# lRomul/sensorium

Measured on AMD Instinct MI355X. Metric: training clips/sec/GPU (DwiseNeuro fwd+bwd, B=32 T=32 36x64) at 1/2/4/8 GPUs, higher is better.
Workload: dtype bf16

## Files before the change

### include/dwn.h

```cpp
#ifndef DWN_H_
#define DWN_H_
#include <stddef.h>
#include <stdint.h>

#ifdef __cplusplus
extern "C" {
#endif

#define DWN_ABI_VERSION 7
#define DWN_F32 0
#define DWN_BF16 1
#define DWN_F32_AUTO 0
#define DWN_F32_NATIVE 1
#define DWN_F32_SPLIT3 2
#define DWN_BN_EVAL 0
#define DWN_BN_TRAIN 1
#define DWN_BN_FROZEN 2
#define DWN_NREP 32

#define DWN_LD_PLAIN 0
#define DWN_LD_PE 1
#define DWN_LD_BNACT 2
#define DWN_LD_AFFINE2 3
#define DWN_LD_DY3 4
// ... 85 lines not shown
    void* dh1;
    float* dw;
    int planes, Hin, Win, Hout, Wout, C, stride, ks;
    double* stats;
    int rows_band;
    int impl;
    const void* a0; long long a0_ld; const void* w1; int Cin;
} dwn_dw_spatial_bwd_args;

typedef struct dwn_dw_temporal_fwd_args {
    dwn_load_desc in;
    const float* w;
    void* out;
    int B, T, HW, C, kt;
    double* stats;
    const float* z_scale; const float* z_shift; long long* pooled;
} dwn_dw_temporal_fwd_args;

typedef struct dwn_dw_temporal_bwd_args {
    dwn_load_desc dy; int dy_kind;
    dwn_load_desc y2;
    const float* w;
    void* dh2;
    float* dw;
    int B, T, HW, C, kt;
    double* stats;
} dwn_dw_temporal_bwd_args;

typedef struct dwn_bn {
    const float* gamma; const float* beta;
    float* running_mean; float* running_var; long long* num_batches_tracked;
    float* coef;
    float* dgamma; float* dbeta;
} dwn_bn;

typedef struct dwn_stem_args {
    int dtype, training, B, Cin, C0; long long S;
    float eps, momentum;
    const float* x;
    const float* w;
    dwn_bn bn;
    const float *pe_t, *pe_h, *pe_w;
    int T, H, W;
    void* y0;
    void* out;
    const void* dout;
    float* dw;
    void* ws; size_t ws_bytes;
    double* xmom;
} dwn_stem_args;

typedef struct dwn_stem_input_grad_args {
    int dtype, training, B, Cin, C0; long long S;
    const float* w;
    const float* coef;
    const void* dout;
    float* dx;
} dwn_stem_input_grad_args;

typedef struct dwn_block_args {
    int dtype, training;
    int B, T, Hin, Win, Hout, Wout, Cin, Cmid, Cout, stride, ks, kt, se_r;
    float eps, momentum;
    const void* x; void* out;
    void *y1, *y2, *y3, *y4;
    void* z3;
    int x_has_pe;
    void* a0;
    const float *pe_t, *pe_h, *pe_w;
    const float *out_pe_t, *out_pe_h, *out_pe_w;
    const float *w_pw, *w_dws, *w_dwt, *w_pwl, *se_wr, *se_br, *se_we, *se_be;
    dwn_bn bn1, bn2, bn3, bn4, bnsc;
    const float* drop_scale;
    const int *hsrc, *wsrc, *hinv, *winv;
    float *se_pmean, *se_hidpre, *se_gate;
    const void* dout; void* dx;
    void *buf_a, *buf_b;
    void *dy4, *da0;
    float *dw_pw, *dw_dws, *dw_dwt, *dw_pwl, *dse_wr, *dse_br, *dse_we, *dse_be;
    void* ws; size_t ws_bytes;
    int pwl_bwd;
    int f32_products;
    int y1_mode;
} dwn_block_args;

typedef struct dwn_pool_args {
    int dtype; long long BT; int HW, C;
    const void* x; void* out; const void* dout; void* dx;
} dwn_pool_args;

typedef struct dwn_cortex_args {
    int dtype, training, B, T, Cin, C, groups;
    float eps, momentum;
    const void* x; void* out; void* y;
    const float* w;
    dwn_bn bn, bnsc;
    const float* drop_scale;
    const void* dout; void* dx; float* dw;
    const float* dout_mask; int dout_mask_ld;
    void* ws; size_t ws_bytes;
    int f32_products;
} dwn_cortex_args;

typedef struct dwn_readout_args {
    int dtype, B, T, Cin, groups, n_out;
    float softplus_beta;
    const void* x;
    const float* w; const float* bias;
    const float* drop_mask;
    float* out;
    const float* dout; void* dx; float* dw; float* dbias;
    void* ws; size_t ws_bytes;
    void* wt;
    int f32_products;
    const float* beta_dev; float* dbeta;
} dwn_readout_args;

typedef struct dwn_tensor_entry {
    float* param; const float* grad; float* exp_avg; float* exp_avg_sq; float* ema;
    long long numel; int is_int64; int pad_;
} dwn_tensor_entry;

typedef struct dwn_guarded_entry {
    float* param; const float* grad; float* exp_avg; float* exp_avg_sq; float* ema;
    long long numel; int is_int64; int pad_;
    long long* step;
} dwn_guarded_entry;
typedef struct dwn_step_guard {
    double norm;
    float coef;
    int skip;
    long long nonfinite;
    long long good_steps, skipped_steps;
} dwn_step_guard;
#define DWN_GS_SEG 1024

#define DWN_VID_U8 0
#define DWN_VID_F32 1
typedef struct dwn_clip_src {
    const void* video; const float* behavior; const float* pupil_center; const float* responses;
    long long length;
    int video_dtype;
    int frame_start, frame_step;
    int valid;
} dwn_clip_src;
#define DWN_MIX_BOX 0
#define DWN_MIX_BLEND 1
typedef struct dwn_clip_desc {
    dwn_clip_src src, mix;
    int bbx1, bby1, bbx2, bby2;
    float one_minus_lam, lam;
    int mouse;
    int mix_mode;
} dwn_clip_desc;

enum {
    DWN_FAM_PW_FWD = 0, DWN_FAM_DWS_FWD, DWN_FAM_DWT_FWD, DWN_FAM_SE_POOL, DWN_FAM_PWL_FWD, DWN_FAM_RESID_FWD,
    DWN_FAM_RESID_BWD, DWN_FAM_PWL_DGRAD, DWN_FAM_PWL_WGRAD, DWN_FAM_BN3_REDUCE, DWN_FAM_DWT_BWD, DWN_FAM_DWS_BWD,
    DWN_FAM_PW_DGRAD, DWN_FAM_PW_WGRAD, DWN_FAM_CORTEX_FWD, DWN_FAM_CORTEX_BWD, DWN_FAM_READOUT_FWD, DWN_FAM_READOUT_BWD,
    DWN_FAM_COUNT
};
#define DWN_PROF_ROCTX (1ull << 63)
int dwn_profile_enable(unsigned long long family_mask, int device);
int dwn_profile_collect(int family, double* total_ms, long long* launches);

int dwn_abi_version(void);
const char* dwn_source_hash(void);
int dwn_sizeof(const char* struct_name);
const char* dwn_last_error(void);

int dwn_gemm_nn(const dwn_gemm_nn_args* a, int dtype, int device, void* stream);
int dwn_gemm_tn(const dwn_gemm_tn_args* a, int dtype, int device, void* stream);
int dwn_dw_spatial_fwd(const dwn_dw_spatial_fwd_args* a, int dtype, int device, void* stream);
int dwn_dw_spatial_bwd(const dwn_dw_spatial_bwd_args* a, int dtype, int device, void* stream);
int dwn_dw_spatial_fwd_rc_supported(const dwn_dw_spatial_fwd_args* a, int dtype);
int dwn_dw_spatial_bwd_rc_supported(const dwn_dw_spatial_bwd_args* a, int dtype);
int dwn_dw_temporal_fwd(const dwn_dw_temporal_fwd_args* a, int dtype, int device, void* stream);
int dwn_dw_temporal_bwd(const dwn_dw_temporal_bwd_args* a, int dtype, int device, void* stream);
int dwn_dw_temporal_wide_fwd(const dwn_dw_temporal_fwd_args* a, int dtype, int device, void* stream);
int dwn_dw_temporal_wide_bwd(const dwn_dw_temporal_bwd_args* a, int dtype, int device, void* stream);
int dwn_bn_finalize(const double* stats, int stat_c, double count, const dwn_bn* bn, int C, int training,
                    float momentum, float eps, int device, void* stream);
int dwn_bn_bwd_finalize(const double* stats, double count, const dwn_bn* bn, float* abc, int C, int device,
                        void* stream);
int dwn_pack_weight(const float* src, void* dst, int groups, int R, int C, int transpose, int Rd, int Cd,
                    int dtype, int device, void* stream);
size_t dwn_conv_pw_bn_stats_workspace_bytes(int Cin);
int dwn_conv_pw_bn_stats(const void* a0, long long a0_ld, long long M, const float* w_pw, int E, int Cin, const dwn_bn* bn,
                         float momentum, float eps, double* sc_stats, void* ws, size_t ws_bytes, int dtype, int device,
                         void* stream);

size_t dwn_stem_workspace_bytes(const dwn_stem_args* a);
int dwn_stem_forward(const dwn_stem_args* a, int device, void* stream);
int dwn_stem_backward(const dwn_stem_args* a, int device, void* stream);
int dwn_stem_input_grad(const dwn_stem_input_grad_args* a, int device, void* stream);
int dwn_stem_backward_input(const dwn_stem_args* a, float* dx, int device, void* stream);
size_t dwn_block_workspace_bytes(const dwn_block_args* a, int backward);
int dwn_block_forward(const dwn_block_args* a, int device, void* stream);
int dwn_block_backward(const dwn_block_args* a, int device, void* stream);
int dwn_block_forward_writes(const dwn_block_args* a);
int dwn_pool_forward(const dwn_pool_args* a, int device, void* stream);
int dwn_pool_backward(const dwn_pool_args* a, int device, void* stream);
size_t dwn_cortex_workspace_bytes(const dwn_cortex_args* a, int backward);
int dwn_cortex_forward(const dwn_cortex_args* a, int device, void* stream);
int dwn_cortex_backward(const dwn_cortex_args* a, int device, void* stream);
size_t dwn_readout_workspace_bytes(const dwn_readout_args* a, int backward);
size_t dwn_readout_wt_bytes(const dwn_readout_args* a);
int dwn_readout_forward(const dwn_readout_args* a, int device, void* stream);
int dwn_readout_backward(const dwn_readout_args* a, int device, void* stream);

int dwn_poisson_loss_forward(const float* pred, const float* target, const float* w, long long per_sample,
                             long long total, float eps, double* loss_acc, int device, void* stream);
int dwn_poisson_loss_backward(const float* pred, const float* target, const float* w, const float* gscale,
                              long long per_sample, long long total, float eps, float* dpred, int device,
                              void* stream);
int dwn_f64_to_f32(const double* src, float* dst, int n, int device, void* stream);

int dwn_adamw_ema_multi(const dwn_tensor_entry* list, int ntensors, int max_blocks, double lr, double beta1,
                        double beta2, double eps, double weight_decay, long long step, double ema_decay,
                        double grad_scale, int device, void* stream);
int dwn_ema_lerp_multi(const dwn_tensor_entry* list, int ntensors, int max_blocks, double decay, int device,
                       void* stream);

size_t dwn_grad_guard_workspace_bytes(int ntensors, int max_blocks);
int dwn_grad_sumsq_multi(const dwn_guarded_entry* list, int ntensors, int max_blocks, double grad_scale, void* ws,
                         size_t ws_bytes, double* pair, int device, void* stream);
int dwn_step_guard_finalize(const double* pair_a, const double* pair_b, double max_norm, int skip_nonfinite,
                            const dwn_guarded_entry* list, int ntensors, dwn_step_guard* guard, int device, void* stream);
int dwn_adamw_ema_multi_guarded(const dwn_guarded_entry* list, int ntensors, int max_blocks, double lr, double beta1,
                                double beta2, double eps, double weight_decay, double ema_decay, double grad_scale,
                                const dwn_step_guard* guard, int device, void* stream);


typedef struct dwn_pw_bwd_args {
    const void* dh1; const void* a0; const float* w_pw; const float* abc;
    void* da0; float* dw;
    long long M; int E; int Cin;
    void* ws; size_t ws_bytes;
    const void* res; const float* res_abc; int res_C;
    const int* res_hinv; const int* res_winv; int res_Hin, res_Win, res_Hout, res_Wout;
} dwn_pw_bwd_args;
int dwn_pw_bwd_fused_supported(int dtype, long long M, int E, int Cin);
size_t dwn_pw_backward_workspace_bytes(int E, int Cin, int dtype);
int dwn_pw_backward(const dwn_pw_bwd_args* a, int dtype, int device, void* stream);

typedef struct dwn_dw_spatial_rc_fwd_args {
    const void* a0; long long a0_ld;
    const void* blob;
    void* out;
    int planes, Hin, Win, Hout, Wout, Cin, E, stride;
    double* stats;
    int rows_band;
    int round_y1;
} dwn_dw_spatial_rc_fwd_args;
size_t dwn_dw_spatial_rc_blob_bytes(int E, int Cin);
int dwn_dw_spatial_rc_prep(const float* w_pw, const float* w_dws, const float* bn1_coef, int E, int Cin, void* blob,
                           int device, void* stream);
int dwn_dw_spatial_rc_supported(int dtype, int Cin, int E, int ks, int stride, int Hin, int Win);
int dwn_dw_spatial_fwd_rc(const dwn_dw_spatial_rc_fwd_args* a, int device, void* stream);

int dwn_assemble_inputs(const dwn_clip_desc* descs, int B, int T, int H0, int W0, int H, int W, float pad_fill,
                        float* x, int device, void* stream);
int dwn_assemble_targets(const dwn_clip_desc* descs, int B, int T, float* const* targets, const int* n_neurons,
                         int n_mice, int max_neurons, float* mice_weights, int device, void* stream);

typedef struct dwn_gaze_args {
    int B, Cin, T, H, W;
    int video_channel;
    float fill;
    int pad_;
    const float* x;
    const float* shift;
    float* out;
    const float* dout;
    float* dx;
    float* dshift;
} dwn_gaze_args;
int dwn_gaze_shift_forward(const dwn_gaze_args* a, int device, void* stream);
int dwn_gaze_shift_backward(const dwn_gaze_args* a, int device, void* stream);
int dwn_plane_mean(const float* x, int B, int Cin, int T, int H, int W, int c0, int nc, float* mean, int device, void* stream);

#define DWN_CORR_STAT_ROWS 8
#define DWN_CORR_TILE 16
enum { DWN_CORR_MEAN = 0, DWN_CORR_SUM = 1 };
typedef struct dwn_corr_args {
    int B, N, T;
    int reduction;
    double eps;
    long long w_stride;
    const float* pred;
    const float* target;
    const float* w;
    double* stat;
    double* count;
    const float* share;
    double* loss_acc;
    const float* gscale;
    float* dpred;
    void* ws; size_t ws_bytes;
} dwn_corr_args;
size_t dwn_corr_ws_bytes(const dwn_corr_args* a);
int dwn_corr_moments(const dwn_corr_args* a, int device, void* stream);
int dwn_corr_loss_finalize(const dwn_corr_args* a, int device, void* stream);
int dwn_corr_loss_backward(const dwn_corr_args* a, int device, void* stream);

enum { DWN_GABOR_GAUSSIAN = 0, DWN_GABOR_NONE = 1 };
typedef struct dwn_gabor_args {
    int B, Cin, T, H, W;
    int video_channel;
    int envelope;
    int clamp;
    int y0, x0, wh, ww;
    float background, lo, hi, pad;
    const float* x;
    const float* params;
    float* out;
    const float* dout;
    float* dparams;
    void* ws; size_t ws_bytes;
} dwn_gabor_args;
size_t dwn_gabor_workspace_bytes(const dwn_gabor_args* a);
int dwn_gabor_forward(const dwn_gabor_args* a, int device, void* stream);
int dwn_gabor_backward(const dwn_gabor_args* a, int device, void* stream);
// ... 212 lines not shown
```

### sensorium_amd/_lib.py

```python
from __future__ import annotations

import ctypes as C
import os
from pathlib import Path

import torch

_HERE = Path(__file__).resolve().parent
DETERMINISTIC = os.environ.get("DWN_DETERMINISTIC", "0") == "1"
_LIB_NAME = "libdwiseneuro_hip_det.so" if DETERMINISTIC else "libdwiseneuro_hip.so"
LIB_PATH = Path(os.environ["DWN_LIB_PATH"]) if os.environ.get("DWN_LIB_PATH") else _HERE / "csrc" / _LIB_NAME

c_p = C.c_void_p
c_i = C.c_int
c_ll = C.c_longlong
c_f = C.c_float
c_d = C.c_double
c_sz = C.c_size_t

DWN_F32, DWN_BF16 = 0, 1
DWN_NREP = 32
LD_PLAIN, LD_PE, LD_BNACT, LD_AFFINE2, LD_DY3, LD_GATE, LD_CAT1 = 0, 1, 2, 3, 4, 5, 6
EPI_STORE, EPI_READOUT, EPI_DG, EPI_STORE_CAT, EPI_DH3 = 0, 1, 2, 3, 4
NN_AUTO, NN_XL128, NN_XL256, NN_TILE128, NN_KD = 0, 1, 2, 3, 4
# ... 7 lines not shown
class LoadDesc(C.Structure):
    _fields_ = [("p", c_p), ("q", c_p), ("ld", c_ll), ("v1", c_p), ("v2", c_p), ("v3", c_p), ("v4", c_p),
                ("v5", c_p), ("gate", c_p), ("gate2", c_p), ("gate_ld", c_i), ("rows_per_sample", c_i),
                ("act", c_i), ("pe_t", c_p), ("pe_h", c_p), ("pe_w", c_p), ("pT", c_i), ("pH", c_i),
                ("pW", c_i), ("pe_ld", c_i), ("ld2", c_ll), ("cat_c1", c_i), ("cat_c2", c_i)]


class GemmNNArgs(C.Structure):
    _fields_ = [("a", LoadDesc), ("a_kind", c_i), ("b", c_p), ("ldb", c_ll), ("c", c_p), ("ldc", c_ll),
                ("M", c_i), ("N", c_i), ("K", c_i), ("groups", c_i), ("stats", c_p),
                ("f32_split", c_i), ("stat_nchan", c_i), ("epi", c_i), ("bias", c_p),
                ("sp_beta", c_f), ("out_nct", c_p), ("Tn", c_i), ("n_valid", c_i), ("y3", c_p), ("ldy3", c_ll),
                ("s3", c_p), ("t3", c_p), ("dg", c_p), ("dg_ld", c_i), ("rows_per_sample", c_i),
                ("a2", c_p), ("a2_ld", c_ll), ("K1", c_i), ("b_sample_stride", c_ll), ("b_rows_per_sample", c_i),
                ("gate3", c_p), ("dps3", c_p), ("coef3", c_p), ("coef3_ld", c_i), ("variant", c_i), ("sp_beta_dev", c_p)]


class GemmTNArgs(C.Structure):
    _fields_ = [("p", LoadDesc), ("p_kind", c_i), ("q", LoadDesc), ("q_kind", c_i), ("M", c_i), ("R", c_i),
                ("Cc", c_i), ("dw", c_p), ("lddw", c_ll), ("groups", c_i), ("rows_per_split", c_i),
                ("nsplit", c_i), ("R_load", c_i), ("rows_per_sample", c_i), ("splits_per_sample", c_i),
                ("dw_sample_stride", c_ll), ("overwrite", c_i), ("dw_f64", c_i)]


class DwSpatialFwdArgs(C.Structure):
    _fields_ = [("inp", LoadDesc), ("w", c_p), ("out", c_p), ("planes", c_i), ("Hin", c_i), ("Win", c_i),
                ("Hout", c_i), ("Wout", c_i), ("C", c_i), ("stride", c_i), ("ks", c_i), ("stats", c_p),
                ("rows_band", c_i), ("impl", c_i),
                ("a0", c_p), ("a0_ld", c_ll), ("w1", c_p), ("Cin", c_i)]


class DwSpatialBwdArgs(C.Structure):
    _fields_ = [("dy", LoadDesc), ("y1", LoadDesc), ("w", c_p), ("dh1", c_p), ("dw", c_p), ("planes", c_i),
                ("Hin", c_i), ("Win", c_i), ("Hout", c_i), ("Wout", c_i), ("C", c_i), ("stride", c_i),
                ("ks", c_i), ("stats", c_p), ("rows_band", c_i), ("impl", c_i),
                ("a0", c_p), ("a0_ld", c_ll), ("w1", c_p), ("Cin", c_i)]


class DwTemporalFwdArgs(C.Structure):
    _fields_ = [("inp", LoadDesc), ("w", c_p), ("out", c_p), ("B", c_i), ("T", c_i), ("HW", c_i), ("C", c_i),
                ("kt", c_i), ("stats", c_p), ("z_scale", c_p), ("z_shift", c_p), ("pooled", c_p)]


class DwTemporalBwdArgs(C.Structure):
    _fields_ = [("dy", LoadDesc), ("dy_kind", c_i), ("y2", LoadDesc), ("w", c_p), ("dh2", c_p), ("dw", c_p),
                ("B", c_i), ("T", c_i), ("HW", c_i), ("C", c_i), ("kt", c_i), ("stats", c_p)]


class BN(C.Structure):
    _fields_ = [("gamma", c_p), ("beta", c_p), ("running_mean", c_p), ("running_var", c_p),
                ("num_batches_tracked", c_p), ("coef", c_p), ("dgamma", c_p), ("dbeta", c_p)]


class StemArgs(C.Structure):
    _fields_ = [("dtype", c_i), ("training", c_i), ("B", c_i), ("Cin", c_i), ("C0", c_i), ("S", c_ll),
                ("eps", c_f), ("momentum", c_f), ("x", c_p), ("w", c_p), ("bn", BN),
                ("pe_t", c_p), ("pe_h", c_p), ("pe_w", c_p), ("T", c_i), ("H", c_i), ("W", c_i),
                ("y0", c_p), ("out", c_p),
                ("dout", c_p), ("dw", c_p), ("ws", c_p), ("ws_bytes", c_sz), ("xmom", c_p)]


class StemInputGradArgs(C.Structure):
    _fields_ = [("dtype", c_i), ("training", c_i), ("B", c_i), ("Cin", c_i), ("C0", c_i), ("S", c_ll),
                ("w", c_p), ("coef", c_p), ("dout", c_p), ("dx", c_p)]


class BlockArgs(C.Structure):
    _fields_ = [("dtype", c_i), ("training", c_i),
                ("B", c_i), ("T", c_i), ("Hin", c_i), ("Win", c_i), ("Hout", c_i), ("Wout", c_i), ("Cin", c_i),
                ("Cmid", c_i), ("Cout", c_i), ("stride", c_i), ("ks", c_i), ("kt", c_i), ("se_r", c_i),
                ("eps", c_f), ("momentum", c_f),
                ("x", c_p), ("out", c_p), ("y1", c_p), ("y2", c_p), ("y3", c_p), ("y4", c_p),
                ("z3", c_p), ("x_has_pe", c_i), ("a0", c_p),
                ("pe_t", c_p), ("pe_h", c_p), ("pe_w", c_p),
                ("out_pe_t", c_p), ("out_pe_h", c_p), ("out_pe_w", c_p),
                ("w_pw", c_p), ("w_dws", c_p), ("w_dwt", c_p), ("w_pwl", c_p), ("se_wr", c_p), ("se_br", c_p),
                ("se_we", c_p), ("se_be", c_p),
                ("bn1", BN), ("bn2", BN), ("bn3", BN), ("bn4", BN), ("bnsc", BN),
                ("drop_scale", c_p), ("hsrc", c_p), ("wsrc", c_p), ("hinv", c_p), ("winv", c_p),
                ("se_pmean", c_p), ("se_hidpre", c_p), ("se_gate", c_p),
                ("dout", c_p), ("dx", c_p), ("buf_a", c_p), ("buf_b", c_p), ("dy4", c_p), ("da0", c_p),
                ("dw_pw", c_p), ("dw_dws", c_p), ("dw_dwt", c_p), ("dw_pwl", c_p), ("dse_wr", c_p),
                ("dse_br", c_p), ("dse_we", c_p), ("dse_be", c_p),
                ("ws", c_p), ("ws_bytes", c_sz), ("pwl_bwd", c_i), ("f32_products", c_i), ("y1_mode", c_i)]


class PoolArgs(C.Structure):
    _fields_ = [("dtype", c_i), ("BT", c_ll), ("HW", c_i), ("C", c_i), ("x", c_p), ("out", c_p), ("dout", c_p),
                ("dx", c_p)]


class CortexArgs(C.Structure):
    _fields_ = [("dtype", c_i), ("training", c_i), ("B", c_i), ("T", c_i), ("Cin", c_i), ("C", c_i),
                ("groups", c_i), ("eps", c_f), ("momentum", c_f), ("x", c_p), ("out", c_p), ("y", c_p),
                ("w", c_p), ("bn", BN), ("bnsc", BN), ("drop_scale", c_p), ("dout", c_p), ("dx", c_p),
                ("dw", c_p), ("dout_mask", c_p), ("dout_mask_ld", c_i), ("ws", c_p), ("ws_bytes", c_sz), ("f32_products", c_i)]


class ReadoutArgs(C.Structure):
    _fields_ = [("dtype", c_i), ("B", c_i), ("T", c_i), ("Cin", c_i), ("groups", c_i), ("n_out", c_i),
                ("softplus_beta", c_f), ("x", c_p), ("w", c_p), ("bias", c_p), ("drop_mask", c_p), ("out", c_p),
                ("dout", c_p), ("dx", c_p), ("dw", c_p), ("dbias", c_p), ("ws", c_p), ("ws_bytes", c_sz), ("wt", c_p),
                ("f32_products", c_i), ("beta_dev", c_p), ("dbeta", c_p)]


class TensorEntry(C.Structure):
    _fields_ = [("param", c_p), ("grad", c_p), ("exp_avg", c_p), ("exp_avg_sq", c_p), ("ema", c_p),
                ("numel", c_ll), ("is_int64", c_i), ("pad_", c_i)]


class GuardedEntry(C.Structure):
    _fields_ = [("param", c_p), ("grad", c_p), ("exp_avg", c_p), ("exp_avg_sq", c_p), ("ema", c_p),
                ("numel", c_ll), ("is_int64", c_i), ("pad_", c_i), ("step", c_p)]


class StepGuard(C.Structure):
    _fields_ = [("norm", c_d), ("coef", c_f), ("skip", c_i), ("nonfinite", c_ll), ("good_steps", c_ll),
                ("skipped_steps", c_ll)]


class ClipSrc(C.Structure):
    _fields_ = [("video", c_p), ("behavior", c_p), ("pupil_center", c_p), ("responses", c_p), ("length", c_ll),
                ("video_dtype", c_i), ("frame_start", c_i), ("frame_step", c_i), ("valid", c_i)]


class ClipDesc(C.Structure):
    _fields_ = [("src", ClipSrc), ("mix", ClipSrc), ("bbx1", c_i), ("bby1", c_i), ("bbx2", c_i), ("bby2", c_i),
                ("one_minus_lam", c_f), ("lam", c_f), ("mouse", c_i), ("mix_mode", c_i)]


class PwBwdArgs(C.Structure):
    _fields_ = [("dh1", c_p), ("a0", c_p), ("w_pw", c_p), ("abc", c_p), ("da0", c_p), ("dw", c_p),
                ("M", c_ll), ("E", c_i), ("Cin", c_i), ("ws", c_p), ("ws_bytes", c_sz), ("res", c_p), ("res_abc", c_p),
                ("res_C", c_i), ("res_hinv", c_p), ("res_winv", c_p), ("res_Hin", c_i), ("res_Win", c_i), ("res_Hout", c_i),
                ("res_Wout", c_i)]


class DwSpatialRcFwdArgs(C.Structure):
    _fields_ = [("a0", c_p), ("a0_ld", c_ll), ("blob", c_p), ("out", c_p), ("planes", c_i), ("Hin", c_i),
                ("Win", c_i), ("Hout", c_i), ("Wout", c_i), ("Cin", c_i), ("E", c_i), ("stride", c_i),
                ("stats", c_p), ("rows_band", c_i), ("round_y1", c_i)]


class GazeArgs(C.Structure):
    _fields_ = [("B", c_i), ("Cin", c_i), ("T", c_i), ("H", c_i), ("W", c_i), ("video_channel", c_i), ("fill", c_f),
                ("pad_", c_i), ("x", c_p), ("shift", c_p), ("out", c_p), ("dout", c_p), ("dx", c_p), ("dshift", c_p)]


class CorrArgs(C.Structure):
    _fields_ = [("B", c_i), ("N", c_i), ("T", c_i), ("reduction", c_i), ("eps", c_d), ("w_stride", c_ll), ("pred", c_p),
                ("target", c_p), ("w", c_p), ("stat", c_p), ("count", c_p), ("share", c_p), ("loss_acc", c_p), ("gscale", c_p),
                ("dpred", c_p), ("ws", c_p), ("ws_bytes", c_sz)]


class GaborArgs(C.Structure):
    _fields_ = [("B", c_i), ("Cin", c_i), ("T", c_i), ("H", c_i), ("W", c_i), ("video_channel", c_i), ("envelope", c_i),
                ("clamp", c_i), ("y0", c_i), ("x0", c_i), ("wh", c_i), ("ww", c_i), ("background", c_f), ("lo", c_f), ("hi", c_f),
                ("pad", c_f), ("x", c_p), ("params", c_p), ("out", c_p), ("dout", c_p), ("dparams", c_p), ("ws", c_p),
                ("ws_bytes", c_sz)]


class ModulatorArgs(C.Structure):
    _fields_ = [("B", c_i), ("N", c_i), ("T", c_i), ("K", c_i), ("max_log_gain", c_f), ("pad_", c_i), ("y", c_p), ("h", c_p),
                ("u", c_p), ("c", c_p), ("out", c_p), ("dout", c_p), ("dy", c_p), ("dh", c_p), ("du", c_p), ("dc", c_p),
                ("ws", c_p), ("ws_bytes", c_sz)]


class Blur3dArgs(C.Structure):
    _fields_ = [("B", c_i), ("T", c_i), ("H", c_i), ("W", c_i), ("Cin_src", c_i), ("c_src", c_i), ("Cin_dst", c_i), ("c_dst", c_i),
                ("Rt", c_i), ("Rh", c_i), ("Rw", c_i), ("y0", c_i), ("x0", c_i), ("wh", c_i), ("ww", c_i), ("pad_", c_i),
                ("src", c_p), ("dst", c_p), ("taps", c_p), ("ws", c_p), ("ws_bytes", c_sz)]


class ClipMomentsArgs(C.Structure):
    _fields_ = [("B", c_i), ("Cin", c_i), ("T", c_i), ("H", c_i), ("W", c_i), ("c", c_i), ("y0", c_i), ("x0", c_i), ("wh", c_i),
                ("ww", c_i), ("x", c_p), ("stat", c_p), ("ws", c_p), ("ws_bytes", c_sz)]


class MeiUpdateArgs(C.Structure):
    _fields_ = [("mode", c_i), ("B", c_i), ("Cin", c_i), ("T", c_i), ("H", c_i), ("W", c_i), ("c", c_i), ("y0", c_i), ("x0", c_i),
                ("wh", c_i), ("ww", c_i), ("Cin_g", c_i), ("c_g", c_i), ("has_mean", c_i), ("has_contrast", c_i),
                ("contrast_mode", c_i), ("lo", c_f), ("hi", c_f), ("mean_target", C.c_double), ("contrast", C.c_double),
                ("x", c_p), ("g", c_p), ("stat", c_p), ("lr", c_p)]


class TrialDesc(C.Structure):
    _fields_ = [("pred", c_p), ("target", c_p), ("ld_pred", c_ll), ("ld_target", c_ll), ("first", c_i), ("frames", c_i)]


class TrialGroup(C.Structure):
    _fields_ = [("first_trial", c_i), ("repeats", c_i), ("frames", c_i)]


class TrialScoreArgs(C.Structure):
    _fields_ = [("N", c_i), ("n_trials", c_i), ("n_groups", c_i), ("max_repeats", c_i), ("max_frames", c_i), ("pad_", c_i),
                ("n_all", c_ll), ("n_repeat", c_ll), ("n_group_frames", c_ll), ("eps", c_d), ("fev_threshold", c_d),
                ("trials", c_p), ("groups", c_p), ("state", c_p), ("scores", c_p), ("summary", c_p), ("ws", c_p), ("ws_bytes", c_sz)]


class PairSeg(C.Structure):
    _fields_ = [("x", c_p), ("ld", c_ll), ("first", c_i), ("frames", c_i)]


class PairArgs(C.Structure):
    _fields_ = [("N", c_i), ("kind", c_i), ("n_segs", c_i), ("n_groups", c_i), ("max_repeats", c_i), ("max_frames", c_i),
                ("cols", c_i), ("out_f32", c_i), ("n", c_ll), ("eps", c_d), ("segs", c_p), ("groups", c_p), ("state", c_p),
                ("out", c_p), ("ws", c_p), ("ws_bytes", c_sz)]


class PairCompareArgs(C.Structure):
    _fields_ = [("N", c_i), ("M", c_i), ("lda", c_ll), ("ldb", c_ll), ("eps", c_d), ("A", c_p), ("B", c_p), ("sel", c_p),
                ("per_neuron", c_p), ("summary", c_p), ("ws", c_p), ("ws_bytes", c_sz)]


class SpatialGainArgs(C.Structure):
    _fields_ = [("B", c_i), ("N", c_i), ("T", c_i), ("Hf", c_i), ("Wf", c_i), ("K", c_i), ("g_dtype", c_i), ("max_log_gain", c_f),
                ("y", c_p), ("g", c_p), ("pos", c_p), ("weight", c_p), ("bias", c_p), ("out", c_p), ("dout", c_p), ("dy", c_p),
                ("dg", c_p), ("dpos", c_p), ("dweight", c_p), ("dbias", c_p), ("ws", c_p), ("ws_bytes", c_sz)]
# ... 12 lines not shown
                ("rel_threshold", c_d), ("x", c_p), ("r", c_p), ("r0", c_p), ("state", c_p), ("cov", c_p), ("z", c_p),
                ("summary", c_p), ("ws", c_p), ("ws_bytes", c_sz)]


class Gauss2dArgs(C.Structure):
    _fields_ = [("R", c_i), ("gh", c_i), ("gw", c_i), ("M", c_i), ("fit_baseline", c_i), ("max_iter", c_i), ("rel_threshold", c_d),
                ("xtol", c_d), ("ftol", c_d), ("maps", c_p), ("sel", c_p), ("params", c_p), ("table", c_p), ("ws", c_p),
                ("ws_bytes", c_sz)]


class Gauss2dProfileArgs(C.Structure):
    _fields_ = [("N", c_i), ("L", c_i), ("gh", c_i), ("gw", c_i), ("fit_baseline", c_i), ("pad_", c_i), ("params", c_p), ("maps", c_p),
                ("profile", c_p), ("separability", c_p)]


CORR_STAT_ROWS, CORR_TILE = 8, 16
CORR_MEAN, CORR_SUM = 0, 1
GABOR_GAUSSIAN, GABOR_NONE = 0, 1
BLUR_MAX_RADIUS, BLUR_TAPS_STRIDE, MOMENTS_CHUNK = 16, 33, 4096
MEI_STEP, MEI_PROJECT = 0, 1
MEI_CONTRAST_MAX, MEI_CONTRAST_FIXED = 0, 1
TRIAL_STATE_ROWS, TRIAL_SCORE_ROWS, TRIAL_SUMMARY, TRIAL_TILE = 17, 5, 8, 4
NOISE_BINARY, NOISE_SPARSE = 0, 1
STA_SUMMARY = 8
GAUSS_PARAMS, GAUSS_TABLE = 7, 16
PAIR_TOTAL, PAIR_SIGNAL, PAIR_NOISE = 0, 1, 2
PAIR_TILE, PAIR_KSTEP, PAIR_SUMMARY, PAIR_ROW_STATS = 64, 4, 8, 8
MIX_BOX, MIX_BLEND = 0, 1
VID_U8, VID_F32 = 0, 1

_OLD_STRUCTS = {
    "dwn_load_desc": LoadDesc, "dwn_gemm_nn_args": GemmNNArgs, "dwn_gemm_tn_args": GemmTNArgs,
    "dwn_dw_spatial_fwd_args": DwSpatialFwdArgs, "dwn_dw_spatial_bwd_args": DwSpatialBwdArgs,
    "dwn_dw_temporal_fwd_args": DwTemporalFwdArgs, "dwn_dw_temporal_bwd_args": DwTemporalBwdArgs,
    "dwn_bn": BN, "dwn_stem_args": StemArgs, "dwn_block_args": BlockArgs, "dwn_pool_args": PoolArgs,
    "dwn_cortex_args": CortexArgs, "dwn_readout_args": ReadoutArgs, "dwn_tensor_entry": TensorEntry,
    "dwn_clip_src": ClipSrc, "dwn_clip_desc": ClipDesc, "dwn_pw_bwd_args": PwBwdArgs,
    "dwn_dw_spatial_rc_fwd_args": DwSpatialRcFwdArgs,
}
_NEW_STRUCTS = {
    "dwn_stem_input_grad_args": StemInputGradArgs,
    "dwn_guarded_entry": GuardedEntry, "dwn_step_guard": StepGuard, "dwn_gaze_args": GazeArgs,
    "dwn_corr_args": CorrArgs, "dwn_gabor_args": GaborArgs, "dwn_modulator_args": ModulatorArgs,
    "dwn_blur3d_args": Blur3dArgs, "dwn_clip_moments_args": ClipMomentsArgs, "dwn_mei_update_args": MeiUpdateArgs,
    "dwn_trial_desc": TrialDesc, "dwn_trial_group": TrialGroup, "dwn_trial_score_args": TrialScoreArgs,
    "dwn_spatial_gain_args": SpatialGainArgs, "dwn_noise_args": NoiseArgs, "dwn_sta_args": StaArgs,
    "dwn_gauss2d_args": Gauss2dArgs, "dwn_gauss2d_profile_args": Gauss2dProfileArgs,
    "dwn_pair_seg": PairSeg, "dwn_pair_args": PairArgs, "dwn_pair_compare_args": PairCompareArgs,
}
_STRUCTS = {**_OLD_STRUCTS, **_NEW_STRUCTS}


class _new(tuple):
    def __new__(cls, restype, argtypes):
        return super().__new__(cls, (restype, argtypes))


_P = C.POINTER
SYMBOLS = {
    "dwn_abi_version": (c_i, []),
    "dwn_source_hash": (C.c_char_p, []),
    "dwn_sizeof": (c_i, [C.c_char_p]),
    "dwn_last_error": (C.c_char_p, []),
    "dwn_profile_enable": (c_i, [C.c_ulonglong, c_i]),
    "dwn_profile_collect": (c_i, [c_i, _P(c_d), _P(c_ll)]),
    "dwn_gemm_nn": (c_i, [_P(GemmNNArgs), c_i, c_i, c_p]),
    "dwn_gemm_tn": (c_i, [_P(GemmTNArgs), c_i, c_i, c_p]),
    "dwn_dw_spatial_fwd": (c_i, [_P(DwSpatialFwdArgs), c_i, c_i, c_p]),
    "dwn_dw_spatial_bwd": (c_i, [_P(DwSpatialBwdArgs), c_i, c_i, c_p]),
    "dwn_dw_spatial_bwd_rc_supported": (c_i, [_P(DwSpatialBwdArgs), c_i]),
    "dwn_dw_spatial_fwd_rc_supported": (c_i, [_P(DwSpatialFwdArgs), c_i]),
    "dwn_dw_temporal_fwd": (c_i, [_P(DwTemporalFwdArgs), c_i, c_i, c_p]),
    "dwn_dw_temporal_bwd": (c_i, [_P(DwTemporalBwdArgs), c_i, c_i, c_p]),
    "dwn_dw_temporal_wide_fwd": _new(c_i, [_P(DwTemporalFwdArgs), c_i, c_i, c_p]),
    "dwn_dw_temporal_wide_bwd": _new(c_i, [_P(DwTemporalBwdArgs), c_i, c_i, c_p]),
    "dwn_bn_finalize": (c_i, [c_p, c_i, c_d, _P(BN), c_i, c_i, c_f, c_f, c_i, c_p]),
    "dwn_bn_bwd_finalize": (c_i, [c_p, c_d, _P(BN), c_p, c_i, c_i, c_p]),
    "dwn_pack_weight": (c_i, [c_p, c_p, c_i, c_i, c_i, c_i, c_i, c_i, c_i, c_i, c_p]),
    "dwn_stem_workspace_bytes": (c_sz, [_P(StemArgs)]),
    "dwn_stem_forward": (c_i, [_P(StemArgs), c_i, c_p]),
    "dwn_stem_backward": (c_i, [_P(StemArgs), c_i, c_p]),
    "dwn_stem_input_grad": _new(c_i, [_P(StemInputGradArgs), c_i, c_p]),
    "dwn_stem_backward_input": _new(c_i, [_P(StemArgs), c_p, c_i, c_p]),
    "dwn_block_workspace_bytes": (c_sz, [_P(BlockArgs), c_i]),
    "dwn_block_forward": (c_i, [_P(BlockArgs), c_i, c_p]),
    "dwn_block_backward": (c_i, [_P(BlockArgs), c_i, c_p]),
    "dwn_block_forward_writes": (c_i, [_P(BlockArgs)]),
    "dwn_pool_forward": (c_i, [_P(PoolArgs), c_i, c_p]),
    "dwn_pool_backward": (c_i, [_P(PoolArgs), c_i, c_p]),
    "dwn_cortex_workspace_bytes": (c_sz, [_P(CortexArgs), c_i]),
    "dwn_cortex_forward": (c_i, [_P(CortexArgs), c_i, c_p]),
    "dwn_cortex_backward": (c_i, [_P(CortexArgs), c_i, c_p]),
    "dwn_readout_workspace_bytes": (c_sz, [_P(ReadoutArgs), c_i]),
    "dwn_readout_wt_bytes": (c_sz, [_P(ReadoutArgs)]),
    "dwn_readout_forward": (c_i, [_P(ReadoutArgs), c_i, c_p]),
    "dwn_readout_backward": (c_i, [_P(ReadoutArgs), c_i, c_p]),
    "dwn_poisson_loss_forward": (c_i, [c_p, c_p, c_p, c_ll, c_ll, c_f, c_p, c_i, c_p]),
    "dwn_poisson_loss_backward": (c_i, [c_p, c_p, c_p, c_p, c_ll, c_ll, c_f, c_p, c_i, c_p]),
    "dwn_f64_to_f32": (c_i, [c_p, c_p, c_i, c_i, c_p]),
    "dwn_adamw_ema_multi": (c_i, [c_p, c_i, c_i, c_d, c_d, c_d, c_d, c_d, c_ll, c_d, c_d, c_i, c_p]),
    "dwn_ema_lerp_multi": (c_i, [c_p, c_i, c_i, c_d, c_i, c_p]),
    "dwn_grad_guard_workspace_bytes": _new(c_sz, [c_i, c_i]),
    "dwn_grad_sumsq_multi": _new(c_i, [c_p, c_i, c_i, c_d, c_p, c_sz, c_p, c_i, c_p]),
    "dwn_step_guard_finalize": _new(c_i, [c_p, c_p, c_d, c_i, c_p, c_i, c_p, c_i, c_p]),
    "dwn_adamw_ema_multi_guarded": _new(c_i, [c_p, c_i, c_i, c_d, c_d, c_d, c_d, c_d, c_d, c_d, c_p, c_i, c_p]),
    "dwn_conv_pw_bn_stats_workspace_bytes": (c_sz, [c_i]),
    "dwn_conv_pw_bn_stats": (c_i, [c_p, c_ll, c_ll, c_p, c_i, c_i, _P(BN), c_f, c_f, c_p, c_p, c_sz, c_i, c_i, c_p]),
    "dwn_pw_bwd_fused_supported": (c_i, [c_i, c_ll, c_i, c_i]),
    "dwn_pw_backward_workspace_bytes": (c_sz, [c_i, c_i, c_i]),
    "dwn_pw_backward": (c_i, [_P(PwBwdArgs), c_i, c_i, c_p]),
    "dwn_dw_spatial_rc_blob_bytes": (c_sz, [c_i, c_i]),
    "dwn_dw_spatial_rc_prep": (c_i, [c_p, c_p, c_p, c_i, c_i, c_p, c_i, c_p]),
    "dwn_dw_spatial_rc_supported": (c_i, [c_i, c_i, c_i, c_i, c_i, c_i, c_i]),
    "dwn_dw_spatial_fwd_rc": (c_i, [_P(DwSpatialRcFwdArgs), c_i, c_p]),
    "dwn_assemble_inputs": (c_i, [c_p, c_i, c_i, c_i, c_i, c_i, c_i, c_f, c_p, c_i, c_p]),
    "dwn_assemble_targets": (c_i, [c_p, c_i, c_i, c_p, c_p, c_i, c_i, c_p, c_i, c_p]),
    "dwn_gaze_shift_forward": _new(c_i, [_P(GazeArgs), c_i, c_p]),
    "dwn_gaze_shift_backward": _new(c_i, [_P(GazeArgs), c_i, c_p]),
    "dwn_plane_mean": _new(c_i, [c_p, c_i, c_i, c_i, c_i, c_i, c_i, c_i, c_p, c_i, c_p]),
    "dwn_corr_ws_bytes": _new(c_sz, [_P(CorrArgs)]),
    "dwn_corr_moments": _new(c_i, [_P(CorrArgs), c_i, c_p]),
    "dwn_corr_loss_finalize": _new(c_i, [_P(CorrArgs), c_i, c_p]),
    "dwn_corr_loss_backward": _new(c_i, [_P(CorrArgs), c_i, c_p]),
    "dwn_gabor_workspace_bytes": _new(c_sz, [_P(GaborArgs)]),
    "dwn_gabor_forward": _new(c_i, [_P(GaborArgs), c_i, c_p]),
    "dwn_gabor_backward": _new(c_i, [_P(GaborArgs), c_i, c_p]),
    "dwn_modulator_ws_bytes": _new(c_sz, [_P(ModulatorArgs)]),
    "dwn_modulator_forward": _new(c_i, [_P(ModulatorArgs), c_i, c_p]),
    "dwn_modulator_backward": _new(c_i, [_P(ModulatorArgs), c_i, c_p]),
    "dwn_blur3d_ws_bytes": _new(c_sz, [_P(Blur3dArgs)]),
    "dwn_clip_moments_ws_bytes": _new(c_sz, [_P(ClipMomentsArgs)]),
    "dwn_blur3d": _new(c_i, [_P(Blur3dArgs), c_i, c_p]),
    "dwn_clip_moments": _new(c_i, [_P(ClipMomentsArgs), c_i, c_p]),
    "dwn_mei_update": _new(c_i, [_P(MeiUpdateArgs), c_i, c_p]),
    "dwn_trial_score_ws_bytes": _new(c_sz, [_P(TrialScoreArgs)]),
    "dwn_trial_moments": _new(c_i, [_P(TrialScoreArgs), c_i, c_p]),
    "dwn_trial_score_finalize": _new(c_i, [_P(TrialScoreArgs), c_i, c_p]),
    "dwn_spatial_gain_ws_bytes": _new(c_sz, [_P(SpatialGainArgs)]),
    "dwn_spatial_gain_forward": _new(c_i, [_P(SpatialGainArgs), c_i, c_p]),
    "dwn_spatial_gain_backward": _new(c_i, [_P(SpatialGainArgs), c_i, c_p]),
    "dwn_pair_ldz": _new(c_ll, [c_i]),
    "dwn_pair_state_bytes": _new(c_sz, [_P(PairArgs)]),
    "dwn_pair_ws_bytes": _new(c_sz, [_P(PairArgs)]),
    "dwn_pair_compare_ws_bytes": _new(c_sz, [_P(PairCompareArgs)]),
    "dwn_pair_stage": _new(c_i, [_P(PairArgs), c_i, c_p]),
    "dwn_pair_syrk": _new(c_i, [_P(PairArgs), c_i, c_p]),
    "dwn_pair_corr_finalize": _new(c_i, [_P(PairArgs), c_i, c_p]),
    "dwn_pair_compare": _new(c_i, [_P(PairCompareArgs), c_i, c_p]),
    "dwn_gauss2d_ws_bytes": _new(c_sz, [_P(Gauss2dArgs)]),
    "dwn_gauss2d_fit": _new(c_i, [_P(Gauss2dArgs), c_i, c_p]),
    "dwn_gauss2d_profile": _new(c_i, [_P(Gauss2dProfileArgs), c_i, c_p]),
    "dwn_noise_forward": _new(c_i, [_P(NoiseArgs), c_i, c_p]),
    "dwn_sta_state_bytes": _new(c_sz, [_P(StaArgs)]),
    "dwn_sta_ws_bytes": _new(c_sz, [_P(StaArgs)]),
    "dwn_sta_accumulate": _new(c_i, [_P(StaArgs), c_i, c_p]),
    "dwn_sta_finalize": _new(c_i, [_P(StaArgs), c_i, c_p]),
}


class DwnError(RuntimeError):
    pass


HASH_SRCS = ("dwn_api.hip", "dwn_gemm.hip", "dwn_gemm_nn_1.hip", "dwn_gemm_nn_2.hip", "dwn_gemm_nn_3.hip", "dwn_gemm_nn_4.hip", "dwn_gemm_nn_5.hip",
             "dwn_gemm_nn_6.hip", "dwn_gemm_tn.hip", "dwn_gram.hip", "dwn_pw_bwd.hip", "dwn_gemm_xl.hip", "dwn_gemm_kd.hip", "dwn_dwconv.hip", "dwn_dwrc.hip",
             "dwn_dwbwd.hip", "dwn_dwfwd.hip", "dwn_elementwise.hip", "dwn_data.hip", "dwn_gaze.hip", "dwn_modulator.hip", "dwn_spatial.hip", "dwn_mei.hip", "dwn_rf_fit.hip", "dwn_pairwise.hip", "dwn_trial_score.hip", "dwn_rf.hip", "dwn_corr.hip", "dwn_stim.hip", "dwn_common.h", "dwn_internal.h",
             "dwn_kernels.h", "dwn_launch.h", "dwn_gemm_nn.h", "dwn_gain.h", "dwn_reduce.h",
             "../../include/dwn.h")


def source_hash() -> str:
    import hashlib
    h = hashlib.sha256()
    for name in HASH_SRCS:
        h.update((_HERE / "csrc" / name).read_bytes())
    return h.hexdigest()[:16]


def _load():
    if not LIB_PATH.exists():
        raise ImportError(
            f"{LIB_PATH} is missing: build it with `python -c 'import __graft_entry__ as g; g.build()'` "
            f"(or `make -C {LIB_PATH.parent}`).  sensorium_amd has no fallback path.")
    lib = C.CDLL(str(LIB_PATH), mode=getattr(os, "RTLD_NOW", 2))
    ab = bool(os.environ.get("DWN_LIB_PATH"))
    for name, proto in SYMBOLS.items():
        if ab and isinstance(proto, _new) and not hasattr(lib, name):
            continue
        restype, argtypes = proto
        fn = getattr(lib, name)
        fn.restype = restype
        fn.argtypes = argtypes
    if lib.dwn_abi_version() != 7 and not (ab and lib.dwn_abi_version() == 6):
        raise ImportError("libdwiseneuro_hip.so ABI version mismatch")
    built, have = lib.dwn_source_hash().decode(), source_hash()
    if built != have and not os.environ.get("DWN_LIB_PATH"):
        raise ImportError(f"{LIB_PATH.name} was built from other sources (binary {built}, tree {have}): rebuild it with "
                          f"`make -C {LIB_PATH.parent}` — binaries are not in git, so what runs must be what is committed")
    for cname, struct in _STRUCTS.items():
        n = lib.dwn_sizeof(cname.encode())
        if n != C.sizeof(struct) and not (ab and (0 < n < C.sizeof(struct) or cname in _NEW_STRUCTS)):
            raise ImportError(f"struct layout mismatch for {cname}: C {n} bytes vs ctypes {C.sizeof(struct)}")
    return lib


lib = _load()


def check(rc: int, what: str = ""):
    if rc != 0:
        msg = lib.dwn_last_error()
        raise DwnError(f"{what} failed (rc={rc}): {msg.decode() if msg else ''}")
```

### sensorium_amd/csrc/dwn_api.hip

```cpp
#include "dwn_internal.h"
#include "dwn_kernels.h"
#include <string.h>
#include <math.h>

static thread_local char g_err[512] = "";
#ifndef DWN_EVAL_CHAIN
#define DWN_EVAL_CHAIN 1
#endif

extern "C" size_t dwn_dw_spatial_rc_blob_bytes(int E, int Cin);
extern "C" int dwn_dw_spatial_rc_supported(int dtype, int Cin, int E, int ks, int stride, int Hin, int Win);
extern "C" int dwn_dw_spatial_rc_prep(const float* w_pw, const float* w_dws, const float* bn1_coef, int E, int Cin, void* blob,
                                      int device, void* stream);
extern "C" int dwn_dw_spatial_fwd_rc(const dwn_dw_spatial_rc_fwd_args* a, int device, void* stream);
bool dw_spatial_bwd_rc_supported(const DwSpatialBwd& a, int dtype);
bool dw_spatial_fwd_rc_walk_supported(const DwSpatialFwd& a, int dtype);

int dwn_set_error(int code, const char* msg) {
    snprintf(g_err, sizeof(g_err), "dwn error %d: %s", code, msg ? msg : "");
    return code;
}

#define TRY(x) do { int rc__ = (x); if (rc__ != 0) return rc__; } while (0)

// ... 334 lines not shown
    ENTER(device);
    return bn_finalize(stats, stat_c, count, *bn, C, training, momentum, eps, (hipStream_t)stream);
}
int dwn_bn_bwd_finalize(const double* stats, double count, const dwn_bn* bn, float* abc, int C, int device,
                        void* stream) {
    ENTER(device);
    return k_bn_bwd_finalize(bwd_job(stats, count, *bn, abc, C, false), BnBwdJob{}, (hipStream_t)stream);
}
size_t dwn_conv_pw_bn_stats_workspace_bytes(int Cin) {
    const int nrep = gram_nrep(DWN_BF16, Cin) > gram_nrep(DWN_F32, Cin) ? gram_nrep(DWN_BF16, Cin) : gram_nrep(DWN_F32, Cin);
    return (size_t)nrep * (Cin + 8) * Cin * sizeof(double) + 256;
}
int dwn_conv_pw_bn_stats(const void* a0, long long a0_ld, long long M, const float* w_pw, int E, int Cin, const dwn_bn* bn,
                         float momentum, float eps, double* sc_stats, void* ws, size_t ws_bytes, int dtype, int device, void* stream) {
    ENTER(device);
    hipStream_t s = (hipStream_t)stream;
    if (!a0 || !w_pw || !bn || !bn->coef || !ws) return dwn_set_error(-1, "conv_pw_bn_stats: null pointer");
    if (Cin % 8 || E <= 0 || M <= 0 || M >= (1ll << 31)) return dwn_set_error(-2, "conv_pw_bn_stats: Cin % 8 == 0, 0 < M < 2^31");
    if (ws_bytes < dwn_conv_pw_bn_stats_workspace_bytes(Cin)) return dwn_set_error(-6, "conv_pw_bn_stats: workspace too small");
    double* gram = reinterpret_cast<double*>(((size_t)ws + 255) & ~(size_t)255);
    const int nrep = gram_nrep(dtype, Cin);
    TRY(k_zero(gram, (size_t)nrep * (Cin + 8) * Cin * sizeof(double), s));
    bool streamed = false;
    TRY(k_gram(a0, a0_ld, M, Cin, gram, dtype, &streamed, s));
    if (!streamed) {
        LoadDesc cat = ld_plain(a0, a0_ld);
        cat.cat_c1 = Cin; cat.cat_c2 = 0;
        GemmTN g = tn_base(cat, LD_CAT1, ld_plain(a0, a0_ld), LD_PLAIN, (int)M, Cin + 8, Cin, reinterpret_cast<float*>(gram), Cin, 1);
        g.dw_f64 = 1;
        TRY(launch_gemm_tn(g, dtype, s));
    }
    return k_bn1_gram_finalize(gram, streamed ? nrep : 1, w_pw, E, Cin, (double)M, bn->gamma, bn->beta, bn->running_mean, bn->running_var,
                               bn->num_batches_tracked, momentum, eps, bn->coef, sc_stats, dtype, s);
}
int dwn_pack_weight(const float* src, void* dst, int groups, int R, int C, int transpose, int Rd, int Cd, int dtype,
                    int device, void* stream) {
    ENTER(device);
    return k_pack_weight(src, dst, groups, R, C, transpose, Rd, Cd, dtype, (hipStream_t)stream);
}

size_t dwn_stem_workspace_bytes(const dwn_stem_args* a) {
    return ((size_t)DWN_NREP * stem_moment_count() * sizeof(double) + 256 +
            (size_t)DWN_NREP * a->C0 * stem_acc_stride() * sizeof(double) + 1024);
}
int dwn_stem_forward(const dwn_stem_args* a, int device, void* stream) {
    ENTER(device);
    hipStream_t s = (hipStream_t)stream;
    if (a->C0 % 8) return dwn_set_error(-2, "stem: C0 must be a multiple of 8");
    if (a->pe_t && (i64)a->T * a->H * a->W != a->S) return dwn_set_error(-2, "stem: T*H*W != S");
    Carver c(a->ws, a->ws_bytes);
    double* mom = c.take<double>((size_t)DWN_NREP * stem_moment_count());
    if (!c.ok()) return dwn_set_error(-6, "stem: workspace too small");
    const i64 M = (i64)a->B * a->S;
    if (a->training == DWN_BN_TRAIN) {
        if (!a->xmom) return dwn_set_error(-1, "stem_forward: xmom buffer required in training mode");
        TRY(k_zero(mom, (size_t)DWN_NREP * stem_moment_count() * sizeof(double), s));
        TRY(k_stem_xmom(a->x, a->B, a->Cin, a->S, mom, s));
        TRY(k_stem_bn_finalize(mom, (double)M, a->w, a->bn.gamma, a->bn.beta, a->bn.running_mean, a->bn.running_var,
                               a->bn.num_batches_tracked, a->momentum, a->eps, a->bn.coef, a->xmom, a->C0, a->Cin, s));
    } else {
        TRY(bn_finalize(nullptr, a->C0, (double)M, a->bn, a->C0, 0, a->momentum, a->eps, s));
    }
    return k_stem_out(a->x, a->w, a->bn.coef, a->pe_t, a->pe_h, a->pe_w, a->T, a->H, a->W, a->B, a->Cin, a->S, a->C0, a->out,
                      a->dtype, s);
}
int dwn_stem_backward(const dwn_stem_args* a, int device, void* stream) {
    ENTER(device);
    hipStream_t s = (hipStream_t)stream;
    const bool frozen = a->training == DWN_BN_FROZEN;
    if (!frozen && !a->xmom) return dwn_set_error(-1, "stem_backward: xmom (saved by the forward) required");
    Carver c(a->ws, a->ws_bytes);
    double* mom = c.take<double>((size_t)DWN_NREP * stem_moment_count());
    double* acc = c.take<double>((size_t)DWN_NREP * a->C0 * stem_acc_stride());
    if (!c.ok()) return dwn_set_error(-6, "stem: workspace too small");
    const i64 M = (i64)a->B * a->S;
    if (frozen) {
        TRY(k_zero(mom, (size_t)((char*)(acc + (size_t)DWN_NREP * a->C0 * stem_acc_stride()) - (char*)mom), s));
        TRY(k_stem_bwd_acc(a->dout, a->x, mom, (double)M, a->B, a->Cin, a->S, a->C0, acc, a->dtype, s));
        return k_stem_bwd_finalize_frozen(acc, a->w, a->bn.coef, a->bn.dgamma, a->bn.dbeta, a->dw, a->C0, a->Cin, s);
    }
    TRY(k_zero(acc, (size_t)DWN_NREP * a->C0 * stem_acc_stride() * sizeof(double), s));
    TRY(k_stem_bwd_acc(a->dout, a->x, a->xmom, (double)M, a->B, a->Cin, a->S, a->C0, acc, a->dtype, s));
    return k_stem_bwd_finalize(acc, a->xmom, a->w, a->bn.coef, (double)M, a->bn.dgamma, a->bn.dbeta, a->dw, a->C0, a->Cin, s);
}

int dwn_stem_backward_input(const dwn_stem_args* a, float* dx, int device, void* stream) {
    g_err[0] = 0;
    if (!a || !dx) return dwn_set_error(-1, "stem_backward_input: null pointer (args, dx)");
    if (a->training != DWN_BN_TRAIN)
        return dwn_set_error(-7, "stem_backward_input: built for batch statistics (DWN_BN_TRAIN) only; the frozen-statistics input "
                                 "gradient is dwn_stem_backward + dwn_stem_input_grad");
    if (!a->x || !a->w || !a->bn.coef || !a->dout || !a->dw || !a->xmom || !a->ws)
        return dwn_set_error(-1, "stem_backward_input: null pointer (x, w, bn.coef, dout, dw, xmom, ws)");
    if (a->C0 <= 0 || a->C0 % 8 || a->Cin <= 0 || a->B <= 0 || a->S <= 0)
        return dwn_set_error(-2, "stem_backward_input: C0 must be a positive multiple of 8; B, Cin, S positive");
    if (a->dtype != DWN_F32 && a->dtype != DWN_BF16) return dwn_set_error(-2, "stem_backward_input: dtype");
    if (a->C0 > (a->dtype == DWN_BF16 ? 128 : 64) || a->Cin > 8)
        return dwn_set_error(-4, "stem_backward_input: more than 128 (bf16) / 64 (fp32) stem channels or 8 input channels not built");
    ENTER(device);
    hipStream_t s = (hipStream_t)stream;
    Carver c(a->ws, a->ws_bytes);
    double* mom = c.take<double>((size_t)DWN_NREP * stem_moment_count());
    double* acc = c.take<double>((size_t)DWN_NREP * a->C0 * stem_acc_stride());
    if (!c.ok()) return dwn_set_error(-6, "stem: workspace too small");
    float* qx = reinterpret_cast<float*>(mom);
    const i64 M = (i64)a->B * a->S;
    TRY(k_zero(acc, (size_t)DWN_NREP * a->C0 * stem_acc_stride() * sizeof(double), s));
    TRY(k_stem_bwd_acc(a->dout, a->x, a->xmom, (double)M, a->B, a->Cin, a->S, a->C0, acc, a->dtype, s));
    TRY(k_stem_bwd_finalize(acc, a->xmom, a->w, a->bn.coef, (double)M, a->bn.dgamma, a->bn.dbeta, a->dw, a->C0, a->Cin, s));
    TRY(k_stem_bwd_finalize_dx(acc, a->xmom, a->w, a->bn.coef, (double)M, qx, a->C0, a->Cin, s));
    return k_stem_input_grad_train(a->dout, a->w, a->bn.coef, a->x, qx, a->B, a->Cin, a->S, a->C0, dx, a->dtype, s);
}

int dwn_stem_input_grad(const dwn_stem_input_grad_args* a, int device, void* stream) {
    g_err[0] = 0;
    if (!a || !a->w || !a->coef || !a->dout || !a->dx) return dwn_set_error(-1, "stem_input_grad: null pointer");
    if (a->C0 <= 0 || a->C0 % 8 || a->Cin <= 0 || a->B <= 0 || a->S <= 0)
        return dwn_set_error(-2, "stem_input_grad: C0 must be a positive multiple of 8; B, Cin, S positive");
    if (a->dtype != DWN_F32 && a->dtype != DWN_BF16) return dwn_set_error(-2, "stem_input_grad: dtype");
    if (a->training != DWN_BN_FROZEN)
        return dwn_set_error(-7, "stem_input_grad: this entry is the frozen-statistics (DWN_BN_FROZEN) input gradient; through batch "
                                 "statistics (DWN_BN_TRAIN) it is dwn_stem_backward_input");
    ENTER(device);
    return k_stem_input_grad(a->dout, a->w, a->coef, a->B, a->Cin, a->S, a->C0, a->dx, a->dtype, (hipStream_t)stream);
}

size_t dwn_block_workspace_bytes(const dwn_block_args* a, int backward) {
    return carve_block(*a, backward, nullptr, 0).bytes;
}

int dwn_block_forward(const dwn_block_args* ap, int device, void* stream) {
    ENTER(device);
    const dwn_block_args& a = *ap;
    hipStream_t s = (hipStream_t)stream;
    TRY(check_block(a));
    BlockWs w = carve_block(a, 0, a.ws, a.ws_bytes);
    if (w.bytes > a.ws_bytes) return dwn_set_error(-6, "block_forward: workspace too small");
    const int dt = a.dtype, tr = a.training != DWN_BN_EVAL;
    const bool bs = a.training == DWN_BN_TRAIN;
    const i64 Min = (i64)a.B * a.T * a.Hin * a.Win, Mout = (i64)a.B * a.T * a.Hout * a.Wout;
    const int S_out = a.T * a.Hout * a.Wout;
    {
        PrepArgs pa;
        bool ok = pa.zero(w.zero_beg, ((size_t)(w.zero_end - w.zero_beg) + 15) & ~(size_t)15);
        ok = ok && pa.packw(a.w_pw, w.wpw, 1, a.Cmid, a.Cin, 0, a.Cmid, a.Cin);
        ok = ok && pa.packw(a.w_pwl, w.wpwl, 1, a.Cout, a.Cmid, 0, a.Cout, a.Cmid);
        ok = ok && pa.packdw(a.w_dws, w.wdws, a.Cmid, a.ks * a.ks);
        ok = ok && pa.packdw(a.w_dwt, w.wdwt, a.Cmid, a.kt);
        if (!bs) {
            ok = ok && pa.bneval(a.bn1, a.Cmid, a.eps) && pa.bneval(a.bn2, a.Cmid, a.eps) && pa.bneval(a.bn3, a.Cmid, a.eps);
            ok = ok && pa.bneval(a.bn4, a.Cout, a.eps) && pa.bneval(a.bnsc, a.Cout, a.eps);
        }
        if (!ok) return dwn_set_error(-2, "block_forward: workspace arena must be 16-byte aligned");
        TRY(k_prep(pa, dt, s));
    }

    const void* a0 = a.x;
    if (!a.x_has_pe) {
        if (!a.a0) return dwn_set_error(-2, "block_forward: a0 buffer required when x_has_pe == 0");
        TRY(k_ew_apply(ld_pe(a.x, a.Cin, a.pe_t, a.pe_h, a.pe_w, a.T, a.Hin, a.Win), LD_PE, a.a0, a.Cin, Min, a.Cin, dt, s));
        a0 = a.a0;
    }
    LoadDesc xin = ld_plain(a0, a.Cin);
    const bool identity_sc = a.stride == 1 && a.Hin == a.Hout && a.Win == a.Wout;
    const bool y1_free = tr && block_y1_free(a);
    bool eval_chain = false;
// ... 18 lines not shown
        PROF(DWN_FAM_PW_FWD, k_gram(a0, a.Cin, Min, a.Cin, w.gram, dt, &streamed, s));
        if (!streamed) {
        GemmTN g = tn_base(cat, LD_CAT1, ld_plain(a0, a.Cin), LD_PLAIN, (int)Min, a.Cin + 8, a.Cin, reinterpret_cast<float*>(w.gram), a.Cin, 1);
        g.dw_f64 = 1;
        PROF(DWN_FAM_PW_FWD, launch_gemm_tn(g, dt, s));
        }
        PROF(DWN_FAM_PW_FWD, k_bn1_gram_finalize(w.gram, streamed ? gram_nrep(dt, a.Cin) : 1, a.w_pw, a.Cmid, a.Cin, (double)Min, a.bn1.gamma, a.bn1.beta, a.bn1.running_mean,
                                                 a.bn1.running_var, a.bn1.num_batches_tracked, a.momentum, a.eps, a.bn1.coef,
                                                 identity_sc ? w.stsc : nullptr, dt, s));
        }
        DwSpatialFwd d; memset(&d, 0, sizeof(d));
        d.in = ld_bnact(nullptr, a.Cmid, a.bn1.coef, a.Cmid, 1, nullptr, 0, 1);
        d.a0 = a0; d.a0_ld = a.Cin; d.w1 = w.wpw; d.Cin = a.Cin;
        d.w = w.wdws; d.out = a.y2; d.planes = a.B * a.T; d.Hin = a.Hin; d.Win = a.Win; d.Hout = a.Hout;
        d.Wout = a.Wout; d.C = a.Cmid; d.stride = a.stride; d.ks = a.ks; d.stats = w.st2;
        PROF(DWN_FAM_DWS_FWD, launch_dw_spatial_fwd(d, dt, s));
    } else if (block_fwd_rc(a)) {
        TRY(dwn_dw_spatial_rc_prep(a.w_pw, w.wdws, a.bn1.coef, a.Cmid, a.Cin, w.rcblob, device, stream));
        dwn_dw_spatial_rc_fwd_args r; memset(&r, 0, sizeof(r));
        r.a0 = a0; r.a0_ld = a.Cin; r.blob = w.rcblob; r.out = a.y2; r.planes = a.B * a.T; r.Hin = a.Hin; r.Win = a.Win;
        r.Hout = a.Hout; r.Wout = a.Wout; r.Cin = a.Cin; r.E = a.Cmid; r.stride = a.stride; r.stats = nullptr;
        r.rows_band = 0; r.round_y1 = 1;
        PROF(DWN_FAM_DWS_FWD, dwn_dw_spatial_fwd_rc(&r, device, stream));
    } else {
    {
        GemmNN g = nn_base(xin, LD_PLAIN, w.wpw, a.Cin, a.y1, a.Cmid, (int)Min, a.Cmid, a.Cin, 1);
        g.f32_split = f32_split_of(a.f32_products, !tr);
        g.stats = tr ? w.st1 : nullptr; g.stat_nchan = a.Cmid;
        PROF(DWN_FAM_PW_FWD, launch_gemm_nn(g, dt, s));
    }
    if (bs) TRY(bn_finalize(w.st1, a.Cmid, (double)Min, a.bn1, a.Cmid, 1, a.momentum, a.eps, s));
    {
        DwSpatialFwd d; memset(&d, 0, sizeof(d));
        d.in = ld_bnact(a.y1, a.Cmid, a.bn1.coef, a.Cmid, 1, nullptr, 0, 1);
        d.w = w.wdws; d.out = a.y2; d.planes = a.B * a.T; d.Hin = a.Hin; d.Win = a.Win; d.Hout = a.Hout;
        d.Wout = a.Wout; d.C = a.Cmid; d.stride = a.stride; d.ks = a.ks; d.stats = tr ? w.st2 : nullptr;
        PROF(DWN_FAM_DWS_FWD, launch_dw_spatial_fwd(d, dt, s));
    }
    }
    if (bs) TRY(bn_finalize(w.st2, a.Cmid, (double)Mout, a.bn2, a.Cmid, 1, a.momentum, a.eps, s));
    const bool eval_z3 = !tr;
    {
        DwTemporalFwd d; memset(&d, 0, sizeof(d));
        d.in = ld_bnact(a.y2, a.Cmid, a.bn2.coef, a.Cmid, 1, nullptr, 0, 1);
        d.w = w.wdwt; d.out = a.y3; d.B = a.B; d.T = a.T; d.HW = a.Hout * a.Wout; d.C = a.Cmid; d.kt = a.kt;
        d.stats = tr ? w.st3 : nullptr;
        if (eval_z3) {
            d.out = a.z3; d.z_scale = a.bn3.coef; d.z_shift = a.bn3.coef + a.Cmid; d.pooled = w.pooled;
        }
        PROF(DWN_FAM_DWT_FWD, launch_dw_temporal_fwd(d, dt, s));
    }
    if (bs) TRY(bn_finalize(w.st3, a.Cmid, (double)Mout, a.bn3, a.Cmid, 1, a.momentum, a.eps, s));
    if (!eval_z3) {
        LoadDesc z3 = ld_bnact(a.y3, a.Cmid, a.bn3.coef, a.Cmid, 1, nullptr, 0, S_out);
        PROF(DWN_FAM_SE_POOL, k_se_pool(z3, a.B, a.Cmid, S_out, w.pooled, a.z3, dt, s));
    }
    int gate_folded = 0;
    TRY(k_se_mlp_fwd(w.pooled, 1.0f / (float)S_out, a.se_wr, a.se_br, a.se_we, a.se_be, a.B, a.Cmid, a.se_r,
                     a.se_pmean, a.se_hidpre, a.se_gate, pwl_gated_weights(a) ? a.w_pwl : nullptr, w.wgated, a.Cout, dt, &gate_folded, s));
    if (pwl_gated_weights(a)) {
        if (!gate_folded) TRY(k_gate_weights(a.w_pwl, a.se_gate, w.wgated, a.B, a.Cout, a.Cmid, dt, s));
        GemmNN g = nn_base(ld_plain(a.z3, a.Cmid), LD_PLAIN, w.wgated, a.Cmid, a.y4, a.Cout, (int)Mout, a.Cout, a.Cmid, 1);
        g.b_sample_stride = (i64)a.Cout * a.Cmid; g.b_rows_per_sample = S_out;
        g.stats = tr ? w.st4 : nullptr; g.stat_nchan = a.Cout; g.f32_split = f32_split_of(a.f32_products, !tr);
        PROF(DWN_FAM_PWL_FWD, launch_gemm_nn(g, dt, s));
    } else {
        LoadDesc u = ld_plain(a.z3, a.Cmid);
        u.gate = a.se_gate; u.gate_ld = a.Cmid; u.rows_per_sample = S_out;
        GemmNN g = nn_base(u, LD_GATE, w.wpwl, a.Cmid, a.y4, a.Cout, (int)Mout, a.Cout, a.Cmid, 1);
        g.stats = tr ? w.st4 : nullptr; g.stat_nchan = a.Cout; g.f32_split = f32_split_of(a.f32_products, !tr);
        PROF(DWN_FAM_PWL_FWD, launch_gemm_nn(g, dt, s));
    }
    ResGeom gm = geom_of(a);
    if (bs) {
        if (!(y1_free && identity_sc)) PROF(DWN_FAM_RESID_FWD, k_shortcut_stats(xin, gm, w.stsc, dt, s));
        TRY(k_bn_finalize_train(fin_job(w.st4, a.Cout, (double)Mout, a.bn4, a.Cout),
                                 fin_job(w.stsc, a.Cin, (double)Mout, a.bnsc, a.Cout), a.momentum, a.eps, s));
    }
    PROF(DWN_FAM_RESID_FWD, k_residual_fwd(xin, a.y4, a.bn4.coef, a.bnsc.coef, a.drop_scale, gm, a.out_pe_t, a.out_pe_h,
                                           a.out_pe_w, a.out, dt, s));
    return 0;
}

static int pw_backward(int dt, const void* dh1, const void* a0, const float* w_pw, const float* abc, int E, int Cin, i64 M,
                       void* bp, float* gacc, float* r3, float* tacc, void* da0, float* dw, const void* res,
                       const float* res_abc, int res_C, const ResGeom* rg, hipStream_t s, bool fold = true) {
    const int res_n = res ? res_C / Cin : 0;
    const bool gathered = res && rg && rg->hinv;
    if (res && (!res_abc || res_C % Cin || res_n < 1 || res_n > 2))
        return dwn_set_error(-2, "pw_backward: the shortcut term needs res_abc and res_C in {Cin, 2 Cin}");
    if (res && !pw_bwd_fused_supported(dt, M, E, Cin))
        return dwn_set_error(-3, "pw_backward: the shortcut term is built into the one-pass kernel only (dwn_pw_bwd_fused_supported)");
    TRY(k_pw_bwd_prep(w_pw, abc, E, Cin, bp, gacc, r3, dt, (res && !gathered) ? res_abc : nullptr, res_C, s));
    if (pw_bwd_fused_supported(dt, M, E, Cin)) {
        PROF(DWN_FAM_PW_DGRAD, launch_pw_bwd_fused(dh1, a0, bp, r3, da0, tacc, M, E, Cin, dt, res, res_abc, res_n,
                                                   gathered ? rg->hinv : nullptr, gathered ? rg->winv : nullptr, gathered ? rg->Hin : 0,
                                                   gathered ? rg->Win : 0, gathered ? rg->Hout : 0, gathered ? rg->Wout : 0, s));
    } else {
        {
            GemmNN g = nn_base(ld_plain(dh1, E), LD_PLAIN, bp, (i64)E + Cin, da0, Cin, (int)M, Cin, E + Cin, 1);
            g.epi = EPI_STORE_CAT; g.a2 = a0; g.a2_ld = Cin; g.K1 = E; g.bias = r3;
            PROF(DWN_FAM_PW_DGRAD, launch_gemm_nn(g, dt, s));
        }
        {
            LoadDesc cat = ld_plain(dh1, E);
            cat.q = a0; cat.ld2 = Cin; cat.cat_c1 = E; cat.cat_c2 = Cin;
            GemmTN g = tn_base(cat, LD_CAT1, ld_plain(a0, Cin), LD_PLAIN, (int)M, E + Cin + 8, Cin, tacc, Cin, 1);
            PROF(DWN_FAM_PW_WGRAD, launch_gemm_tn(g, dt, s));
        }
    }
    if (!fold) return 0;
    return k_pw_wgrad_fold(tacc, abc, w_pw, E, Cin, dw, dt, s);
}

int dwn_block_backward(const dwn_block_args* ap, int device, void* stream) {
    const dwn_block_args& a = *ap;
    hipStream_t s = (hipStream_t)stream;
    g_err[0] = 0;
    TRY(check_block(a));
    if (a.training == DWN_BN_EVAL)
        return dwn_set_error(-7, "block_backward: only training-mode (batch-statistics) and frozen-statistics backward are built");
    ENTER(device);
    const bool frozen = a.training == DWN_BN_FROZEN;
    BlockWs w = carve_block(a, 1, a.ws, a.ws_bytes);
    if (w.bytes > a.ws_bytes) return dwn_set_error(-6, "block_backward: workspace too small");
    const int dt = a.dtype;
    const i64 Min = (i64)a.B * a.T * a.Hin * a.Win, Mout = (i64)a.B * a.T * a.Hout * a.Wout;
    const int S_out = a.T * a.Hout * a.Wout;
    float* dg = reinterpret_cast<float*>(w.pooled);
    const bool y1_free = block_y1_free(a);
    {
        PrepArgs pa;
        bool ok = pa.zero(w.zero_beg, ((size_t)(w.zero_end - w.zero_beg) + 15) & ~(size_t)15);
        ok = ok && pa.packw(a.w_pwl, w.wpwl, 1, a.Cout, a.Cmid, 1, a.Cmid, a.Cout);
        if (y1_free) ok = ok && pa.packw(a.w_pw, w.wpw, 1, a.Cmid, a.Cin, 0, a.Cmid, a.Cin);
        ok = ok && pa.packdw(a.w_dws, w.wdws, a.Cmid, a.ks * a.ks);
        ok = ok && pa.packdw(a.w_dwt, w.wdwt, a.Cmid, a.kt);
        ok = ok && pa.fill(w.ident3, 1.0f, a.Cmid);
        ok = ok && pa.fill(w.ident3 + a.Cmid, 0.0f, 2 * a.Cmid);
        ok = ok && pa.zero(a.dw_dws, (size_t)a.Cmid * a.ks * a.ks * sizeof(float));
        ok = ok && pa.zero(a.dw_dwt, (size_t)a.Cmid * a.kt * sizeof(float));
        ok = ok && pa.zero(a.dw_pwl, (size_t)a.Cout * a.Cmid * sizeof(float));
        if (w.pb) ok = ok && pa.zero(w.pb, (size_t)a.B * a.Cout * a.Cmid * sizeof(float));
        ok = ok && pa.zero(w.gacc, pw_fold_floats(a.Cin) * sizeof(float));
        ok = ok && pa.zero(w.tacc, pw_wgrad_tacc_floats(a.Cmid, a.Cin) * sizeof(float));
        if (!ok) return dwn_set_error(-2, "block_backward: workspace arena and dw_* buffers must be 16-byte aligned");
        TRY(k_prep(pa, dt, s));
    }

    LoadDesc xin = ld_plain(a.x_has_pe ? a.x : a.a0, a.Cin);
    ResGeom gm = geom_of(a);
    PROF(DWN_FAM_RESID_BWD, k_residual_bwd_reduce(xin, a.y4, a.dout, a.bn4.coef, a.bnsc.coef, a.drop_scale, gm, w.st4, w.stsc, dt, s));
    TRY(k_bn_bwd_finalize(bwd_job(w.st4, (double)Mout, a.bn4, w.abc4, a.Cout, frozen),
                          bwd_job(w.stsc, (double)Mout, a.bnsc, w.abcsc, a.Cout, frozen), s));
    PROF(DWN_FAM_RESID_BWD, k_residual_bwd_dy4(a.y4, a.dout, w.abc4, a.drop_scale, gm, a.dy4, dt, s));
    void* du = a.buf_a;
    if (w.pb) {
        {
            GemmTN g = tn_base(ld_plain(a.dy4, a.Cout), LD_PLAIN, ld_plain(a.z3, a.Cmid), LD_PLAIN, (int)Mout, a.Cout,
                               a.Cmid, w.pb, a.Cmid, 1);
            g.rows_per_sample = S_out; g.dw_sample_stride = (i64)a.Cout * a.Cmid;
            PROF(DWN_FAM_PWL_WGRAD, launch_gemm_tn(g, dt, s));
        }
        PROF(DWN_FAM_PWL_WGRAD, k_pwl_bwd_reduce(w.pb, a.se_gate, a.w_pwl, a.B, a.Cout, a.Cmid, a.dw_pwl, dg, s));
        TRY(k_se_mlp_bwd(dg, a.se_gate, a.se_hidpre, a.se_pmean, a.se_wr, a.se_we, a.B, a.Cmid, a.se_r,
                         1.0f / (float)S_out, w.dgp, w.dhp, w.dps, a.dse_wr, a.dse_br, a.dse_we, a.dse_be, s, false));
        GemmNN g = nn_base(ld_plain(a.dy4, a.Cout), LD_PLAIN, w.wpwl, a.Cout, du, a.Cmid, (int)Mout, a.Cmid, a.Cout, 1);
        g.epi = EPI_DH3; g.y3 = a.y3; g.ldy3 = a.Cmid; g.gate3 = a.se_gate; g.dps3 = w.dps; g.dg_ld = a.Cmid;
        g.coef3 = a.bn3.coef; g.coef3_ld = a.Cmid; g.rows_per_sample = S_out;
        g.stats = w.st3; g.stat_nchan = a.Cmid;
        PROF(DWN_FAM_PWL_DGRAD, launch_gemm_nn(g, dt, s));
    } else {
    {
        GemmNN g = nn_base(ld_plain(a.dy4, a.Cout), LD_PLAIN, w.wpwl, a.Cout, du, a.Cmid, (int)Mout, a.Cmid, a.Cout, 1);
        g.epi = EPI_DG; g.y3 = a.z3; g.ldy3 = a.Cmid; g.s3 = nullptr; g.t3 = nullptr; g.dg = dg;
        g.dg_ld = a.Cmid; g.rows_per_sample = S_out;
        PROF(DWN_FAM_PWL_DGRAD, launch_gemm_nn(g, dt, s));
    }
    {
        LoadDesc u = ld_plain(a.z3, a.Cmid);
        u.gate = a.se_gate; u.gate_ld = a.Cmid; u.rows_per_sample = S_out;
        GemmTN g = tn_base(ld_plain(a.dy4, a.Cout), LD_PLAIN, u, LD_GATE, (int)Mout, a.Cout, a.Cmid, a.dw_pwl, a.Cmid, 1);
        PROF(DWN_FAM_PWL_WGRAD, launch_gemm_tn(g, dt, s));
    }
    TRY(k_se_mlp_bwd(dg, a.se_gate, a.se_hidpre, a.se_pmean, a.se_wr, a.se_we, a.B, a.Cmid, a.se_r,
                     1.0f / (float)S_out, w.dgp, w.dhp, w.dps, a.dse_wr, a.dse_br, a.dse_we, a.dse_be, s, false));
    LoadDesc d3; memset(&d3, 0, sizeof(d3));
    d3.p = du; d3.q = a.y3; d3.ld = a.Cmid; d3.v1 = w.ident3; d3.v2 = w.ident3 + a.Cmid; d3.v3 = w.ident3 + 2 * a.Cmid;
    d3.v4 = a.bn3.coef; d3.v5 = a.bn3.coef + a.Cmid; d3.gate = a.se_gate; d3.gate2 = w.dps; d3.gate_ld = a.Cmid;
    d3.rows_per_sample = S_out;
    PROF(DWN_FAM_BN3_REDUCE, k_bn3_bwd_reduce(d3, a.bn3.coef, Mout, a.Cmid, w.st3, du, dt, s));
    }
    TRY(k_bn_bwd_finalize(bwd_job(w.st3, (double)Mout, a.bn3, w.abc3, a.Cmid, frozen), BnBwdJob{}, s));
    {
        DwTemporalBwd d; memset(&d, 0, sizeof(d));
        d.dy = ld_affine2(du, a.y3, a.Cmid, w.abc3, a.Cmid);
        d.dy_kind = LD_PLAIN;
        d.y2 = ld_ycoef(a.y2, a.Cmid, a.bn2.coef, a.Cmid);
        d.w = w.wdwt; d.dh2 = a.buf_b; d.dw = a.dw_dwt; d.B = a.B; d.T = a.T; d.HW = a.Hout * a.Wout; d.C = a.Cmid;
        d.kt = a.kt; d.stats = w.st2;
        PROF(DWN_FAM_DWT_BWD, launch_dw_temporal_bwd(d, dt, s));
    }
    TRY(k_bn_bwd_finalize(bwd_job(w.st2, (double)Mout, a.bn2, w.abc2, a.Cmid, frozen), BnBwdJob{}, s));
    void* dh1 = a.buf_a;
    {
        DwSpatialBwd d; memset(&d, 0, sizeof(d));
        d.dy = ld_affine2(a.buf_b, a.y2, a.Cmid, w.abc2, a.Cmid);
        d.y1 = ld_ycoef(y1_free ? nullptr : a.y1, a.Cmid, a.bn1.coef, a.Cmid);
        if (y1_free) { d.a0 = xin.p; d.a0_ld = a.Cin; d.w1 = w.wpw; d.Cin = a.Cin; }
        d.w = w.wdws; d.dh1 = dh1; d.dw = a.dw_dws; d.planes = a.B * a.T; d.Hin = a.Hin; d.Win = a.Win;
        d.Hout = a.Hout; d.Wout = a.Wout; d.C = a.Cmid; d.stride = a.stride; d.ks = a.ks; d.stats = w.st1;
        PROF(DWN_FAM_DWS_BWD, launch_dw_spatial_bwd(d, dt, s));
    }
    TRY(k_bn_bwd_finalize(bwd_job(w.st1, (double)Min, a.bn1, w.abc1, a.Cmid, frozen), BnBwdJob{}, s));
    const bool identity_sc = a.stride == 1 && a.Hin == a.Hout && a.Win == a.Wout;
    const bool dx_folded = a.Cout % a.Cin == 0 && a.Cout / a.Cin <= 2 && dwn_pw_bwd_fused_supported(dt, Min, a.Cmid, a.Cin) &&
                           (identity_sc || (gm.hinv && gm.winv && a.Hin + a.Win <= 512));
    TRY(pw_backward(dt, dh1, xin.p, a.w_pw, w.abc1, a.Cmid, a.Cin, Min, w.bp, w.gacc, w.r3, w.tacc, dx_folded ? a.dx : a.da0, a.dw_pw,
                    dx_folded ? a.dout : nullptr, w.abcsc, a.Cout, (dx_folded && !identity_sc) ? &gm : nullptr, s, false));
    if (!dx_folded) PROF(DWN_FAM_RESID_BWD, k_residual_bwd_dx(xin, a.da0, a.dout, w.abcsc, gm, a.dx, dt, s));
    return k_block_param_tail(w.dgp, w.dhp, a.se_pmean, a.se_hidpre, a.B, a.Cmid, a.se_r, a.dse_wr, a.dse_br, a.dse_we, a.dse_be,
                              w.tacc, w.abc1, a.w_pw, a.Cmid, a.Cin, a.dw_pw, dt, s);
}

int dwn_block_forward_writes(const dwn_block_args* ap) {
    const dwn_block_args& a = *ap;
    if (a.training) return block_y1_free(a) ? 2 : 3;
    if (block_fwd_rc(a)) return 0;
    if (DWN_EVAL_CHAIN && a.dtype == DWN_BF16) {
        DwSpatialFwd f; memset(&f, 0, sizeof(f));
        f.planes = a.B * a.T; f.Hin = a.Hin; f.Win = a.Win; f.Hout = a.Hout; f.Wout = a.Wout; f.C = a.Cmid; f.stride = a.stride; f.ks = a.ks;
        f.in.ld = a.Cmid; f.a0_ld = a.Cin; f.Cin = a.Cin;
        if (dw_spatial_fwd_rc_walk_supported(f, a.dtype)) return 0;
    }
    return 1;
}

int dwn_pool_forward(const dwn_pool_args* a, int device, void* stream) {
    ENTER(device);
    if (a->C % 8) return dwn_set_error(-2, "pool: C must be a multiple of 8");
    return k_pool_fwd(a->x, a->out, a->BT, a->HW, a->C, a->dtype, (hipStream_t)stream);
}
int dwn_pool_backward(const dwn_pool_args* a, int device, void* stream) {
    ENTER(device);
    if (a->C % 8) return dwn_set_error(-2, "pool: C must be a multiple of 8");
    return k_pool_bwd(a->dout, a->dx, a->BT, a->HW, a->C, a->dtype, (hipStream_t)stream);
}

namespace {
struct CortexWs { void* wp; double *st, *stsc; float *abc, *abcsc; void *dy, *dxmain; char *zb, *ze; size_t bytes; };
CortexWs carve_cortex(const dwn_cortex_args& a, int backward, void* base, size_t cap) {
    CortexWs w; memset(&w, 0, sizeof(w));
    Carver c(base, cap);
    const size_t ts = tsize(a.dtype);
    const i64 M = (i64)a.B * a.T;
    w.wp = c.take<char>((size_t)a.C * (a.Cin / a.groups) * ts);
    c.take<char>(0);
    size_t z0 = (c.off + 255) & ~(size_t)255;
    w.st = c.take<double>(nstat(a.C));
    w.stsc = c.take<double>(nstat(backward ? a.C : a.Cin));
    size_t z1 = c.off;
    if (backward) {
        w.abc = c.take<float>(3 * (size_t)a.C);
        w.abcsc = c.take<float>(3 * (size_t)a.C);
        w.dy = c.take<char>((size_t)M * a.C * ts);
        w.dxmain = c.take<char>((size_t)M * a.Cin * ts);
    }
    w.bytes = c.off + 256;
    if (base) { w.zb = (char*)base + z0; w.ze = (char*)base + z1; }
    return w;
}
}

size_t dwn_cortex_workspace_bytes(const dwn_cortex_args* a, int backward) {
    return carve_cortex(*a, backward, nullptr, 0).bytes;
}
int dwn_cortex_forward(const dwn_cortex_args* ap, int device, void* stream) {
    ENTER(device);
    const dwn_cortex_args& a = *ap;
    hipStream_t s = (hipStream_t)stream;
    if (a.Cin % (8 * a.groups) || a.C % (8 * a.groups)) return dwn_set_error(-2, "cortex: channels per group must be multiples of 8");
    CortexWs w = carve_cortex(a, 0, a.ws, a.ws_bytes);
    if (w.bytes > a.ws_bytes) return dwn_set_error(-6, "cortex_forward: workspace too small");
    const int M = a.B * a.T, Kg = a.Cin / a.groups, Ng = a.C / a.groups, dt = a.dtype, tr = a.training != DWN_BN_EVAL;
    const bool bs = a.training == DWN_BN_TRAIN;
    {
        PrepArgs pa;
        bool ok = pa.zero(w.zb, ((size_t)(w.ze - w.zb) + 15) & ~(size_t)15);
        ok = ok && pa.packw(a.w, w.wp, 1, a.C, Kg, 0, a.C, Kg);
        if (tr && !bs) ok = ok && pa.bneval(a.bn, a.C, a.eps) && pa.bneval(a.bnsc, a.C, a.eps);
        if (!ok) return dwn_set_error(-2, "cortex_forward: workspace arena must be 16-byte aligned");
        TRY(k_prep(pa, dt, s));
    }
    GemmNN g = nn_base(ld_plain(a.x, a.Cin), LD_PLAIN, w.wp, Kg, a.y, a.C, M, Ng, Kg, a.groups);
    g.f32_split = f32_split_of(a.f32_products, !tr);
    PROF(DWN_FAM_CORTEX_FWD, launch_gemm_nn(g, dt, s));
    if (bs) {
        TRY(k_cortex_stats(a.y, a.x, M, a.Cin, a.C, w.st, w.stsc, dt, s));
        TRY(k_bn_finalize_train(fin_job(w.st, a.C, (double)M, a.bn, a.C), fin_job(w.stsc, a.Cin, (double)M, a.bnsc, a.C),
                                 a.momentum, a.eps, s));
    } else if (!tr) {
        TRY(bn_finalize(w.st, a.C, (double)M, a.bn, a.C, 0, a.momentum, a.eps, s));
// ... 125 lines not shown

int dwn_poisson_loss_forward(const float* pred, const float* target, const float* w, long long per_sample,
                             long long total, float eps, double* loss_acc, int device, void* stream) {
    ENTER(device);
    return k_poisson_fwd(pred, target, w, per_sample, total, eps, loss_acc, (hipStream_t)stream);
}
int dwn_poisson_loss_backward(const float* pred, const float* target, const float* w, const float* gscale,
                              long long per_sample, long long total, float eps, float* dpred, int device,
                              void* stream) {
    ENTER(device);
    return k_poisson_bwd(pred, target, w, gscale, per_sample, total, eps, dpred, (hipStream_t)stream);
}
int dwn_f64_to_f32(const double* src, float* dst, int n, int device, void* stream) {
    ENTER(device);
    return k_f64_to_f32(src, dst, n, (hipStream_t)stream);
}
int dwn_adamw_ema_multi(const dwn_tensor_entry* list, int ntensors, int max_blocks, double lr, double beta1,
                        double beta2, double eps, double weight_decay, long long step, double ema_decay,
                        double grad_scale, int device, void* stream) {
    ENTER(device);
    if (step < 1) return dwn_set_error(-2, "adamw: step must be >= 1");
    const double bc1 = 1.0 - pow(beta1, (double)step);
    const double bc2 = 1.0 - pow(beta2, (double)step);
    return k_adamw_ema(list, ntensors, max_blocks, (float)(1.0 - lr * weight_decay), (float)(1.0 - beta1), (float)beta2,
                       (float)(1.0 - beta2), (float)eps, (float)(lr / bc1), (float)sqrt(bc2), (float)ema_decay,
                       (float)(1.0 - ema_decay), (float)grad_scale, (hipStream_t)stream);
}
int dwn_ema_lerp_multi(const dwn_tensor_entry* list, int ntensors, int max_blocks, double decay, int device,
                       void* stream) {
    ENTER(device);
    return k_ema_lerp(list, ntensors, max_blocks, (float)decay, (float)(1.0 - decay), (hipStream_t)stream);
}

size_t dwn_grad_guard_workspace_bytes(int ntensors, int max_blocks) {
    if (ntensors < 0 || max_blocks < 1) return 0;
    const size_t nseg = ntensors == 0 ? 1 : ((size_t)ntensors + DWN_GS_SEG - 1) / DWN_GS_SEG;
    return nseg * (size_t)max_blocks * 16;
}
int dwn_grad_sumsq_multi(const dwn_guarded_entry* list, int ntensors, int max_blocks, double grad_scale, void* ws,
                         size_t ws_bytes, double* pair, int device, void* stream) {
    g_err[0] = 0;
    if (ntensors < 0) return dwn_set_error(-2, "grad_sumsq_multi: ntensors < 0");
    if (max_blocks < 1 || max_blocks > 65536) return dwn_set_error(-2, "grad_sumsq_multi: 1 <= max_blocks <= 65536");
    if (!list && ntensors > 0) return dwn_set_error(-1, "grad_sumsq_multi: null table");
    if (!ws || !pair) return dwn_set_error(-1, "grad_sumsq_multi: null pointer (ws, pair)");
    if (((size_t)ws & 15) || ((size_t)pair & 7)) return dwn_set_error(-2, "grad_sumsq_multi: ws 16-byte, pair 8-byte aligned");
    if (ws_bytes < dwn_grad_guard_workspace_bytes(ntensors, max_blocks)) return dwn_set_error(-6, "grad_sumsq_multi: workspace too small");
    ENTER(device);
    return k_grad_sumsq(list, ntensors, max_blocks, grad_scale, ws, pair, (hipStream_t)stream);
}
int dwn_step_guard_finalize(const double* pair_a, const double* pair_b, double max_norm, int skip_nonfinite,
                            const dwn_guarded_entry* list, int ntensors, dwn_step_guard* guard, int device, void* stream) {
    g_err[0] = 0;
    if (ntensors < 0) return dwn_set_error(-2, "step_guard_finalize: ntensors < 0");
    if (!guard) return dwn_set_error(-1, "step_guard_finalize: null guard");
    if (!pair_a) return dwn_set_error(-1, "step_guard_finalize: null pair_a");
    if (!list && ntensors > 0) return dwn_set_error(-1, "step_guard_finalize: null table");
    if (!(max_norm == max_norm)) return dwn_set_error(-2, "step_guard_finalize: max_norm is NaN");
    ENTER(device);
    return k_step_guard_finalize(pair_a, pair_b, max_norm, skip_nonfinite ? 1 : 0, list, ntensors, guard, (hipStream_t)stream);
}
int dwn_adamw_ema_multi_guarded(const dwn_guarded_entry* list, int ntensors, int max_blocks, double lr, double beta1,
                                double beta2, double eps, double weight_decay, double ema_decay, double grad_scale,
                                const dwn_step_guard* guard, int device, void* stream) {
    g_err[0] = 0;
    if (ntensors < 0) return dwn_set_error(-2, "adamw_ema_multi_guarded: ntensors < 0");
    if (max_blocks < 1 || max_blocks > 65535 || ntensors > 65535)
        return dwn_set_error(-2, "adamw_ema_multi_guarded: max_blocks and ntensors are grid dimensions (1 <= max_blocks, both <= 65535)");
    if (!list && ntensors > 0) return dwn_set_error(-1, "adamw_ema_multi_guarded: null table");
    if (!guard) return dwn_set_error(-1, "adamw_ema_multi_guarded: null guard");
    ENTER(device);
    return k_adamw_ema_guarded(list, ntensors, max_blocks, lr, beta1, beta2, eps, weight_decay, ema_decay, grad_scale, guard,
                               (hipStream_t)stream);
}

int dwn_pw_bwd_fused_supported(int dtype, long long M, int E, int Cin) {
    return pw_bwd_fused_supported(dtype, M, E, Cin) ? 1 : 0;
}
size_t dwn_pw_backward_workspace_bytes(int E, int Cin, int dtype) {
    return (size_t)Cin * (E + Cin) * tsize(dtype) + 256 + (pw_fold_floats(Cin) + pw_wgrad_tacc_floats(E, Cin)) * sizeof(float) + 256;
}
int dwn_pw_backward(const dwn_pw_bwd_args* a, int dtype, int device, void* stream) {
    ENTER(device);
    if (!a || !a->dh1 || !a->a0 || !a->w_pw || !a->abc || !a->da0 || !a->dw || !a->ws)
        return dwn_set_error(-1, "pw_backward: null pointer");
    if (a->E <= 0 || a->Cin <= 0 || a->E % 8 || a->Cin % 8 || a->M <= 0 || a->M > 0x7fffffffLL)
        return dwn_set_error(-2, "pw_backward: E and Cin must be positive multiples of 8, 0 < M < 2^31");
    if (a->ws_bytes < dwn_pw_backward_workspace_bytes(a->E, a->Cin, dtype)) return dwn_set_error(-6, "pw_backward: workspace too small");
    hipStream_t s = (hipStream_t)stream;
    Carver c(a->ws, a->ws_bytes);
    void* bp = c.take<char>((size_t)a->Cin * (a->E + a->Cin) * tsize(dtype));
    const size_t nz = pw_fold_floats(a->Cin) + pw_wgrad_tacc_floats(a->E, a->Cin);
    float* gacc = c.take<float>(nz);
    float* r3 = gacc + (size_t)a->Cin * a->Cin;
    float* tacc = gacc + pw_fold_floats(a->Cin);
    TRY(k_zero(gacc, nz * sizeof(float), s));
    ResGeom rg; memset(&rg, 0, sizeof(rg));
    rg.hinv = a->res_hinv; rg.winv = a->res_winv; rg.Hin = a->res_Hin; rg.Win = a->res_Win; rg.Hout = a->res_Hout; rg.Wout = a->res_Wout;
    return pw_backward(dtype, a->dh1, a->a0, a->w_pw, a->abc, a->E, a->Cin, a->M, bp, gacc, r3, tacc, a->da0, a->dw, a->res,
                       a->res_abc, a->res_C, a->res_hinv ? &rg : nullptr, s);
}

int dwn_assemble_inputs(const dwn_clip_desc* descs, int B, int T, int H0, int W0, int H, int W, float pad_fill,
                        float* x, int device, void* stream) {
    ENTER(device);
    if (!descs || !x) return dwn_set_error(-1, "assemble_inputs: null pointer");
    if (B <= 0 || T <= 0 || H0 <= 0 || W0 <= 0) return dwn_set_error(-2, "assemble_inputs: B, T, H0, W0 must be positive");
    if (H < H0 || W < W0) return dwn_set_error(-2, "assemble_inputs: output frame smaller than the video");
    return k_assemble_inputs(descs, B, T, H0, W0, H, W, pad_fill, x, (hipStream_t)stream);
}

int dwn_assemble_targets(const dwn_clip_desc* descs, int B, int T, float* const* targets, const int* n_neurons,
                         int n_mice, int max_neurons, float* mice_weights, int device, void* stream) {
    ENTER(device);
    if (!descs || !targets || !n_neurons || !mice_weights) return dwn_set_error(-1, "assemble_targets: null pointer");
    if (B <= 0 || T <= 0 || n_mice <= 0 || max_neurons <= 0)
        return dwn_set_error(-2, "assemble_targets: B, T, n_mice, max_neurons must be positive");
    if (B > 65535 || n_mice > 65535) return dwn_set_error(-2, "assemble_targets: B and n_mice are grid dimensions (<= 65535)");
    return k_assemble_targets(descs, B, T, targets, n_neurons, n_mice, max_neurons, mice_weights, (hipStream_t)stream);
}

#define ARGS(a, who) do { g_err[0] = 0; if (!(a)) return dwn_set_error(-1, who ": null arguments"); } while (0)
#define WS_CHECK(a, code, who, need, getter, align) do { \
    if ((a)->ws_bytes < (need) || ((size_t)(a)->ws & ((align) - 1))) \
        return dwn_set_error(code, who ": workspace smaller than " getter " or not " #align "-byte aligned"); } while (0)
#define WS_BYTES_OR_0(a, geometry, bytes) do { if (!(a) || geometry(a) != 0) { g_err[0] = 0; return 0; } return (bytes); } while (0)

enum { PL_PLANE = 1, PL_WINDOW = 2, PL_EMPTY_OK = 4, PL_CELL = 8, PL_CLIP = 16 };
struct PlaneArgs { int B, Cin, T, H, W, c, nc; const char* chan; int y0, x0, wh, ww, cell; };
static int plane_check(const char* who, unsigned parts, const PlaneArgs& p) {
    const char* bad = nullptr;
    const long long HW = (long long)p.H * p.W;
    if (parts & PL_PLANE) {
        if (p.B <= 0 || p.Cin <= 0 || p.T <= 0 || p.H <= 0 || p.W <= 0) bad = "B, Cin, T, H, W must be positive";
        else if (p.nc <= 0 || p.c < 0 || p.c >= p.Cin || p.nc > p.Cin - p.c) bad = p.chan;
        else if (HW > (1ll << 30) || (long long)p.B * p.Cin * p.T >= (1ll << 31)) bad = "more than 2^30 pixels per plane or 2^31 planes";
    }
    if (!bad && (parts & PL_WINDOW)) {
        if ((parts & PL_EMPTY_OK) && p.wh == 0 && p.ww == 0) {
            if (p.y0 != 0 || p.x0 != 0) bad = "window not inside the plane (an empty window must start at 0, 0)";
        } else if (p.y0 < 0 || p.x0 < 0 || p.wh <= 0 || p.ww <= 0 || p.wh > p.H - p.y0 || p.ww > p.W - p.x0) {
            bad = "window not inside the plane";
        }
    }
    if (!bad && (parts & PL_CELL) && (p.cell < 1 || p.wh % p.cell || p.ww % p.cell)) bad = "cell must be positive and divide both window sides";
    if (!bad && (parts & PL_CLIP) && (p.T * HW > (1ll << 30) || (long long)p.B * p.T * HW / 64 >= (1ll << 31))) bad = "more than 2^30 elements per clip or 2^37 in all";
    if (!bad) return 0;
    char msg[160];
    snprintf(msg, sizeof msg, "%s: %s", who, bad);
    return dwn_set_error(-2, msg);
}

static int gaze_geometry(const dwn_gaze_args* a) {
    return plane_check("gaze_shift", PL_PLANE, {a->B, a->Cin, a->T, a->H, a->W, a->video_channel, 1, "video_channel outside [0, Cin)"});
}
int dwn_gaze_shift_forward(const dwn_gaze_args* a, int device, void* stream) {
    ARGS(a, "gaze_shift_forward");
    TRY(gaze_geometry(a));
    if (!a->x || !a->shift || !a->out) return dwn_set_error(-1, "gaze_shift_forward: null pointer (x, shift, out)");
    ENTER(device);
    return k_gaze_forward(*a, (hipStream_t)stream);
}
int dwn_gaze_shift_backward(const dwn_gaze_args* a, int device, void* stream) {
    ARGS(a, "gaze_shift_backward");
    TRY(gaze_geometry(a));
    if (!a->dx && !a->dshift) return dwn_set_error(-1, "gaze_shift_backward: dx and dshift are both null");
    if (!a->shift || !a->dout) return dwn_set_error(-1, "gaze_shift_backward: null pointer (shift, dout)");
    if (a->dshift && !a->x) return dwn_set_error(-1, "gaze_shift_backward: dshift needs x");
    ENTER(device);
    return k_gaze_backward(*a, (hipStream_t)stream);
}
int dwn_plane_mean(const float* x, int B, int Cin, int T, int H, int W, int c0, int nc, float* mean, int device, void* stream) {
    g_err[0] = 0;
    if (!x || !mean) return dwn_set_error(-1, "plane_mean: null pointer (x, mean)");
    TRY(plane_check("plane_mean", PL_PLANE, {B, Cin, T, H, W, c0, nc, "channels [c0, c0 + nc) outside [0, Cin)"}));
    ENTER(device);
    return k_plane_mean(x, B, Cin, T, H, W, c0, nc, mean, (hipStream_t)stream);
}

static int corr_geometry(const dwn_corr_args* a) {
    if (a->B <= 0 || a->N <= 0 || a->T <= 0) return dwn_set_error(-2, "corr: B, N, T must be positive");
    if ((long long)a->N * a->T > (1ll << 31) - 4096) return dwn_set_error(-2, "corr: N * T must stay below 2^31 - 4096");
    if (a->w_stride < 1) return dwn_set_error(-2, "corr: w_stride must be at least 1");
// ... 379 lines not shown
```

### sensorium_amd/csrc/dwn_internal.h

```cpp
#pragma once
#include "dwn_common.h"

enum { EPI_STORE = DWN_EPI_STORE, EPI_READOUT = DWN_EPI_READOUT, EPI_DG = DWN_EPI_DG, EPI_STORE_CAT = DWN_EPI_STORE_CAT, EPI_DH3 = DWN_EPI_DH3,
       EPI_READOUT_LB = 100 };
typedef dwn_gemm_nn_args GemmNN;
typedef dwn_gemm_tn_args GemmTN;
typedef dwn_dw_spatial_fwd_args DwSpatialFwd;
typedef dwn_dw_spatial_bwd_args DwSpatialBwd;
typedef dwn_dw_temporal_fwd_args DwTemporalFwd;
typedef dwn_dw_temporal_bwd_args DwTemporalBwd;

int launch_gemm_nn(const GemmNN& g, int dtype, hipStream_t s);
int launch_gemm_tn(const GemmTN& g, int dtype, hipStream_t s);
bool gemm_nn_xl_eligible(const GemmNN& g, int dtype);
int launch_gemm_nn_xl(const GemmNN& g, hipStream_t s);
bool gemm_nn_kd_eligible(const GemmNN& g, int dtype);
int launch_gemm_nn_kd(const GemmNN& g, hipStream_t s);
int launch_dw_spatial_fwd(const DwSpatialFwd& a, int dtype, hipStream_t s);
int launch_dw_spatial_bwd(const DwSpatialBwd& a, int dtype, hipStream_t s);
int launch_dw_temporal_fwd(const DwTemporalFwd& a, int dtype, hipStream_t s);
int launch_dw_temporal_bwd(const DwTemporalBwd& a, int dtype, hipStream_t s);
int dw_temporal_wide_check(int kt, int C, int dy_kind);
int launch_dw_temporal_wide_fwd(const DwTemporalFwd& a, int dtype, hipStream_t s);
int launch_dw_temporal_wide_bwd(const DwTemporalBwd& a, int dtype, hipStream_t s);
bool pw_bwd_fused_supported(int dtype, long long M, int E, int Cin);
int launch_pw_bwd_fused(const void* dh1, const void* a0, const void* bp, const float* r3, void* da0, float* tacc,
                        long long M, int E, int Cin, int dtype, const void* res, const float* res_coef, int res_n,
                        const int* hinv, const int* winv, int Hin, int Win, int Hout, int Wout, hipStream_t s);
```

### sensorium_amd/csrc/dwn_pw_bwd.hip

```cpp
#include "dwn_gemm_nn.h"

static __device__ __forceinline__ unsigned pwb_pack2(float a, float b) { return pk_bf16(a, b); }
namespace pwb {
constexpr int CIN = 64, BM = 128;
constexpr int RS = 160;
template <int NKC> struct Cfg {
    static constexpr int E = NKC * 64, KCAT = E + CIN;
    static constexpr int WRS = KCAT * 2 + 16;
    static constexpr int SW_BYTES = CIN * WRS, SD_BYTES = BM * RS, SX_BYTES = BM * RS;
    static constexpr int MAP_INTS = 512;
    static constexpr int LDS_BYTES = SW_BYTES + 2 * SD_BYTES + 2 * SX_BYTES + 7 * CIN * 4 + MAP_INTS * 4;
};
}
struct PwbGather { const int* hinv; const int* winv; int Hin, Win, Hout, Wout; };
template <int NKC>
__global__ __launch_bounds__(512) __attribute__((amdgpu_waves_per_eu(2, 2))) void pw_bwd_fused_kernel(const bf16_t* __restrict__ dh1, const bf16_t* __restrict__ a0,
                                                       const bf16_t* __restrict__ bp, const float* __restrict__ r3,
                                                       bf16_t* __restrict__ da0, float* __restrict__ tacc, int M,
                                                       const bf16_t* __restrict__ res, const float* __restrict__ res_coef, int res_n,
                                                       const PwbGather gq) {
    using namespace pwb;
    constexpr int E = Cfg<NKC>::E, KCAT = Cfg<NKC>::KCAT, WRS = Cfg<NKC>::WRS;
    constexpr int SW_BYTES = Cfg<NKC>::SW_BYTES, SD_BYTES = Cfg<NKC>::SD_BYTES, SX_BYTES = Cfg<NKC>::SX_BYTES;
    extern __shared__ __attribute__((aligned(16))) unsigned char pwb_smem[];
    unsigned char* const smem = pwb_smem;
    unsigned char* sW = smem;
    unsigned char* sD = smem + SW_BYTES;
    unsigned char* sX = sD + 2 * SD_BYTES;
    float* sR3 = reinterpret_cast<float*>(sX + 2 * SX_BYTES);
    const int tid = threadIdx.x, wave = tid >> 6, lane = tid & 63;
    const int lr = lane & 15, lg = lane >> 4;
    const int wm = wave & 3, wn = wave >> 2;
    if (tid < CIN) sR3[tid] = r3[tid];
    const bool gather = res && gq.hinv;
    if (res) for (int i = tid; i < (gather ? 3 : 1) * res_n * CIN; i += 512) sR3[CIN + i] = res_coef[i];
    int* sMap = reinterpret_cast<int*>(sR3 + 7 * CIN);
    if (gather) for (int i = tid; i < gq.Hin + gq.Win; i += 512) sMap[i] = i < gq.Hin ? gq.hinv[i] : gq.winv[i - gq.Hin];
    const RasterIdx ridx(gather ? gq.Hin : 1, gather ? gq.Win : 1);
    for (int c = tid; c < CIN * (KCAT / 8); c += 512) {
        const int n = c / (KCAT / 8), kc8 = c % (KCAT / 8);
        *reinterpret_cast<uint4*>(sW + n * WRS + kc8 * 16) = *reinterpret_cast<const uint4*>(bp + (size_t)n * KCAT + kc8 * 8);
    }
    f32x4_t acc_dw[NKC][2], acc_ga[2], acc_s[2];
#pragma unroll
    for (int k = 0; k < NKC; ++k) { acc_dw[k][0] = f32x4_t{0, 0, 0, 0}; acc_dw[k][1] = f32x4_t{0, 0, 0, 0}; }
    acc_ga[0] = acc_ga[1] = acc_s[0] = acc_s[1] = f32x4_t{0, 0, 0, 0};
    const int ntiles = M / BM;
    const int ch = tid & 7;
    const int row_a = tid >> 3;
    struct Pair { uint4 lo, hi; };
    Pair rd[NKC], rx;
    auto fetch_a0 = [&](int tile) {
        const bf16_t* src = a0 + ((size_t)tile * BM + row_a) * CIN + ch * 8;
        return Pair{*reinterpret_cast<const uint4*>(src), *reinterpret_cast<const uint4*>(src + (size_t)64 * CIN)};
    };
    auto fetch_chunk = [&](int tile, int kc) {
        const bf16_t* src = dh1 + ((size_t)tile * BM + row_a) * E + kc * 64 + ch * 8;
        return Pair{*reinterpret_cast<const uint4*>(src), *reinterpret_cast<const uint4*>(src + (size_t)64 * E)};
    };
    int tile = blockIdx.x;
    {
        const int t0 = tile < ntiles ? tile : 0;
        rx = fetch_a0(t0);
#pragma unroll
        for (int kc = 0; kc < NKC; ++kc) rd[kc] = fetch_chunk(t0, kc);
    }
    __syncthreads();
    const int q = lr >> 2, p = lr & 3;
    const bf16x8_t ones = {(short)0x3F80, (short)0x3F80, (short)0x3F80, (short)0x3F80, (short)0x3F80, (short)0x3F80, (short)0x3F80, (short)0x3F80};
    int tpar = 0, step = 0;
    for (; tile < ntiles; tile += gridDim.x, tpar ^= 1) {
        const size_t m0 = (size_t)tile * BM;
        const int ntile = tile + (int)gridDim.x < ntiles ? tile + (int)gridDim.x : tile;
        unsigned char* sXt = sX + tpar * SX_BYTES;
        *reinterpret_cast<uint4*>(sXt + row_a * RS + ch * 16) = rx.lo;
        *reinterpret_cast<uint4*>(sXt + (row_a + 64) * RS + ch * 16) = rx.hi;
        rx = fetch_a0(ntile);
        f32x4_t acc_da[2][2];
        uint2 rres[2][2][2];
        bool rgat[2] = {true, true};
#pragma unroll
        for (int i = 0; i < 2; ++i) { acc_da[i][0] = f32x4_t{0, 0, 0, 0}; acc_da[i][1] = f32x4_t{0, 0, 0, 0}; }
#pragma unroll
        for (int kc = 0; kc < NKC; ++kc) {
            unsigned char* sDk = sD + ((step + kc) & 1) * SD_BYTES;
            *reinterpret_cast<uint4*>(sDk + row_a * RS + ch * 16) = rd[kc].lo;
            *reinterpret_cast<uint4*>(sDk + (row_a + 64) * RS + ch * 16) = rd[kc].hi;
            nn_lds_barrier();
            rd[kc] = fetch_chunk(ntile, kc);
            if (kc == NKC - 3 && res) {
#pragma unroll
                for (int i = 0; i < 2; ++i) {
                    size_t rrow = m0 + wm * 32 + i * 16 + lr;
                    if (gather) {
                        unsigned bt; int hi, wi;
                        ridx.decode((unsigned)rrow, bt, hi, wi);
                        const int ho = sMap[hi], wo = sMap[gq.Hin + wi];
                        rgat[i] = ho >= 0 && wo >= 0;
                        rrow = rgat[i] ? ((size_t)bt * gq.Hout + ho) * gq.Wout + wo : 0;
                    }
#pragma unroll
                    for (int j = 0; j < 2; ++j) {
                        const bf16_t* rp_ = res + rrow * (size_t)(res_n * CIN) + wn * 32 + j * 16 + 4 * lg;
                        rres[i][j][0] = *reinterpret_cast<const uint2*>(rp_);
                        rres[i][j][1] = *reinterpret_cast<const uint2*>(rp_ + (res_n > 1 ? CIN : 0));
                    }
                }
            }
#pragma unroll
            for (int kb = 0; kb < 2; ++kb) {
                bf16x8_t af[2], wf[2];
#pragma unroll
                for (int i = 0; i < 2; ++i)
                    af[i] = *reinterpret_cast<const bf16x8_t*>(sDk + (wm * 32 + i * 16 + lr) * RS + (kb * 4 + lg) * 16);
#pragma unroll
                for (int j = 0; j < 2; ++j)
                    wf[j] = *reinterpret_cast<const bf16x8_t*>(sW + (wn * 32 + j * 16 + lr) * WRS + (kc * 64 + kb * 32 + lg * 8) * 2);
#pragma unroll
                for (int i = 0; i < 2; ++i)
#pragma unroll
                    for (int j = 0; j < 2; ++j)
                        acc_da[i][j] = __builtin_amdgcn_mfma_f32_16x16x32_bf16(wf[j], af[i], acc_da[i][j], 0, 0, 0);
            }
#pragma unroll
            for (int kb = 0; kb < BM / 32; ++kb) {
                const int rb = kb * 32 + 8 * lg + q;
                bf16x8_t ef, cf[2];
                {
                    const int colb = (wm * 16 + 4 * p) * 2;
                    auto lo = __builtin_amdgcn_ds_read_tr16_b64_v4i16((__attribute__((address_space(3))) s16x4_t*)(sDk + rb * RS + colb));
                    auto hi = __builtin_amdgcn_ds_read_tr16_b64_v4i16((__attribute__((address_space(3))) s16x4_t*)(sDk + (rb + 4) * RS + colb));
                    ef = bf16x8_t{lo[0], lo[1], lo[2], lo[3], hi[0], hi[1], hi[2], hi[3]};
                }
#pragma unroll
                for (int j = 0; j < 2; ++j) {
                    const int colb = (wn * 32 + j * 16 + 4 * p) * 2;
                    auto lo = __builtin_amdgcn_ds_read_tr16_b64_v4i16((__attribute__((address_space(3))) s16x4_t*)(sXt + rb * RS + colb));
                    auto hi = __builtin_amdgcn_ds_read_tr16_b64_v4i16((__attribute__((address_space(3))) s16x4_t*)(sXt + (rb + 4) * RS + colb));
                    cf[j] = bf16x8_t{lo[0], lo[1], lo[2], lo[3], hi[0], hi[1], hi[2], hi[3]};
                }
#pragma unroll
                for (int j = 0; j < 2; ++j)
                    acc_dw[kc][j] = __builtin_amdgcn_mfma_f32_16x16x32_bf16(ef, cf[j], acc_dw[kc][j], 0, 0, 0);
            }
            if (kc == 0) {
#pragma unroll
                for (int kb = 0; kb < 2; ++kb) {
                    bf16x8_t af[2], wf[2];
#pragma unroll
                    for (int i = 0; i < 2; ++i)
                        af[i] = *reinterpret_cast<const bf16x8_t*>(sXt + (wm * 32 + i * 16 + lr) * RS + (kb * 4 + lg) * 16);
#pragma unroll
                    for (int j = 0; j < 2; ++j)
                        wf[j] = *reinterpret_cast<const bf16x8_t*>(sW + (wn * 32 + j * 16 + lr) * WRS + (E + kb * 32 + lg * 8) * 2);
#pragma unroll
                    for (int i = 0; i < 2; ++i)
#pragma unroll
                        for (int j = 0; j < 2; ++j)
                            acc_da[i][j] = __builtin_amdgcn_mfma_f32_16x16x32_bf16(wf[j], af[i], acc_da[i][j], 0, 0, 0);
                }
#pragma unroll
                for (int kb = 0; kb < BM / 32; ++kb) {
                    const int rb = kb * 32 + 8 * lg + q;
                    bf16x8_t ef, cf[2];
                    {
                        const int colb = (wm * 16 + 4 * p) * 2;
                        auto lo = __builtin_amdgcn_ds_read_tr16_b64_v4i16((__attribute__((address_space(3))) s16x4_t*)(sXt + rb * RS + colb));
                        auto hi = __builtin_amdgcn_ds_read_tr16_b64_v4i16((__attribute__((address_space(3))) s16x4_t*)(sXt + (rb + 4) * RS + colb));
                        ef = bf16x8_t{lo[0], lo[1], lo[2], lo[3], hi[0], hi[1], hi[2], hi[3]};
                    }
#pragma unroll
                    for (int j = 0; j < 2; ++j) {
                        const int colb = (wn * 32 + j * 16 + 4 * p) * 2;
                        auto lo = __builtin_amdgcn_ds_read_tr16_b64_v4i16((__attribute__((address_space(3))) s16x4_t*)(sXt + rb * RS + colb));
                        auto hi = __builtin_amdgcn_ds_read_tr16_b64_v4i16((__attribute__((address_space(3))) s16x4_t*)(sXt + (rb + 4) * RS + colb));
                        cf[j] = bf16x8_t{lo[0], lo[1], lo[2], lo[3], hi[0], hi[1], hi[2], hi[3]};
                    }
#pragma unroll
                    for (int j = 0; j < 2; ++j) {
                        acc_ga[j] = __builtin_amdgcn_mfma_f32_16x16x32_bf16(ef, cf[j], acc_ga[j], 0, 0, 0);
                        if (wm == 0) acc_s[j] = __builtin_amdgcn_mfma_f32_16x16x32_bf16(ones, cf[j], acc_s[j], 0, 0, 0);
                    }
                }
            }
        }
        step += NKC;
#pragma unroll
        for (int i = 0; i < 2; ++i)
#pragma unroll
            for (int j = 0; j < 2; ++j) {
                const size_t m = m0 + wm * 32 + i * 16 + lr;
                const int n = wn * 32 + j * 16 + 4 * lg;
                const float4 b4 = *reinterpret_cast<const float4*>(sR3 + n);
                float o[4] = {acc_da[i][j][0] + b4.x, acc_da[i][j][1] + b4.y, acc_da[i][j][2] + b4.z, acc_da[i][j][3] + b4.w};
                if (res) {
                    const int rc = res_n * CIN;
                    float x4[4] = {0.f, 0.f, 0.f, 0.f};
                    if (gather) {
                        const uint2 xv = *reinterpret_cast<const uint2*>(sXt + (wm * 32 + i * 16 + lr) * RS + n * 2);
                        x4[0] = __uint_as_float(xv.x << 16); x4[1] = __uint_as_float(xv.x & 0xffff0000u);
                        x4[2] = __uint_as_float(xv.y << 16); x4[3] = __uint_as_float(xv.y & 0xffff0000u);
                    }
#pragma unroll
                    for (int jj = 0; jj < 2; ++jj) {
                        if (jj >= res_n || !rgat[i]) break;
                        const uint2 rv = rres[i][j][jj];
                        const float4 c4 = *reinterpret_cast<const float4*>(sR3 + CIN + jj * CIN + n);
                        float t[4] = {c4.x * __uint_as_float(rv.x << 16), c4.y * __uint_as_float(rv.x & 0xffff0000u),
                                      c4.z * __uint_as_float(rv.y << 16), c4.w * __uint_as_float(rv.y & 0xffff0000u)};
                        if (gather) {
                            const float4 a2 = *reinterpret_cast<const float4*>(sR3 + CIN + rc + jj * CIN + n);
                            const float4 a3 = *reinterpret_cast<const float4*>(sR3 + CIN + 2 * rc + jj * CIN + n);
                            t[0] += fmaf(a2.x, x4[0], a3.x); t[1] += fmaf(a2.y, x4[1], a3.y);
                            t[2] += fmaf(a2.z, x4[2], a3.z); t[3] += fmaf(a2.w, x4[3], a3.w);
                        }
                        o[0] += t[0]; o[1] += t[1]; o[2] += t[2]; o[3] += t[3];
                    }
                }
                uint2 v = make_uint2(pwb_pack2(o[0], o[1]), pwb_pack2(o[2], o[3]));
                *reinterpret_cast<uint2*>(da0 + m * CIN + n) = v;
            }
    }
    DET_ENTER();
#pragma unroll
    for (int kc = 0; kc < NKC; ++kc)
#pragma unroll
        for (int j = 0; j < 2; ++j)
#pragma unroll
            for (int r = 0; r < 4; ++r)
                atomicAdd(tacc + (size_t)(kc * 64 + wm * 16 + 4 * lg + r) * CIN + wn * 32 + j * 16 + lr, acc_dw[kc][j][r]);
#pragma unroll
    for (int j = 0; j < 2; ++j) {
#pragma unroll
        for (int r = 0; r < 4; ++r)
            atomicAdd(tacc + (size_t)(E + wm * 16 + 4 * lg + r) * CIN + wn * 32 + j * 16 + lr, acc_ga[j][r]);
        if (wm == 0 && lg == 0) atomicAdd(tacc + (size_t)KCAT * CIN + wn * 32 + j * 16 + lr, acc_s[j][0]);
    }
    DET_EXIT();
}


bool pw_bwd_fused_supported(int dtype, long long M, int E, int Cin) {
    return dtype == DWN_BF16 && (E == 448 || E == 384) && Cin == pwb::CIN && M > 0 && M % pwb::BM == 0 && M <= 0x7fffffffLL;
}
template <int NKC>
static int launch_pw_bwd_fused_t(const void* dh1, const void* a0, const void* bp, const float* r3, void* da0, float* tacc,
                                 long long M, const void* res, const float* res_coef, int res_n, const PwbGather& gq, hipStream_t s) {
    auto kern = pw_bwd_fused_kernel<NKC>;
    {
        hipError_t e = lds_opt_in(kern, pwb::Cfg<NKC>::LDS_BYTES);
        if (e != hipSuccess) return dwn_set_error((int)e, hipGetErrorString(e));
    }
    int grid = 256;
    if (grid > (int)(M / pwb::BM)) grid = (int)(M / pwb::BM);
    hipLaunchKernelGGL(kern, dim3(grid), dim3(512), pwb::Cfg<NKC>::LDS_BYTES, s, (const bf16_t*)dh1, (const bf16_t*)a0,
                       (const bf16_t*)bp, r3, (bf16_t*)da0, tacc, (int)M, (const bf16_t*)res, res_coef, res_n, gq);
    DWN_CHECK_LAUNCH();
    return 0;
}
int launch_pw_bwd_fused(const void* dh1, const void* a0, const void* bp, const float* r3, void* da0, float* tacc,
                        long long M, int E, int Cin, int dtype, const void* res, const float* res_coef, int res_n,
                        const int* hinv, const int* winv, int Hin, int Win, int Hout, int Wout, hipStream_t s) {
    PwbGather gq; gq.hinv = hinv; gq.winv = winv; gq.Hin = Hin; gq.Win = Win; gq.Hout = Hout; gq.Wout = Wout;
    if (res && hinv && (!winv || Hin <= 0 || Win <= 0 || Hout <= 0 || Wout <= 0 || M % ((long long)Hin * Win) || Hin + Win > 512))
        return dwn_set_error(-2, "pw_bwd_fused: the gathered shortcut form needs both inverse maps, M = frames * Hin * Win and Hin + Win <= 512");
    if (!pw_bwd_fused_supported(dtype, M, E, Cin))
        return dwn_set_error(-3, "pw_bwd_fused: built for bf16, Cin = 64, E = 448 or 384, M % 128 == 0 only");
    if (res && (!res_coef || res_n < 1 || res_n > 2)) return dwn_set_error(-3, "pw_bwd_fused: the residual term needs res_coef and res_n in {1, 2}");
    return E == 448 ? launch_pw_bwd_fused_t<7>(dh1, a0, bp, r3, da0, tacc, M, res, res_coef, res_n, gq, s)
                    : launch_pw_bwd_fused_t<6>(dh1, a0, bp, r3, da0, tacc, M, res, res_coef, res_n, gq, s);
}
```

### sensorium_amd/dwiseneuro.py

```python
from __future__ import annotations

import math
from typing import Optional, Sequence

import torch
from torch import nn

from . import ops


def _select_dtype(explicit: Optional[torch.dtype]) -> torch.dtype:
    if explicit is not None:
        return explicit
    if torch.is_autocast_enabled():
        return torch.bfloat16
    return torch.float32


class BatchNormAct(nn.Module):

    def __init__(self, num_features: int, bn_layer=nn.BatchNorm3d, apply_act: bool = True):
        super().__init__()
        self.bn = bn_layer(num_features)
        self.apply_act = apply_act
# ... 175 lines not shown
        self.param = param
        if param == "beta":
            self.beta = nn.Parameter(torch.tensor(float(softplus_beta), dtype=torch.float32))
        else:
            self.log_beta = nn.Parameter(torch.tensor(math.log(float(softplus_beta)), dtype=torch.float32))

    def value(self) -> torch.Tensor:
        return self.beta if self.param == "beta" else self.log_beta.float().exp()

    def extra_repr(self) -> str:
        return f"param={self.param!r}"


class Readout(nn.Module):

    def __init__(self, in_features: int, out_features: int, groups: int = 1, softplus_beta: float = 1.0,
                 drop_rate: float = 0.0, learnable_softplus: bool = False, softplus_param: str = "beta"):
        super().__init__()
        if softplus_param not in ("beta", "log"):
            raise ValueError("softplus_param: 'beta' or 'log'")
        self.learnable_softplus = bool(learnable_softplus)
        self.in_features = in_features
        self.out_features = out_features
        self.groups = groups
        self.softplus_beta = float(softplus_beta)
        self.drop_rate = float(drop_rate)
        padded = int(math.ceil(out_features / groups) * groups)
        self.layer = nn.Sequential(nn.Dropout1d(p=drop_rate),
                                   nn.Conv1d(in_features, padded, (1,), groups=groups, bias=True))
        self.gate = SoftplusGate(softplus_beta, softplus_param) if self.learnable_softplus else nn.Softplus(beta=softplus_beta)

    def beta(self) -> torch.Tensor:
        if self.learnable_softplus:
            return self.gate.value().detach()
        return torch.tensor(self.softplus_beta, dtype=torch.float32, device=self.layer[1].weight.device)

    def forward(self, x: torch.Tensor) -> torch.Tensor:
        mask = None
        if self.training and self.drop_rate > 0.0:
            keep = 1.0 - self.drop_rate
            mask = torch.empty(x.shape[0], x.shape[2], dtype=torch.float32, device=x.device).bernoulli_(keep)
            mask.div_(keep)
        conv = self.layer[1]
        if self.learnable_softplus:
            return ops.ReadoutFn.apply(x, mask, self, conv.weight, conv.bias, self.gate.value())
        return ops.ReadoutFn.apply(x, mask, self, conv.weight, conv.bias)


class DepthwiseCore(nn.Module):

    def __init__(self, in_channels: int = 1, features: Sequence[int] = (64, 128, 256, 512),
                 spatial_strides: Sequence[int] = (2, 2, 2, 2), spatial_kernel: int = 3, temporal_kernel: int = 3,
                 expansion_ratio: int = 3, se_reduce_ratio: int = 16, drop_path_rate: float = 0.0):
        super().__init__()
        num_blocks = len(features)
        assert num_blocks and num_blocks == len(spatial_strides)
        self.stem = nn.Sequential(nn.Conv3d(in_channels, features[0], (1, 1, 1), bias=False),
                                  BatchNormAct(features[0], apply_act=False))
        blocks = []
        nxt = features[0]
        for i in range(num_blocks):
            if i < num_blocks - 1:
                nxt = features[i + 1]
            blocks += [
                PositionalEncoding3d(features[i]),
                InvertedResidual3d(features[i], nxt, spatial_kernel=spatial_kernel, temporal_kernel=temporal_kernel,
                                   spatial_stride=spatial_strides[i], expansion_ratio=expansion_ratio,
                                   se_reduce_ratio=se_reduce_ratio,
                                   drop_path_rate=drop_path_rate * i / num_blocks, bias=False),
            ]
        self.blocks = nn.Sequential(*blocks)

    def forward(self, x: torch.Tensor, dtype: torch.dtype) -> torch.Tensor:
        bn = self.stem[1].bn
        mods = list(self.blocks)
        pes, blks = mods[0::2], mods[1::2]
        _, _, t, h, w = x.shape
        sizes = []
        for blk in blks:
            sizes.append((h, w))
            s = blk.spatial_stride
            h, w = (h - 1) // s + 1, (w - 1) // s + 1
        tables = [blk.geometry(pe, t, hw[0], hw[1], x.device)[:3] for pe, blk, hw in zip(pes, blks, sizes)]
        x = ops.StemFn.apply(x, self.stem[0].weight, bn.weight, bn.bias, self, dtype, tables[0], ops.bn_mode(bn.training, x))
        for i, (pe, blk) in enumerate(zip(pes, blks)):
            x = blk(x, pe, dtype, True, tables[i + 1] if i + 1 < len(blks) else None)
        return x


class DwiseNeuro(nn.Module):

    def __init__(self,
                 readout_outputs: Sequence[int],
                 in_channels: int = 5,
                 core_features: Sequence[int] = (64, 64, 64, 64, 128, 128, 128, 256, 256),
                 spatial_strides: Sequence[int] = (2, 1, 1, 1, 2, 1, 1, 2, 1),
                 spatial_kernel: int = 3,
                 temporal_kernel: int = 5,
                 expansion_ratio: int = 6,
                 se_reduce_ratio: int = 32,
                 cortex_features: Sequence[int] = (1024, 2048, 4096),
                 groups: int = 2,
                 softplus_beta: float = 0.07,
                 drop_rate: float = 0.4,
                 drop_path_rate: float = 0.1,
                 compute_dtype: Optional[torch.dtype] = None,
                 learnable_softplus: bool = False,
                 softplus_param: str = "beta"):
        super().__init__()
        self.compute_dtype = compute_dtype
        self.fp32_eval_products = "bf16x3"
        self.bn_frozen_finetune = False
        self.core = DepthwiseCore(in_channels=in_channels, features=core_features, spatial_strides=spatial_strides,
                                  spatial_kernel=spatial_kernel, temporal_kernel=temporal_kernel,
                                  expansion_ratio=expansion_ratio, se_reduce_ratio=se_reduce_ratio,
                                  drop_path_rate=drop_path_rate)
        self.pool = nn.AdaptiveAvgPool3d((None, 1, 1))
        self.cortex = Cortex(in_features=core_features[-1], features=cortex_features, groups=groups,
                             drop_path_rate=drop_path_rate)
        self.readouts = nn.ModuleList()
        for n in readout_outputs:
            self.readouts.append(Readout(in_features=cortex_features[-1], out_features=n, groups=groups,
                                         softplus_beta=softplus_beta, drop_rate=drop_rate,
                                         learnable_softplus=learnable_softplus, softplus_param=softplus_param))

    def softplus_parameters(self):
        return [p for r in self.readouts if r.learnable_softplus for p in r.gate.parameters()]

    def set_fp32_eval_products(self, mode: str = "bf16x3") -> "DwiseNeuro":
        if mode not in ("bf16x3", "native"):
            raise ValueError("fp32 eval products: 'bf16x3' or 'native'")
        self.fp32_eval_products = mode
        for m in self.modules():
            if isinstance(m, (InvertedResidual3d, ShuffleLayer, Readout)):
                m._dwn_fp32_native = mode == "native"
        return self

    def freeze_batchnorm(self, flag: bool = True) -> "DwiseNeuro":
        self.bn_frozen_finetune = bool(flag)
        return self

    def _draw_drop_paths(self, batch: int, device) -> None:
        layers = [m for m in self.modules() if isinstance(m, DropPath) and m.drop_prob > 0.0 and m.training]
        if not layers:
            return
        key = (tuple(m.drop_prob for m in layers), batch)
        cache = getattr(self, "_dp_keep", None)
        if cache is None or cache[0] != key or cache[1].device != device:
            keep = torch.tensor([1.0 - q for q in key[0]], dtype=torch.float32)
            inv = torch.where(keep > 0, 1.0 / keep.clamp_min(1e-30), torch.zeros_like(keep))
            cache = (key, keep.unsqueeze(1).expand(len(layers), batch).contiguous().to(device), inv.unsqueeze(1).to(device))
            self._dp_keep = cache
        factors = torch.bernoulli(cache[1]).mul_(cache[2])
        for m, row in zip(layers, factors.unbind(0)):
            m._pooled = row

    def trunk(self, x: torch.Tensor, mode_from: Optional[torch.Tensor] = None) -> torch.Tensor:
        return self._trunk(x, mode_from, False)

    def trunk_with_map(self, x: torch.Tensor, mode_from: Optional[torch.Tensor] = None):
        return self._trunk(x, mode_from, True)

    def _trunk(self, x: torch.Tensor, mode_from: Optional[torch.Tensor], return_map: bool):
        if x.dim() != 5:
            raise RuntimeError("DwiseNeuro expects (batch, channel, time, height, width)")
        if self.training:
            self._draw_drop_paths(x.shape[0], x.device)
        dtype = _select_dtype(self.compute_dtype)
# ... 15 lines not shown
```

### sensorium_amd/ops.py

```python
from __future__ import annotations

import ctypes as C
import math
import os
import threading
from typing import Optional

import numpy as np
import torch
from torch.autograd.function import once_differentiable

from . import _lib as L

_DT = {torch.float32: L.DWN_F32, torch.bfloat16: L.DWN_BF16}


def _ptr(t: Optional[torch.Tensor]):
    return None if t is None else t.data_ptr()


def _stream(device: torch.device):
    return torch.cuda.current_stream(device).cuda_stream


def _require_gpu(t: torch.Tensor, what: str):
    if not t.is_cuda:
        raise RuntimeError(f"sensorium_amd.{what}: tensors must be on a GPU (got {t.device}); "
                           "the HIP path has no CPU fallback")


def _bn_struct(bn: torch.nn.modules.batchnorm._BatchNorm, coef: torch.Tensor, dgamma=None, dbeta=None) -> L.BN:
    s = L.BN()
    s.gamma = bn.weight.data_ptr()
    s.beta = bn.bias.data_ptr()
    s.running_mean = bn.running_mean.data_ptr()
    s.running_var = bn.running_var.data_ptr()
    s.num_batches_tracked = bn.num_batches_tracked.data_ptr()
    s.coef = coef.data_ptr()
    s.dgamma = _ptr(dgamma)
    s.dbeta = _ptr(dbeta)
    return s


def _check_bn(bn):
    if bn.momentum is None or not bn.affine or not bn.track_running_stats:
        raise RuntimeError("sensorium_amd: BatchNorm must be affine with running stats and a fixed momentum")


def _f32_products(mod, inference_readout: bool = False) -> int:
    native = getattr(mod, "_dwn_fp32_native", False)
    if inference_readout:
        return L.F32_NATIVE if native else L.F32_SPLIT3
    return L.F32_NATIVE if native else L.F32_AUTO


_EVAL_BACKWARD_ERROR = "sensorium_amd: backward through eval-mode BatchNorm is not built"


class _BnModeState(threading.local):
    override: Optional[int] = None


_BN_MODE = _BnModeState()


class bn_mode_scope:

    def __init__(self, mode: Optional[int]):
        self.mode = mode

    def __enter__(self):
        self.prev, _BN_MODE.override = _BN_MODE.override, self.mode
        return self

    def __exit__(self, *exc):
        _BN_MODE.override = self.prev
        return False


def wants_frozen(x: torch.Tensor, switch: bool = False) -> bool:
    return torch.is_grad_enabled() and (bool(x.requires_grad) or switch)


def bn_mode(training: bool, x: torch.Tensor) -> int:
    if training:
        return L.BN_TRAIN
    if _BN_MODE.override is not None:
        return _BN_MODE.override
    return L.BN_FROZEN if wants_frozen(x) else L.BN_EVAL


def _ddp_flush() -> None:
    from . import ddp
    if ddp._LIVE:
        ddp.flush_ready_all()


def _ws(nbytes: int, device) -> torch.Tensor:
    return torch.empty(int(nbytes), dtype=torch.uint8, device=device)


def _env_choice(name: str, table: dict) -> int:
    v = os.environ.get(name, "")
    if v not in table:
        raise ValueError(f"{name}={v!r}: expected one of {sorted(k for k in table if k)} (or unset)")
    return table[v]


_PWL_BWD = _env_choice("DWN_PWL_BWD", {"": 0, "new": 1, "old": 2})
_Y1_MODE = _env_choice("DWN_Y1", {"": 0, "free": 0, "materialise": 1, "all": 2})


def grad_out(param: torch.Tensor, zero: bool = False) -> torch.Tensor:
    slot = getattr(param, "_dwn_grad_slot", None)
    if slot is not None and param.grad is None and not getattr(param, "_dwn_slot_out", False):
        param._dwn_slot_out = True
        flat, off = slot
        g = flat[off:off + param.numel()].view(param.shape)
        return g.zero_() if zero else g
    if zero:
        return torch.zeros_like(param, dtype=torch.float32)
    return torch.empty_like(param, dtype=torch.float32)


def nearest_src_index(out_size: int, in_size: int) -> np.ndarray:
    scale = np.float32(in_size) / np.float32(out_size)
    src = np.floor(np.arange(out_size, dtype=np.float32) * scale).astype(np.int64)
    return np.minimum(src, in_size - 1).astype(np.int32)


def inverse_index(src: np.ndarray, in_size: int) -> np.ndarray:
    inv = np.full(in_size, -1, dtype=np.int32)
    inv[src] = np.arange(len(src), dtype=np.int32)
    if len(np.unique(src)) != len(src):
        raise RuntimeError("nearest-neighbour shortcut map is not injective (stride < 1?)")
    return inv


def pe_axis_tables(channels: int, inv_freq: torch.Tensor, t: int, h: int, w: int):
    ch = int(math.ceil(channels / 6) * 2)
    if ch % 2:
        ch += 1
    inv = inv_freq.detach().float().cpu()
    tabs = []
    for axis, size in enumerate((t, h, w)):
        arg = inv[:, None] * torch.arange(size).float()[None, :]
        emb = torch.cat([arg.sin(), arg.cos()], dim=0)
        tab = torch.zeros(size, channels, dtype=torch.float32)
        lo = axis * ch
        n = max(0, min(ch, channels - lo))
        if n > 0:
            tab[:, lo:lo + n] = emb[:n].t()
        tabs.append(tab.contiguous())
    return tabs


class StemFn(torch.autograd.Function):

    @staticmethod
    def forward(ctx, x, weight, gamma, beta, mod, dtype, pe=None, mode=None):
        _require_gpu(x, "StemFn")
        conv, bn = mod.stem[0], mod.stem[1].bn
        _check_bn(bn)
        if mode is None:
            mode = int(bn.training)
        x = x.contiguous().float()
        B, Cin, T, H, W = x.shape
        C0 = weight.shape[0]
        dev = x.device
        out = torch.empty(B, T, H, W, C0, dtype=dtype, device=dev)
        coef = torch.empty(4 * C0, dtype=torch.float32, device=dev)
        xmom = torch.empty(72, dtype=torch.float64, device=dev)
# ... 57 lines not shown
    B, T, Hin, Win, Cin = x.shape
    a = L.BlockArgs()
    a.dtype = _DT[dtype]; a.training = int(training)
    a.B = B; a.T = T; a.Hin = Hin; a.Win = Win
    a.Hout = (Hin - 1) // blk.spatial_stride + 1
    a.Wout = (Win - 1) // blk.spatial_stride + 1
    a.Cin = Cin; a.Cmid = blk.mid_features; a.Cout = blk.out_features
    a.stride = blk.spatial_stride; a.ks = blk.spatial_kernel; a.kt = blk.temporal_kernel
    a.se_r = blk.se.conv_reduce.out_channels
    bn1 = blk.conv_pw[1].bn
    a.eps = bn1.eps; a.momentum = bn1.momentum
    a.x = x.data_ptr()
    a.x_has_pe = int(x_has_pe)
    a.a0 = _ptr(a0)
    pe_t, pe_h, pe_w, hsrc, wsrc, hinv, winv = geom
    a.pe_t = pe_t.data_ptr(); a.pe_h = pe_h.data_ptr(); a.pe_w = pe_w.data_ptr()
    a.hsrc = hsrc.data_ptr(); a.wsrc = wsrc.data_ptr(); a.hinv = hinv.data_ptr(); a.winv = winv.data_ptr()
    a.w_pw = blk.conv_pw[0].weight.data_ptr()
    a.w_dws = blk.spat_covn_dw[0].weight.data_ptr()
    a.w_dwt = blk.temp_covn_dw[0].weight.data_ptr()
    a.w_pwl = blk.conv_pwl[0].weight.data_ptr()
    a.se_wr = blk.se.conv_reduce.weight.data_ptr(); a.se_br = blk.se.conv_reduce.bias.data_ptr()
    a.se_we = blk.se.conv_expand.weight.data_ptr(); a.se_be = blk.se.conv_expand.bias.data_ptr()
    a.drop_scale = _ptr(drop_scale)
    a.se_pmean = saved["pmean"].data_ptr(); a.se_hidpre = saved["hidpre"].data_ptr()
    a.se_gate = saved["gate"].data_ptr()
    a.f32_products = _f32_products(blk)
    a.y1_mode = getattr(blk, "_dwn_y1_mode", _Y1_MODE)
    return a


class BlockFn(torch.autograd.Function):

    @staticmethod
    def forward(ctx, x, drop_scale, blk, geom, dtype, x_has_pe, out_pe, mode, *params):
        _require_gpu(x, "BlockFn")
        x = x.contiguous()
        dev = x.device
        B, T, Hin, Win, Cin = x.shape
        s = blk.spatial_stride
        Hout, Wout = (Hin - 1) // s + 1, (Win - 1) // s + 1
        Cmid, Cout = blk.mid_features, blk.out_features
        bns = blk.bn_modules()
        for bn in bns:
            _check_bn(bn)
        training = mode
        f32 = dict(dtype=torch.float32, device=dev)
        y2 = torch.empty(B, T, Hout, Wout, Cmid, dtype=dtype, device=dev)
        z3 = torch.empty_like(y2)
        a0 = None if x_has_pe else torch.empty_like(x)
        y4 = torch.empty(B, T, Hout, Wout, Cout, dtype=dtype, device=dev)
        out = torch.empty_like(y4)
        coefs = [torch.empty(4 * c, **f32) for c in (Cmid, Cmid, Cmid, Cout, Cout)]
        R = blk.se.conv_reduce.out_channels
        saved = dict(pmean=torch.empty(B, Cmid, **f32), hidpre=torch.empty(B, R, **f32),
                     gate=torch.empty(B, Cmid, **f32))
        a = _block_args(blk, geom, x, dtype, training, coefs, saved, drop_scale, x_has_pe, a0)
        a.out = out.data_ptr()
        writes = L.lib.dwn_block_forward_writes(C.byref(a))
        y1 = torch.empty(B, T, Hin, Win, Cmid, dtype=dtype, device=dev) if writes & 1 else None
        y3 = torch.empty_like(y2) if writes & 2 else None
        a.y1 = _ptr(y1); a.y2 = y2.data_ptr(); a.y3 = _ptr(y3); a.y4 = y4.data_ptr()
        a.z3 = z3.data_ptr()
        if out_pe is not None:
            a.out_pe_t, a.out_pe_h, a.out_pe_w = (t.data_ptr() for t in out_pe)
        a.bn1, a.bn2, a.bn3, a.bn4, a.bnsc = (_bn_struct(bn, cf) for bn, cf in zip(bns, coefs))
        ws = _ws(L.lib.dwn_block_workspace_bytes(C.byref(a), 0), dev)
        a.ws = ws.data_ptr(); a.ws_bytes = ws.numel()
        L.check(L.lib.dwn_block_forward(C.byref(a), dev.index, _stream(dev)), "dwn_block_forward")
        ctx.blk = blk; ctx.geom = geom; ctx.dtype = dtype; ctx.mode = mode
        if getattr(blk, "_capture", False):
            blk._captured = dict(y1=y1, y2=y2, y3=y3, y4=y4, z3=z3, coefs=coefs, **saved)
        ctx.has_drop = drop_scale is not None
        if mode == L.BN_EVAL:
            return out
        tensors = [x if x_has_pe else a0, y1, y2, y3, y4, *coefs, saved["pmean"], saved["hidpre"], saved["gate"], z3]
        if drop_scale is not None:
            tensors.append(drop_scale)
        ctx.save_for_backward(*tensors)
        return out

    @staticmethod
    def backward(ctx, dout):
        if ctx.mode == L.BN_EVAL:
            raise RuntimeError(_EVAL_BACKWARD_ERROR)
        blk, dtype = ctx.blk, ctx.dtype
        t = ctx.saved_tensors
        x, y1, y2, y3, y4 = t[:5]
        coefs = list(t[5:10])
        saved = dict(pmean=t[10], hidpre=t[11], gate=t[12])
        z3 = t[13]
        drop_scale = t[14] if ctx.has_drop else None
        dev = x.device
        dout = dout.contiguous()
        B, T, Hin, Win, Cin = x.shape
        Hout, Wout = y2.shape[2], y2.shape[3]
        Cmid, Cout = blk.mid_features, blk.out_features
        f32 = dict(dtype=torch.float32, device=dev)
        a = _block_args(blk, ctx.geom, x, dtype, ctx.mode, coefs, saved, drop_scale, True, None)
        a.y1 = _ptr(y1); a.y2 = y2.data_ptr(); a.y3 = y3.data_ptr(); a.y4 = y4.data_ptr()
        a.z3 = z3.data_ptr()
        bns = blk.bn_modules()
        dg = [grad_out(bn.weight) for bn in bns]
        db = [grad_out(bn.bias) for bn in bns]
        a.bn1, a.bn2, a.bn3, a.bn4, a.bnsc = (_bn_struct(bn, cf, g_, b_) for bn, cf, g_, b_ in zip(bns, coefs, dg, db))
        m_in, m_out = B * T * Hin * Win, B * T * Hout * Wout
        buf_a = torch.empty(max(m_in, m_out) * Cmid, dtype=dtype, device=dev)
        buf_b = torch.empty(m_out * Cmid, dtype=dtype, device=dev)
        dy4 = torch.empty(m_out * Cout, dtype=dtype, device=dev)
        da0 = torch.empty(m_in * Cin, dtype=dtype, device=dev)
        dx = torch.empty_like(x)
        R = blk.se.conv_reduce.out_channels
        dw_pw = grad_out(blk.conv_pw[0].weight)
        dw_dws = grad_out(blk.spat_covn_dw[0].weight)
        dw_dwt = grad_out(blk.temp_covn_dw[0].weight)
        dw_pwl = grad_out(blk.conv_pwl[0].weight)
        dse_wr = grad_out(blk.se.conv_reduce.weight); dse_br = grad_out(blk.se.conv_reduce.bias)
        dse_we = grad_out(blk.se.conv_expand.weight); dse_be = grad_out(blk.se.conv_expand.bias)
        a.dout = dout.data_ptr(); a.dx = dx.data_ptr()
        a.buf_a = buf_a.data_ptr(); a.buf_b = buf_b.data_ptr(); a.dy4 = dy4.data_ptr(); a.da0 = da0.data_ptr()
        a.dw_pw = dw_pw.data_ptr(); a.dw_dws = dw_dws.data_ptr(); a.dw_dwt = dw_dwt.data_ptr()
        a.dw_pwl = dw_pwl.data_ptr()
        a.dse_wr = dse_wr.data_ptr(); a.dse_br = dse_br.data_ptr(); a.dse_we = dse_we.data_ptr()
        a.dse_be = dse_be.data_ptr()
        a.pwl_bwd = _PWL_BWD
        ws = _ws(L.lib.dwn_block_workspace_bytes(C.byref(a), 1), dev)
        a.ws = ws.data_ptr(); a.ws_bytes = ws.numel()
        L.check(L.lib.dwn_block_backward(C.byref(a), dev.index, _stream(dev)), "dwn_block_backward")
        _ddp_flush()
        grads = (dw_pw, dg[0], db[0], dw_dws, dg[1], db[1], dw_dwt, dg[2], db[2], dse_wr, dse_br, dse_we, dse_be,
                 dw_pwl, dg[3], db[3], dg[4], db[4])
        return (dx, None, None, None, None, None, None, None) + grads


class PoolFn(torch.autograd.Function):

    @staticmethod
    def forward(ctx, x):
        _require_gpu(x, "PoolFn")
        x = x.contiguous()
        B, T, H, W, Cc = x.shape
        out = torch.empty(B, T, Cc, dtype=x.dtype, device=x.device)
        a = L.PoolArgs()
        a.dtype = _DT[x.dtype]; a.BT = B * T; a.HW = H * W; a.C = Cc; a.x = x.data_ptr(); a.out = out.data_ptr()
        L.check(L.lib.dwn_pool_forward(C.byref(a), x.device.index, _stream(x.device)), "dwn_pool_forward")
        ctx.shape = (B, T, H, W, Cc)
        return out

    @staticmethod
    def backward(ctx, dout):
        B, T, H, W, Cc = ctx.shape
        dout = dout.contiguous()
        dx = torch.empty(B, T, H, W, Cc, dtype=dout.dtype, device=dout.device)
        a = L.PoolArgs()
        a.dtype = _DT[dout.dtype]; a.BT = B * T; a.HW = H * W; a.C = Cc; a.dout = dout.data_ptr(); a.dx = dx.data_ptr()
        L.check(L.lib.dwn_pool_backward(C.byref(a), dout.device.index, _stream(dout.device)), "dwn_pool_backward")
        return dx


class CortexFn(torch.autograd.Function):

    @staticmethod
    def forward(ctx, x, drop_scale, layer, dtype, mode, weight, g, b, gsc, bsc):
        _require_gpu(x, "CortexFn")
        x = x.contiguous()
        dev = x.device
        B, T, Cin = x.shape
        Cc = layer.out_features
        bn, bnsc = layer.bn.bn, layer.bn_sc.bn
        _check_bn(bn); _check_bn(bnsc)
        y = torch.empty(B, T, Cc, dtype=dtype, device=dev)
        out = torch.empty_like(y)
        coef = torch.empty(4 * Cc, dtype=torch.float32, device=dev)
        coefsc = torch.empty(4 * Cc, dtype=torch.float32, device=dev)
        a = L.CortexArgs()
        a.dtype = _DT[dtype]; a.training = mode; a.B = B; a.T = T; a.Cin = Cin; a.C = Cc
        a.groups = layer.groups; a.eps = bn.eps; a.momentum = bn.momentum
        a.x = x.data_ptr(); a.out = out.data_ptr(); a.y = y.data_ptr(); a.w = weight.data_ptr()
        a.bn = _bn_struct(bn, coef); a.bnsc = _bn_struct(bnsc, coefsc); a.drop_scale = _ptr(drop_scale)
        a.f32_products = _f32_products(layer)
        ws = _ws(L.lib.dwn_cortex_workspace_bytes(C.byref(a), 0), dev)
        a.ws = ws.data_ptr(); a.ws_bytes = ws.numel()
        L.check(L.lib.dwn_cortex_forward(C.byref(a), dev.index, _stream(dev)), "dwn_cortex_forward")
        ctx.layer = layer; ctx.dtype = dtype; ctx.mode = mode; ctx.has_drop = drop_scale is not None
        tensors = [x, y, coef, coefsc, weight]
        if drop_scale is not None:
            tensors.append(drop_scale)
        ctx.save_for_backward(*tensors)
        return out

    @staticmethod
    def backward(ctx, dout):
        if ctx.mode == L.BN_EVAL:
            raise RuntimeError(_EVAL_BACKWARD_ERROR)
        layer, dtype = ctx.layer, ctx.dtype
        t = ctx.saved_tensors
        x, y, coef, coefsc, weight = t[:5]
        drop_scale = t[5] if ctx.has_drop else None
        dev = x.device
        dout = dout.contiguous()
        B, T, Cin = x.shape
        Cc = layer.out_features
        bn, bnsc = layer.bn.bn, layer.bn_sc.bn
        f32 = dict(dtype=torch.float32, device=dev)
        dgm, dbm, dgs, dbs = grad_out(bn.weight), grad_out(bn.bias), grad_out(bnsc.weight), grad_out(bnsc.bias)
        dw = grad_out(layer.conv.weight)
        dx = torch.empty_like(x)
        a = L.CortexArgs()
        a.dtype = _DT[dtype]; a.training = ctx.mode; a.B = B; a.T = T; a.Cin = Cin; a.C = Cc
        a.groups = layer.groups; a.eps = bn.eps; a.momentum = bn.momentum
        a.x = x.data_ptr(); a.y = y.data_ptr(); a.w = weight.data_ptr()
        a.bn = _bn_struct(bn, coef, dgm, dbm); a.bnsc = _bn_struct(bnsc, coefsc, dgs, dbs)
        a.drop_scale = _ptr(drop_scale)
        a.dout = dout.data_ptr(); a.dx = dx.data_ptr(); a.dw = dw.data_ptr()
        ws = _ws(L.lib.dwn_cortex_workspace_bytes(C.byref(a), 1), dev)
# ... 911 lines not shown
```

Baseline: 1483.

## Fuse stem backward accumulation into first block's conv_pw backward kernel

Adds a 'stem sink' path. The first block's one-pass conv_pw backward kernel accumulates the stem conv/BN weight-gradient statistics directly from the stem input, so the block's input gradient (the stem output gradient) is never written to memory and the separate stem backward pass over it is dropped. A new StemBlock0Fn autograd function runs stem and block 0 forward together and calls a new stem finalize entry point. This saves a large bf16 activation-gradient write and read plus a kernel launch. In exchange the kernel does extra per-tile work and double-precision atomics, and the path only applies under restricted shapes and modes.

Measured after the change: 1488, median of 6. Within noise of the previous version (+0.3%).

```diff
diff --git a/include/dwn.h b/include/dwn.h
--- a/include/dwn.h
+++ b/include/dwn.h
@@ -191,6 +191,7 @@
     int pwl_bwd;
     int f32_products;
     int y1_mode;
+    const float* stem_x; const double* stem_xmom; double* stem_acc; int stem_Cin;
 } dwn_block_args;
 
 typedef struct dwn_pool_args {
@@ -304,6 +305,8 @@
 int dwn_stem_backward(const dwn_stem_args* a, int device, void* stream);
 int dwn_stem_input_grad(const dwn_stem_input_grad_args* a, int device, void* stream);
 int dwn_stem_backward_input(const dwn_stem_args* a, float* dx, int device, void* stream);
+
+int dwn_stem_backward_finalize(const dwn_stem_args* a, const double* acc, int device, void* stream);
 size_t dwn_block_workspace_bytes(const dwn_block_args* a, int backward);
 int dwn_block_forward(const dwn_block_args* a, int device, void* stream);
 int dwn_block_backward(const dwn_block_args* a, int device, void* stream);
@@ -348,6 +351,7 @@
     void* ws; size_t ws_bytes;
     const void* res; const float* res_abc; int res_C;
     const int* res_hinv; const int* res_winv; int res_Hin, res_Win, res_Hout, res_Wout;
+    const float* stem_x; const double* stem_xmom; double* stem_acc; int stem_Cin; long long stem_S;
 } dwn_pw_bwd_args;
 int dwn_pw_bwd_fused_supported(int dtype, long long M, int E, int Cin);
 size_t dwn_pw_backward_workspace_bytes(int E, int Cin, int dtype);
diff --git a/sensorium_amd/_lib.py b/sensorium_amd/_lib.py
--- a/sensorium_amd/_lib.py
+++ b/sensorium_amd/_lib.py
@@ -113,7 +113,8 @@
                 ("dout", c_p), ("dx", c_p), ("buf_a", c_p), ("buf_b", c_p), ("dy4", c_p), ("da0", c_p),
                 ("dw_pw", c_p), ("dw_dws", c_p), ("dw_dwt", c_p), ("dw_pwl", c_p), ("dse_wr", c_p),
                 ("dse_br", c_p), ("dse_we", c_p), ("dse_be", c_p),
-                ("ws", c_p), ("ws_bytes", c_sz), ("pwl_bwd", c_i), ("f32_products", c_i), ("y1_mode", c_i)]
+                ("ws", c_p), ("ws_bytes", c_sz), ("pwl_bwd", c_i), ("f32_products", c_i), ("y1_mode", c_i),
+                ("stem_x", c_p), ("stem_xmom", c_p), ("stem_acc", c_p), ("stem_Cin", c_i)]
 
 
 class PoolArgs(C.Structure):
@@ -164,7 +165,7 @@
     _fields_ = [("dh1", c_p), ("a0", c_p), ("w_pw", c_p), ("abc", c_p), ("da0", c_p), ("dw", c_p),
                 ("M", c_ll), ("E", c_i), ("Cin", c_i), ("ws", c_p), ("ws_bytes", c_sz), ("res", c_p), ("res_abc", c_p),
                 ("res_C", c_i), ("res_hinv", c_p), ("res_winv", c_p), ("res_Hin", c_i), ("res_Win", c_i), ("res_Hout", c_i),
-                ("res_Wout", c_i)]
+                ("res_Wout", c_i), ("stem_x", c_p), ("stem_xmom", c_p), ("stem_acc", c_p), ("stem_Cin", c_i), ("stem_S", c_ll)]
 
 
 class DwSpatialRcFwdArgs(C.Structure):
@@ -343,6 +344,7 @@
     "dwn_stem_backward": (c_i, [_P(StemArgs), c_i, c_p]),
     "dwn_stem_input_grad": _new(c_i, [_P(StemInputGradArgs), c_i, c_p]),
     "dwn_stem_backward_input": _new(c_i, [_P(StemArgs), c_p, c_i, c_p]),
+    "dwn_stem_backward_finalize": _new(c_i, [_P(StemArgs), c_p, c_i, c_p]),
     "dwn_block_workspace_bytes": (c_sz, [_P(BlockArgs), c_i]),
     "dwn_block_forward": (c_i, [_P(BlockArgs), c_i, c_p]),
     "dwn_block_backward": (c_i, [_P(BlockArgs), c_i, c_p]),
@@ -426,7 +428,7 @@
 HASH_SRCS = ("dwn_api.hip", "dwn_gemm.hip", "dwn_gemm_nn_1.hip", "dwn_gemm_nn_2.hip", "dwn_gemm_nn_3.hip", "dwn_gemm_nn_4.hip", "dwn_gemm_nn_5.hip",
              "dwn_gemm_nn_6.hip", "dwn_gemm_tn.hip", "dwn_gram.hip", "dwn_pw_bwd.hip", "dwn_gemm_xl.hip", "dwn_gemm_kd.hip", "dwn_dwconv.hip", "dwn_dwrc.hip",
              "dwn_dwbwd.hip", "dwn_dwfwd.hip", "dwn_elementwise.hip", "dwn_data.hip", "dwn_gaze.hip", "dwn_modulator.hip", "dwn_spatial.hip", "dwn_mei.hip", "dwn_rf_fit.hip", "dwn_pairwise.hip", "dwn_trial_score.hip", "dwn_rf.hip", "dwn_corr.hip", "dwn_stim.hip", "dwn_common.h", "dwn_internal.h",
-             "dwn_kernels.h", "dwn_launch.h", "dwn_gemm_nn.h", "dwn_gain.h", "dwn_reduce.h",
+             "dwn_kernels.h", "dwn_launch.h", "dwn_gemm_nn.h", "dwn_gain.h", "dwn_reduce.h", "dwn_pw_bwd_kernel.inc",
              "../../include/dwn.h")
 
 
diff --git a/sensorium_amd/csrc/dwn_api.hip b/sensorium_amd/csrc/dwn_api.hip
--- a/sensorium_amd/csrc/dwn_api.hip
+++ b/sensorium_amd/csrc/dwn_api.hip
@@ -440,6 +440,19 @@
     TRY(k_zero(acc, (size_t)DWN_NREP * a->C0 * stem_acc_stride() * sizeof(double), s));
     TRY(k_stem_bwd_acc(a->dout, a->x, a->xmom, (double)M, a->B, a->Cin, a->S, a->C0, acc, a->dtype, s));
     return k_stem_bwd_finalize(acc, a->xmom, a->w, a->bn.coef, (double)M, a->bn.dgamma, a->bn.dbeta, a->dw, a->C0, a->Cin, s);
+}
+
+int dwn_stem_backward_finalize(const dwn_stem_args* a, const double* acc, int device, void* stream) {
+    g_err[0] = 0;
+    if (!a || !acc) return dwn_set_error(-1, "stem_backward_finalize: null pointer (args, acc)");
+    if (a->training != DWN_BN_TRAIN)
+        return dwn_set_error(-7, "stem_backward_finalize: built for batch statistics (DWN_BN_TRAIN) only");
+    if (!a->w || !a->bn.coef || !a->dw || !a->xmom) return dwn_set_error(-1, "stem_backward_finalize: null pointer (w, bn.coef, dw, xmom)");
+    if (a->C0 <= 0 || a->C0 % 8 || a->Cin <= 0 || a->Cin > 8 || a->B <= 0 || a->S <= 0)
+        return dwn_set_error(-2, "stem_backward_finalize: C0 must be a positive multiple of 8; B, S positive; 1 <= Cin <= 8");
+    ENTER(device);
+    return k_stem_bwd_finalize(acc, a->xmom, a->w, a->bn.coef, (double)((i64)a->B * a->S), a->bn.dgamma, a->bn.dbeta, a->dw, a->C0,
+                               a->Cin, (hipStream_t)stream);
 }
 
 int dwn_stem_backward_input(const dwn_stem_args* a, float* dx, int device, void* stream) {
@@ -624,17 +637,33 @@
     return 0;
 }
 
+struct PwSink { const float* x; const double* xmom; double* acc; int Cin; i64 S; };
+static int pw_sink_check(const PwSink& k, bool folded, i64 M) {
+    if (!k.x || !k.xmom || !k.acc) return dwn_set_error(-1, "stem sink: stem_x, stem_xmom and stem_acc must all be set");
+    if (!folded)
+        return dwn_set_error(-3, "stem sink: only where the one-pass conv_pw backward folds the shortcut term in (dwn_pw_bwd_fused_supported, "
+                                 "Cout in {Cin, 2 Cin}): the block's input gradient is then never stored");
+    if (k.Cin < 1 || k.Cin > 5 || k.S <= 0 || M % k.S) return dwn_set_error(-3, "stem sink: 1..5 stem input channels, M = samples * S");
+    if ((size_t)k.acc & 15) return dwn_set_error(-2, "stem sink: stem_acc must be 16-byte aligned");
+    return 0;
+}
 static int pw_backward(int dt, const void* dh1, const void* a0, const float* w_pw, const float* abc, int E, int Cin, i64 M,
                        void* bp, float* gacc, float* r3, float* tacc, void* da0, float* dw, const void* res,
-                       const float* res_abc, int res_C, const ResGeom* rg, hipStream_t s, bool fold = true) {
+                       const float* res_abc, int res_C, const ResGeom* rg, hipStream_t s, bool fold = true, const PwSink* sink = nullptr) {
     const int res_n = res ? res_C / Cin : 0;
     const bool gathered = res && rg && rg->hinv;
+    if (sink) TRY(pw_sink_check(*sink, res && pw_bwd_fused_supported(dt, M, E, Cin), M));
     if (res && (!res_abc || res_C % Cin || res_n < 1 || res_n > 2))
         return dwn_set_error(-2, "pw_backward: the shortcut term needs res_abc and res_C in {Cin, 2 Cin}");
     if (res && !pw_bwd_fused_supported(dt, M, E, Cin))
         return dwn_set_error(-3, "pw_backward: the shortcut term is built into the one-pass kernel only (dwn_pw_bwd_fused_supported)");
     TRY(k_pw_bwd_prep(w_pw, abc, E, Cin, bp, gacc, r3, dt, (res && !gathered) ? res_abc : nullptr, res_C, s));
-    if (pw_bwd_fused_supported(dt, M, E, Cin)) {
+    if (sink) {
+        PROF(DWN_FAM_PW_DGRAD, launch_pw_bwd_sink(dh1, a0, bp, r3, tacc, M, E, Cin, dt, res, res_abc, res_n,
+                                                  gathered ? rg->hinv : nullptr, gathered ? rg->winv : nullptr, gathered ? rg->Hin : 0,
+                                                  gathered ? rg->Win : 0, gathered ? rg->Hout : 0, gathered ? rg->Wout : 0,
+                                                  sink->x, sink->xmom, sink->acc, sink->Cin, sink->S, s));
+    } else if (pw_bwd_fused_supported(dt, M, E, Cin)) {
         PROF(DWN_FAM_PW_DGRAD, launch_pw_bwd_fused(dh1, a0, bp, r3, da0, tacc, M, E, Cin, dt, res, res_abc, res_n,
                                                    gathered ? rg->hinv : nullptr, gathered ? rg->winv : nullptr, gathered ? rg->Hin : 0,
                                                    gathered ? rg->Win : 0, gathered ? rg->Hout : 0, gathered ? rg->Wout : 0, s));
@@ -655,6 +684,13 @@
     return k_pw_wgrad_fold(tacc, abc, w_pw, E, Cin, dw, dt, s);
 }
 
+static bool block_dx_folded(const dwn_block_args& a) {
+    const i64 Min = (i64)a.B * a.T * a.Hin * a.Win;
+    const bool identity_sc = a.stride == 1 && a.Hin == a.Hout && a.Win == a.Wout;
+    return a.Cout % a.Cin == 0 && a.Cout / a.Cin <= 2 && dwn_pw_bwd_fused_supported(a.dtype, Min, a.Cmid, a.Cin) &&
+           (identity_sc || (a.hinv && a.winv && a.Hin + a.Win <= 512));
+}
+
 int dwn_block_backward(const dwn_block_args* ap, int device, void* stream) {
     const dwn_block_args& a = *ap;
     hipStream_t s = (hipStream_t)stream;
@@ -662,12 +698,15 @@
     TRY(check_block(a));
     if (a.training == DWN_BN_EVAL)
         return dwn_set_error(-7, "block_backward: only training-mode (batch-statistics) and frozen-statistics backward are built");
+    const int dt = a.dtype;
+    const i64 Min = (i64)a.B * a.T * a.Hin * a.Win, Mout = (i64)a.B * a.T * a.Hout * a.Wout;
+    const bool has_sink = a.stem_x || a.stem_xmom || a.stem_acc;
+    const PwSink sink = {a.stem_x, a.stem_xmom, a.stem_acc, a.stem_Cin, (i64)a.T * a.Hin * a.Win};
+    if (has_sink) TRY(pw_sink_check(sink, block_dx_folded(a), Min));
     ENTER(device);
     const bool frozen = a.training == DWN_BN_FROZEN;
     BlockWs w = carve_block(a, 1, a.ws, a.ws_bytes);
     if (w.bytes > a.ws_bytes) return dwn_set_error(-6, "block_backward: workspace too small");
-    const int dt = a.dtype;
-    const i64 Min = (i64)a.B * a.T * a.Hin * a.Win, Mout = (i64)a.B * a.T * a.Hout * a.Wout;
     const int S_out = a.T * a.Hout * a.Wout;
     float* dg = reinterpret_cast<float*>(w.pooled);
     const bool y1_free = block_y1_free(a);
@@ -686,6 +725,7 @@
         if (w.pb) ok = ok && pa.zero(w.pb, (size_t)a.B * a.Cout * a.Cmid * sizeof(float));
         ok = ok && pa.zero(w.gacc, pw_fold_floats(a.Cin) * sizeof(float));
         ok = ok && pa.zero(w.tacc, pw_wgrad_tacc_floats(a.Cmid, a.Cin) * sizeof(float));
+        if (has_sink) ok = ok && pa.zero(a.stem_acc, (size_t)DWN_NREP * a.Cin * stem_acc_stride() * sizeof(double));
         if (!ok) return dwn_set_error(-2, "block_backward: workspace arena and dw_* buffers must be 16-byte aligned");
         TRY(k_prep(pa, dt, s));
     }
@@ -756,10 +796,10 @@
     }
     TRY(k_bn_bwd_finalize(bwd_job(w.st1, (double)Min, a.bn1, w.abc1, a.Cmid, frozen), BnBwdJob{}, s));
     const bool identity_sc = a.stride == 1 && a.Hin == a.Hout && a.Win == a.Wout;
-    const bool dx_folded = a.Cout % a.Cin == 0 && a.Cout / a.Cin <= 2 && dwn_pw_bwd_fused_supported(dt, Min, a.Cmid, a.Cin) &&
-                           (identity_sc || (gm.hinv && gm.winv && a.Hin + a.Win <= 512));
+    const bool dx_folded = block_dx_folded(a);
     TRY(pw_backward(dt, dh1, xin.p, a.w_pw, w.abc1, a.Cmid, a.Cin, Min, w.bp, w.gacc, w.r3, w.tacc, dx_folded ? a.dx : a.da0, a.dw_pw,
-                    dx_folded ? a.dout : nullptr, w.abcsc, a.Cout, (dx_folded && !identity_sc) ? &gm : nullptr, s, false));
+                    dx_folded ? a.dout : nullptr, w.abcsc, a.Cout, (dx_folded && !identity_sc) ? &gm : nullptr, s, false,
+                    has_sink ? &sink : nullptr));
     if (!dx_folded) PROF(DWN_FAM_RESID_BWD, k_residual_bwd_dx(xin, a.da0, a.dout, w.abcsc, gm, a.dx, dt, s));
     return k_block_param_tail(w.dgp, w.dhp, a.se_pmean, a.se_hidpre, a.B, a.Cmid, a.se_r, a.dse_wr, a.dse_br, a.dse_we, a.dse_be,
                               w.tacc, w.abc1, a.w_pw, a.Cmid, a.Cin, a.dw_pw, dt, s);
@@ -1051,7 +1091,8 @@
 }
 int dwn_pw_backward(const dwn_pw_bwd_args* a, int dtype, int device, void* stream) {
     ENTER(device);
-    if (!a || !a->dh1 || !a->a0 || !a->w_pw || !a->abc || !a->da0 || !a->dw || !a->ws)
+    const bool has_sink = a && (a->stem_x || a->stem_xmom || a->stem_acc);
+    if (!a || !a->dh1 || !a->a0 || !a->w_pw || !a->abc || (!a->da0 && !has_sink) || !a->dw || !a->ws)
         return dwn_set_error(-1, "pw_backward: null pointer");
     if (a->E <= 0 || a->Cin <= 0 || a->E % 8 || a->Cin % 8 || a->M <= 0 || a->M > 0x7fffffffLL)
         return dwn_set_error(-2, "pw_backward: E and Cin must be positive multiples of 8, 0 < M < 2^31");
@@ -1066,8 +1107,13 @@
     TRY(k_zero(gacc, nz * sizeof(float), s));
     ResGeom rg; memset(&rg, 0, sizeof(rg));
     rg.hinv = a->res_hinv; rg.winv = a->res_winv; rg.Hin = a->res_Hin; rg.Win = a->res_Win; rg.Hout = a->res_Hout; rg.Wout = a->res_Wout;
+    const PwSink sink = {a->stem_x, a->stem_xmom, a->stem_acc, a->stem_Cin, a->stem_S};
+    if (has_sink) {
+        TRY(pw_sink_check(sink, a->res && pw_bwd_fused_supported(dtype, a->M, a->E, a->Cin), a->M));
+        TRY(k_zero(a->stem_acc, (size_t)DWN_NREP * a->Cin * stem_acc_stride() * sizeof(double), s));
+    }
     return pw_backward(dtype, a->dh1, a->a0, a->w_pw, a->abc, a->E, a->Cin, a->M, bp, gacc, r3, tacc, a->da0, a->dw, a->res,
-                       a->res_abc, a->res_C, a->res_hinv ? &rg : nullptr, s);
+                       a->res_abc, a->res_C, a->res_hinv ? &rg : nullptr, s, true, has_sink ? &sink : nullptr);
 }
 
 int dwn_assemble_inputs(const dwn_clip_desc* descs, int B, int T, int H0, int W0, int H, int W, float pad_fill,
diff --git a/sensorium_amd/csrc/dwn_internal.h b/sensorium_amd/csrc/dwn_internal.h
--- a/sensorium_amd/csrc/dwn_internal.h
+++ b/sensorium_amd/csrc/dwn_internal.h
@@ -27,3 +27,7 @@
 int launch_pw_bwd_fused(const void* dh1, const void* a0, const void* bp, const float* r3, void* da0, float* tacc,
                         long long M, int E, int Cin, int dtype, const void* res, const float* res_coef, int res_n,
                         const int* hinv, const int* winv, int Hin, int Win, int Hout, int Wout, hipStream_t s);
+int launch_pw_bwd_sink(const void* dh1, const void* a0, const void* bp, const float* r3, float* tacc, long long M, int E, int Cin,
+                       int dtype, const void* res, const float* res_coef, int res_n, const int* hinv, const int* winv, int Hin,
+                       int Win, int Hout, int Wout, const float* stem_x, const double* stem_xmom, double* stem_acc, int stem_Cin,
+                       long long stem_S, hipStream_t s);
diff --git a/sensorium_amd/csrc/dwn_pw_bwd.hip b/sensorium_amd/csrc/dwn_pw_bwd.hip
--- a/sensorium_amd/csrc/dwn_pw_bwd.hip
+++ b/sensorium_amd/csrc/dwn_pw_bwd.hip
@@ -13,231 +13,18 @@
 };
 }
 struct PwbGather { const int* hinv; const int* winv; int Hin, Win, Hout, Wout; };
-template <int NKC>
-__global__ __launch_bounds__(512) __attribute__((amdgpu_waves_per_eu(2, 2))) void pw_bwd_fused_kernel(const bf16_t* __restrict__ dh1, const bf16_t* __restrict__ a0,
-                                                       const bf16_t* __restrict__ bp, const float* __restrict__ r3,
-                                                       bf16_t* __restrict__ da0, float* __restrict__ tacc, int M,
-                                                       const bf16_t* __restrict__ res, const float* __restrict__ res_coef, int res_n,
-                                                       const PwbGather gq) {
-    using namespace pwb;
-    constexpr int E = Cfg<NKC>::E, KCAT = Cfg<NKC>::KCAT, WRS = Cfg<NKC>::WRS;
-    constexpr int SW_BYTES = Cfg<NKC>::SW_BYTES, SD_BYTES = Cfg<NKC>::SD_BYTES, SX_BYTES = Cfg<NKC>::SX_BYTES;
-    extern __shared__ __attribute__((aligned(16))) unsigned char pwb_smem[];
-    unsigned char* const smem = pwb_smem;
-    unsigned char* sW = smem;
-    unsigned char* sD = smem + SW_BYTES;
-    unsigned char* sX = sD + 2 * SD_BYTES;
-    float* sR3 = reinterpret_cast<float*>(sX + 2 * SX_BYTES);
-    const int tid = threadIdx.x, wave = tid >> 6, lane = tid & 63;
-    const int lr = lane & 15, lg = lane >> 4;
-    const int wm = wave & 3, wn = wave >> 2;
-    if (tid < CIN) sR3[tid] = r3[tid];
-    const bool gather = res && gq.hinv;
-    if (res) for (int i = tid; i < (gather ? 3 : 1) * res_n * CIN; i += 512) sR3[CIN + i] = res_coef[i];
-    int* sMap = reinterpret_cast<int*>(sR3 + 7 * CIN);
-    if (gather) for (int i = tid; i < gq.Hin + gq.Win; i += 512) sMap[i] = i < gq.Hin ? gq.hinv[i] : gq.winv[i - gq.Hin];
-    const RasterIdx ridx(gather ? gq.Hin : 1, gather ? gq.Win : 1);
-    for (int c = tid; c < CIN * (KCAT / 8); c += 512) {
-        const int n = c / (KCAT / 8), kc8 = c % (KCAT / 8);
-        *reinterpret_cast<uint4*>(sW + n * WRS + kc8 * 16) = *reinterpret_cast<const uint4*>(bp + (size_t)n * KCAT + kc8 * 8);
-    }
-    f32x4_t acc_dw[NKC][2], acc_ga[2], acc_s[2];
-#pragma unroll
-    for (int k = 0; k < NKC; ++k) { acc_dw[k][0] = f32x4_t{0, 0, 0, 0}; acc_dw[k][1] = f32x4_t{0, 0, 0, 0}; }
-    acc_ga[0] = acc_ga[1] = acc_s[0] = acc_s[1] = f32x4_t{0, 0, 0, 0};
-    const int ntiles = M / BM;
-    const int ch = tid & 7;
-    const int row_a = tid >> 3;
-    struct Pair { uint4 lo, hi; };
-    Pair rd[NKC], rx;
-    auto fetch_a0 = [&](int tile) {
-        const bf16_t* src = a0 + ((size_t)tile * BM + row_a) * CIN + ch * 8;
-        return Pair{*reinterpret_cast<const uint4*>(src), *reinterpret_cast<const uint4*>(src + (size_t)64 * CIN)};
-    };
-    auto fetch_chunk = [&](int tile, int kc) {
-        const bf16_t* src = dh1 + ((size_t)tile * BM + row_a) * E + kc * 64 + ch * 8;
-        return Pair{*reinterpret_cast<const uint4*>(src), *reinterpret_cast<const uint4*>(src + (size_t)64 * E)};
-    };
-    int tile = blockIdx.x;
-    {
-        const int t0 = tile < ntiles ? tile : 0;
-        rx = fetch_a0(t0);
-#pragma unroll
-        for (int kc = 0; kc < NKC; ++kc) rd[kc] = fetch_chunk(t0, kc);
-    }
-    __syncthreads();
-    const int q = lr >> 2, p = lr & 3;
-    const bf16x8_t ones = {(short)0x3F80, (short)0x3F80, (short)0x3F80, (short)0x3F80, (short)0x3F80, (short)0x3F80, (short)0x3F80, (short)0x3F80};
-    int tpar = 0, step = 0;
-    for (; tile < ntiles; tile += gridDim.x, tpar ^= 1) {
-        const size_t m0 = (size_t)tile * BM;
-        const int ntile = tile + (int)gridDim.x < ntiles ? tile + (int)gridDim.x : tile;
-        unsigned char* sXt = sX + tpar * SX_BYTES;
-        *reinterpret_cast<uint4*>(sXt + row_a * RS + ch * 16) = rx.lo;
-        *reinterpret_cast<uint4*>(sXt + (row_a + 64) * RS + ch * 16) = rx.hi;
-        rx = fetch_a0(ntile);
-        f32x4_t acc_da[2][2];
-        uint2 rres[2][2][2];
-        bool rgat[2] = {true, true};
-#pragma unroll
-        for (int i = 0; i < 2; ++i) { acc_da[i][0] = f32x4_t{0, 0, 0, 0}; acc_da[i][1] = f32x4_t{0, 0, 0, 0}; }
-#pragma unroll
-        for (int kc = 0; kc < NKC; ++kc) {
-            unsigned char* sDk = sD + ((step + kc) & 1) * SD_BYTES;
-            *reinterpret_cast<uint4*>(sDk + row_a * RS + ch * 16) = rd[kc].lo;
-            *reinterpret_cast<uint4*>(sDk + (row_a + 64) * RS + ch * 16) = rd[kc].hi;
-            nn_lds_barrier();
-            rd[kc] = fetch_chunk(ntile, kc);
-            if (kc == NKC - 3 && res) {
-#pragma unroll
-                for (int i = 0; i < 2; ++i) {
-                    size_t rrow = m0 + wm * 32 + i * 16 + lr;
-                    if (gather) {
-                        unsigned bt; int hi, wi;
-                        ridx.decode((unsigned)rrow, bt, hi, wi);
-                        const int ho = sMap[hi], wo = sMap[gq.Hin + wi];
-                        rgat[i] = ho >= 0 && wo >= 0;
-                        rrow = rgat[i] ? ((size_t)bt * gq.Hout + ho) * gq.Wout + wo : 0;
-                    }
-#pragma unroll
-                    for (int j = 0; j < 2; ++j) {
-                        const bf16_t* rp_ = res + rrow * (size_t)(res_n * CIN) + wn * 32 + j * 16 + 4 * lg;
-                        rres[i][j][0] = *reinterpret_cast<const uint2*>(rp_);
-                        rres[i][j][1] = *reinterpret_cast<const uint2*>(rp_ + (res_n > 1 ? CIN : 0));
-                    }
-                }
-            }
-#pragma unroll
-            for (int kb = 0; kb < 2; ++kb) {
-                bf16x8_t af[2], wf[2];
-#pragma unroll
-                for (int i = 0; i < 2; ++i)
-                    af[i] = *reinterpret_cast<const bf16x8_t*>(sDk + (wm * 32 + i * 16 + lr) * RS + (kb * 4 + lg) * 16);
-#pragma unroll
-                for (int j = 0; j < 2; ++j)
-                    wf[j] = *reinterpret_cast<const bf16x8_t*>(sW + (wn * 32 + j * 16 + lr) * WRS + (kc * 64 + kb * 32 + lg * 8) * 2);
-#pragma unroll
-                for (int i = 0; i < 2; ++i)
-#pragma unroll
-                    for (int j = 0; j < 2; ++j)
-                        acc_da[i][j] = __builtin_amdgcn_mfma_f32_16x16x32_bf16(wf[j], af[i], acc_da[i][j], 0, 0, 0);
-            }
-#pragma unroll
-            for (int kb = 0; kb < BM / 32; ++kb) {
-                const int rb = kb * 32 + 8 * lg + q;
-                bf16x8_t ef, cf[2];
-                {
-                    const int colb = (wm * 16 + 4 * p) * 2;
-                    auto lo = __builtin_amdgcn_ds_read_tr16_b64_v4i16((__attribute__((address_space(3))) s16x4_t*)(sDk + rb * RS + colb));
-                    auto hi = __builtin_amdgcn_ds_read_tr16_b64_v4i16((__attribute__((address_space(3))) s16x4_t*)(sDk + (rb + 4) * RS + colb));
-                    ef = bf16x8_t{lo[0], lo[1], lo[2], lo[3], hi[0], hi[1], hi[2], hi[3]};
-                }
-#pragma unroll
-                for (int j = 0; j < 2; ++j) {
-                    const int colb = (wn * 32 + j * 16 + 4 * p) * 2;
-                    auto lo = __builtin_amdgcn_ds_read_tr16_b64_v4i16((__attribute__((address_space(3))) s16x4_t*)(sXt + rb * RS + colb));
-                    auto hi = __builtin_amdgcn_ds_read_tr16_b64_v4i16((__attribute__((address_space(3))) s16x4_t*)(sXt + (rb + 4) * RS + colb));
-                    cf[j] = bf16x8_t{lo[0], lo[1], lo[2], lo[3], hi[0], hi[1], hi[2], hi[3]};
-                }
-#pragma unroll
-                for (int j = 0; j < 2; ++j)
-                    acc_dw[kc][j] = __builtin_amdgcn_mfma_f32_16x16x32_bf16(ef, cf[j], acc_dw[kc][j], 0, 0, 0);
-            }
-            if (kc == 0) {
-#pragma unroll
-                for (int kb = 0; kb < 2; ++kb) {
-                    bf16x8_t af[2], wf[2];
-#pragma unroll
-                    for (int i = 0; i < 2; ++i)
-                        af[i] = *reinterpret_cast<const bf16x8_t*>(sXt + (wm * 32 + i * 16 + lr) * RS + (kb * 4 + lg) * 16);
-#pragma unroll
-                    for (int j = 0; j < 2; ++j)
-                        wf[j] = *reinterpret_cast<const bf16x8_t*>(sW + (wn * 32 + j * 16 + lr) * WRS + (E + kb * 32 + lg * 8) * 2);
-#pragma unroll
-                    for (int i = 0; i < 2; ++i)
-#pragma unroll
-                        for (int j = 0; j < 2; ++j)
-                            acc_da[i][j] = __builtin_amdgcn_mfma_f32_16x16x32_bf16(wf[j], af[i], acc_da[i][j], 0, 0, 0);
-                }
-#pragma unroll
-                for (int kb = 0; kb < BM / 32; ++kb) {
-                    const int rb = kb * 32 + 8 * lg + q;
-                    bf16x8_t ef, cf[2];
-                    {
-                        const int colb = (wm * 16 + 4 * p) * 2;
-                        auto lo = __builtin_amdgcn_ds_read_tr16_b64_v4i16((__attribute__((address_space(3))) s16x4_t*)(sXt + rb * RS + colb));
-                        auto hi = __builtin_amdgcn_ds_read_tr16_b64_v4i16((__attribute__((address_space(3))) s16x4_t*)(sXt + (rb + 4) * RS + colb));
-                        ef = bf16x8_t{lo[0], lo[1], lo[2], lo[3], hi[0], hi[1], hi[2], hi[3]};
-                    }
-#pragma unroll
-                    for (int j = 0; j < 2; ++j) {
-                        const int colb = (wn * 32 + j * 16 + 4 * p) * 2;
-                        auto lo = __builtin_amdgcn_ds_read_tr16_b64_v4i16((__attribute__((address_space(3))) s16x4_t*)(sXt + rb * RS + colb));
-                        auto hi = __builtin_amdgcn_ds_read_tr16_b64_v4i16((__attribute__((address_space(3))) s16x4_t*)(sXt + (rb + 4) * RS + colb));
-                        cf[j] = bf16x8_t{lo[0], lo[1], lo[2], lo[3], hi[0], hi[1], hi[2], hi[3]};
-                    }
-#pragma unroll
-                    for (int j = 0; j < 2; ++j) {
-                        acc_ga[j] = __builtin_amdgcn_mfma_f32_16x16x32_bf16(ef, cf[j], acc_ga[j], 0, 0, 0);
-                        if (wm == 0) acc_s[j] = __builtin_amdgcn_mfma_f32_16x16x32_bf16(ones, cf[j], acc_s[j], 0, 0, 0);
-                    }
-                }
-            }
-        }
-        step += NKC;
-#pragma unroll
-        for (int i = 0; i < 2; ++i)
-#pragma unroll
-            for (int j = 0; j < 2; ++j) {
-                const size_t m = m0 + wm * 32 + i * 16 + lr;
-                const int n = wn * 32 + j * 16 + 4 * lg;
-                const float4 b4 = *reinterpret_cast<const float4*>(sR3 + n);
-                float o[4] = {acc_da[i][j][0] + b4.x, acc_da[i][j][1] + b4.y, acc_da[i][j][2] + b4.z, acc_da[i][j][3] + b4.w};
-                if (res) {
-                    const int rc = res_n * CIN;
-                    float x4[4] = {0.f, 0.f, 0.f, 0.f};
-                    if (gather) {
-                        const uint2 xv = *reinterpret_cast<const uint2*>(sXt + (wm * 32 + i * 16 + lr) * RS + n * 2);
-                        x4[0] = __uint_as_float(xv.x << 16); x4[1] = __uint_as_float(xv.x & 0xffff0000u);
-                        x4[2] = __uint_as_float(xv.y << 16); x4[3] = __uint_as_float(xv.y & 0xffff0000u);
-                    }
-#pragma unroll
-                    for (int jj = 0; jj < 2; ++jj) {
-                        if (jj >= res_n || !rgat[i]) break;
-                        const uint2 rv = rres[i][j][jj];
-                        const float4 c4 = *reinterpret_cast<const float4*>(sR3 + CIN + jj * CIN + n);
-                        float t[4] = {c4.x * __uint_as_float(rv.x << 16), c4.y * __uint_as_float(rv.x & 0xffff0000u),
-                                      c4.z * __uint_as_float(rv.y << 16), c4.w * __uint_as_float(rv.y & 0xffff0000u)};
-                        if (gather) {
-                            const float4 a2 = *reinterpret_cast<const float4*>(sR3 + CIN + rc + jj * CIN + n);
-                            const float4 a3 = *reinterpret_cast<const float4*>(sR3 + CIN + 2 * rc + jj * CIN + n);
-                            t[0] += fmaf(a2.x, x4[0], a3.x); t[1] += fmaf(a2.y, x4[1], a3.y);
-                            t[2] += fmaf(a2.z, x4[2], a3.z); t[3] += fmaf(a2.w, x4[3], a3.w);
-                        }
-                        o[0] += t[0]; o[1] += t[1]; o[2] += t[2]; o[3] += t[3];
-                    }
-                }
-                uint2 v = make_uint2(pwb_pack2(o[0], o[1]), pwb_pack2(o[2], o[3]));
-                *reinterpret_cast<uint2*>(da0 + m * CIN + n) = v;
-            }
-    }
-    DET_ENTER();
-#pragma unroll
-    for (int kc = 0; kc < NKC; ++kc)
-#pragma unroll
-        for (int j = 0; j < 2; ++j)
-#pragma unroll
-            for (int r = 0; r < 4; ++r)
-                atomicAdd(tacc + (size_t)(kc * 64 + wm * 16 + 4 * lg + r) * CIN + wn * 32 + j * 16 + lr, acc_dw[kc][j][r]);
-#pragma unroll
-    for (int j = 0; j < 2; ++j) {
-#pragma unroll
-        for (int r = 0; r < 4; ++r)
-            atomicAdd(tacc + (size_t)(E + wm * 16 + 4 * lg + r) * CIN + wn * 32 + j * 16 + lr, acc_ga[j][r]);
-        if (wm == 0 && lg == 0) atomicAdd(tacc + (size_t)KCAT * CIN + wn * 32 + j * 16 + lr, acc_s[j][0]);
-    }
-    DET_EXIT();
+struct PwbSink { const float* x; const double* xmom; double* acc; double count; int Cin; unsigned S; };
+namespace pwb {
+constexpr int XRS = 48, SXA_BYTES = BM * XRS;
+constexpr int SINK_COLS = 6, SINK_MAXCIN = 5;
+constexpr int SINK_BYTES = SXA_BYTES + CIN * SINK_COLS * 8 + 32;
 }
+#define PWB_SINK 0
+#include "dwn_pw_bwd_kernel.inc"
+#undef PWB_SINK
+#define PWB_SINK 1
+#include "dwn_pw_bwd_kernel.inc"
+#undef PWB_SINK
 
 
 bool pw_bwd_fused_supported(int dtype, long long M, int E, int Cin) {
@@ -258,6 +45,23 @@
     DWN_CHECK_LAUNCH();
     return 0;
 }
+template <int NKC>
+static int launch_pw_bwd_sink_t(const void* dh1, const void* a0, const void* bp, const float* r3, float* tacc, long long M,
+                                const void* res, const float* res_coef, int res_n, const PwbGather& gq, const PwbSink& sk, hipStream_t s) {
+    auto kern = pw_bwd_sink_kernel<NKC>;
+    constexpr int LDS = pwb::Cfg<NKC>::LDS_BYTES + pwb::SINK_BYTES;
+    static_assert(LDS <= 160 * 1024, "pw_bwd_sink: LDS budget");
+    {
+        hipError_t e = lds_opt_in(kern, LDS);
+        if (e != hipSuccess) return dwn_set_error((int)e, hipGetErrorString(e));
+    }
+    int grid = 256;
+    if (grid > (int)(M / pwb::BM)) grid = (int)(M / pwb::BM);
+    hipLaunchKernelGGL(kern, dim3(grid), dim3(512), LDS, s, (const bf16_t*)dh1, (const bf16_t*)a0, (const bf16_t*)bp, r3, tacc, (int)M,
+                       (const bf16_t*)res, res_coef, res_n, gq, sk);
+    DWN_CHECK_LAUNCH();
+    return 0;
+}
 int launch_pw_bwd_fused(const void* dh1, const void* a0, const void* bp, const float* r3, void* da0, float* tacc,
                         long long M, int E, int Cin, int dtype, const void* res, const float* res_coef, int res_n,
                         const int* hinv, const int* winv, int Hin, int Win, int Hout, int Wout, hipStream_t s) {
@@ -270,3 +74,22 @@
     return E == 448 ? launch_pw_bwd_fused_t<7>(dh1, a0, bp, r3, da0, tacc, M, res, res_coef, res_n, gq, s)
                     : launch_pw_bwd_fused_t<6>(dh1, a0, bp, r3, da0, tacc, M, res, res_coef, res_n, gq, s);
 }
+
+int launch_pw_bwd_sink(const void* dh1, const void* a0, const void* bp, const float* r3, float* tacc, long long M, int E, int Cin,
+                       int dtype, const void* res, const float* res_coef, int res_n, const int* hinv, const int* winv, int Hin,
+                       int Win, int Hout, int Wout, const float* stem_x, const double* stem_xmom, double* stem_acc, int stem_Cin,
+                       long long stem_S, hipStream_t s) {
+    PwbGather gq; gq.hinv = hinv; gq.winv = winv; gq.Hin = Hin; gq.Win = Win; gq.Hout = Hout; gq.Wout = Wout;
+    if (!stem_x || !stem_xmom || !stem_acc) return dwn_set_error(-1, "pw_bwd_sink: null pointer (stem_x, stem_xmom, stem_acc)");
+    if (!res) return dwn_set_error(-3, "pw_bwd_sink: only where the shortcut term is folded in (the result is the block's input gradient)");
+    if (hinv && (!winv || Hin <= 0 || Win <= 0 || Hout <= 0 || Wout <= 0 || M % ((long long)Hin * Win) || Hin + Win > 512))
+        return dwn_set_error(-2, "pw_bwd_sink: the gathered shortcut form needs both inverse maps, M = frames * Hin * Win and Hin + Win <= 512");
+    if (!pw_bwd_fused_supported(dtype, M, E, Cin))
+        return dwn_set_error(-3, "pw_bwd_sink: built for bf16, Cin = 64, E = 448 or 384, M % 128 == 0 only");
+    if (!res_coef || res_n < 1 || res_n > 2) return dwn_set_error(-3, "pw_bwd_sink: the residual term needs res_coef and res_n in {1, 2}");
+    if (stem_Cin < 1 || stem_Cin > pwb::SINK_MAXCIN || stem_S <= 0 || M % stem_S)
+        return dwn_set_error(-3, "pw_bwd_sink: 1..5 stem input channels and M = samples * stem_S only");
+    PwbSink sk; sk.x = stem_x; sk.xmom = stem_xmom; sk.acc = stem_acc; sk.count = (double)M; sk.Cin = stem_Cin; sk.S = (unsigned)stem_S;
+    return E == 448 ? launch_pw_bwd_sink_t<7>(dh1, a0, bp, r3, tacc, M, res, res_coef, res_n, gq, sk, s)
+                    : launch_pw_bwd_sink_t<6>(dh1, a0, bp, r3, tacc, M, res, res_coef, res_n, gq, sk, s);
+}
diff --git a/sensorium_amd/csrc/dwn_pw_bwd_kernel.inc b/sensorium_amd/csrc/dwn_pw_bwd_kernel.inc
--- /dev/null
+++ b/sensorium_amd/csrc/dwn_pw_bwd_kernel.inc
@@ -0,0 +1,325 @@
+template <int NKC>
+#if PWB_SINK
+__global__ __launch_bounds__(512) __attribute__((amdgpu_waves_per_eu(2, 2))) void pw_bwd_sink_kernel(const bf16_t* __restrict__ dh1, const bf16_t* __restrict__ a0,
+                                                       const bf16_t* __restrict__ bp, const float* __restrict__ r3,
+                                                       float* __restrict__ tacc, int M,
+                                                       const bf16_t* __restrict__ res, const float* __restrict__ res_coef, int res_n,
+                                                       const PwbGather gq, const PwbSink sk) {
+#else
+__global__ __launch_bounds__(512) __attribute__((amdgpu_waves_per_eu(2, 2))) void pw_bwd_fused_kernel(const bf16_t* __restrict__ dh1, const bf16_t* __restrict__ a0,
+                                                       const bf16_t* __restrict__ bp, const float* __restrict__ r3,
+                                                       bf16_t* __restrict__ da0, float* __restrict__ tacc, int M,
+                                                       const bf16_t* __restrict__ res, const float* __restrict__ res_coef, int res_n,
+                                                       const PwbGather gq) {
+#endif
+    using namespace pwb;
+    constexpr int E = Cfg<NKC>::E, KCAT = Cfg<NKC>::KCAT, WRS = Cfg<NKC>::WRS;
+    constexpr int SW_BYTES = Cfg<NKC>::SW_BYTES, SD_BYTES = Cfg<NKC>::SD_BYTES, SX_BYTES = Cfg<NKC>::SX_BYTES;
+    extern __shared__ __attribute__((aligned(16))) unsigned char pwb_smem[];
+    unsigned char* const smem = pwb_smem;
+    unsigned char* sW = smem;
+    unsigned char* sD = smem + SW_BYTES;
+    unsigned char* sX = sD + 2 * SD_BYTES;
+    float* sR3 = reinterpret_cast<float*>(sX + 2 * SX_BYTES);
+    const int tid = threadIdx.x, wave = tid >> 6, lane = tid & 63;
+    const int lr = lane & 15, lg = lane >> 4;
+    const int wm = wave & 3, wn = wave >> 2;
+    if (tid < CIN) sR3[tid] = r3[tid];
+    const bool gather = res && gq.hinv;
+    if (res) for (int i = tid; i < (gather ? 3 : 1) * res_n * CIN; i += 512) sR3[CIN + i] = res_coef[i];
+    int* sMap = reinterpret_cast<int*>(sR3 + 7 * CIN);
+    if (gather) for (int i = tid; i < gq.Hin + gq.Win; i += 512) sMap[i] = i < gq.Hin ? gq.hinv[i] : gq.winv[i - gq.Hin];
+    const RasterIdx ridx(gather ? gq.Hin : 1, gather ? gq.Win : 1);
+    for (int c = tid; c < CIN * (KCAT / 8); c += 512) {
+        const int n = c / (KCAT / 8), kc8 = c % (KCAT / 8);
+        *reinterpret_cast<uint4*>(sW + n * WRS + kc8 * 16) = *reinterpret_cast<const uint4*>(bp + (size_t)n * KCAT + kc8 * 8);
+    }
+    f32x4_t acc_dw[NKC][2], acc_ga[2], acc_s[2];
+#pragma unroll
+    for (int k = 0; k < NKC; ++k) { acc_dw[k][0] = f32x4_t{0, 0, 0, 0}; acc_dw[k][1] = f32x4_t{0, 0, 0, 0}; }
+    acc_ga[0] = acc_ga[1] = acc_s[0] = acc_s[1] = f32x4_t{0, 0, 0, 0};
+    const int ntiles = M / BM;
+    const int ch = tid & 7;
+    const int row_a = tid >> 3;
+    struct Pair { uint4 lo, hi; };
+    Pair rd[NKC], rx;
+    auto fetch_a0 = [&](int tile) {
+        const bf16_t* src = a0 + ((size_t)tile * BM + row_a) * CIN + ch * 8;
+        return Pair{*reinterpret_cast<const uint4*>(src), *reinterpret_cast<const uint4*>(src + (size_t)64 * CIN)};
+    };
+    auto fetch_chunk = [&](int tile, int kc) {
+        const bf16_t* src = dh1 + ((size_t)tile * BM + row_a) * E + kc * 64 + ch * 8;
+        return Pair{*reinterpret_cast<const uint4*>(src), *reinterpret_cast<const uint4*>(src + (size_t)64 * E)};
+    };
+#if PWB_SINK
+    double* const sAcc = reinterpret_cast<double*>(sMap + Cfg<NKC>::MAP_INTS);
+    unsigned char* const sXa = reinterpret_cast<unsigned char*>(sAcc + CIN * SINK_COLS);
+    float* const sXbar = reinterpret_cast<float*>(sXa + SXA_BYTES);
+    const UDiv32 dS(sk.S);
+    struct XPair { float a, b; };
+    XPair xv = {0.f, 0.f};
+    auto fetch_x = [&](int tile) {
+        int tl = tid;
+        asm volatile("" : "+v"(tl));
+        const int xrow = tl & (BM - 1), xg = __builtin_amdgcn_readfirstlane(tl >> 7);
+        const unsigned m = (unsigned)tile * BM + xrow, b = dS.div(m), sp = m - b * sk.S;
+        const float* src = sk.x + (size_t)b * sk.Cin * sk.S + sp;
+        const int ca = xg < sk.Cin ? xg : sk.Cin - 1, cb = xg + 4 < sk.Cin ? xg + 4 : sk.Cin - 1;
+        return XPair{src[(size_t)ca * sk.S], src[(size_t)cb * sk.S]};
+    };
+    {
+        if (tid < 8) sXbar[tid] = tid < sk.Cin ? (float)(sk.xmom[tid] / sk.count) : 0.f;
+        for (int i = tid; i < CIN * SINK_COLS; i += 512) sAcc[i] = 0.0;
+        for (int i = tid; i < BM * 16; i += 512)
+            reinterpret_cast<unsigned short*>(sXa + (i >> 4) * XRS)[i & 15] = (i & 15) == sk.Cin ? (unsigned short)0x3F80 : (unsigned short)0;
+    }
+#endif
+    int tile = blockIdx.x;
+    {
+        const int t0 = tile < ntiles ? tile : 0;
+        rx = fetch_a0(t0);
+#pragma unroll
+        for (int kc = 0; kc < NKC; ++kc) rd[kc] = fetch_chunk(t0, kc);
+    }
+    __syncthreads();
+    const int q = lr >> 2, p = lr & 3;
+    const bf16x8_t ones = {(short)0x3F80, (short)0x3F80, (short)0x3F80, (short)0x3F80, (short)0x3F80, (short)0x3F80, (short)0x3F80, (short)0x3F80};
+    int tpar = 0, step = 0;
+    for (; tile < ntiles; tile += gridDim.x, tpar ^= 1) {
+        const size_t m0 = (size_t)tile * BM;
+        const int ntile = tile + (int)gridDim.x < ntiles ? tile + (int)gridDim.x : tile;
+        unsigned char* sXt = sX + tpar * SX_BYTES;
+        *reinterpret_cast<uint4*>(sXt + row_a * RS + ch * 16) = rx.lo;
+        *reinterpret_cast<uint4*>(sXt + (row_a + 64) * RS + ch * 16) = rx.hi;
+        rx = fetch_a0(ntile);
+        f32x4_t acc_da[2][2];
+        uint2 rres[2][2][2];
+        bool rgat[2] = {true, true};
+#pragma unroll
+        for (int i = 0; i < 2; ++i) { acc_da[i][0] = f32x4_t{0, 0, 0, 0}; acc_da[i][1] = f32x4_t{0, 0, 0, 0}; }
+#pragma unroll
+        for (int kc = 0; kc < NKC; ++kc) {
+            unsigned char* sDk = sD + ((step + kc) & 1) * SD_BYTES;
+            *reinterpret_cast<uint4*>(sDk + row_a * RS + ch * 16) = rd[kc].lo;
+            *reinterpret_cast<uint4*>(sDk + (row_a + 64) * RS + ch * 16) = rd[kc].hi;
+            nn_lds_barrier();
+            rd[kc] = fetch_chunk(ntile, kc);
+#if PWB_SINK
+            if (kc == NKC - 3) xv = fetch_x(tile);
+#endif
+            if (kc == NKC - 3 && res) {
+#pragma unroll
+                for (int i = 0; i < 2; ++i) {
+                    size_t rrow = m0 + wm * 32 + i * 16 + lr;
+                    if (gather) {
+                        unsigned bt; int hi, wi;
+                        ridx.decode((unsigned)rrow, bt, hi, wi);
+                        const int ho = sMap[hi], wo = sMap[gq.Hin + wi];
+                        rgat[i] = ho >= 0 && wo >= 0;
+                        rrow = rgat[i] ? ((size_t)bt * gq.Hout + ho) * gq.Wout + wo : 0;
+                    }
+#pragma unroll
+                    for (int j = 0; j < 2; ++j) {
+                        const bf16_t* rp_ = res + rrow * (size_t)(res_n * CIN) + wn * 32 + j * 16 + 4 * lg;
+                        rres[i][j][0] = *reinterpret_cast<const uint2*>(rp_);
+                        rres[i][j][1] = *reinterpret_cast<const uint2*>(rp_ + (res_n > 1 ? CIN : 0));
+                    }
+                }
+            }
+#pragma unroll
+            for (int kb = 0; kb < 2; ++kb) {
+                bf16x8_t af[2], wf[2];
+#pragma unroll
+                for (int i = 0; i < 2; ++i)
+                    af[i] = *reinterpret_cast<const bf16x8_t*>(sDk + (wm * 32 + i * 16 + lr) * RS + (kb * 4 + lg) * 16);
+#pragma unroll
+                for (int j = 0; j < 2; ++j)
+                    wf[j] = *reinterpret_cast<const bf16x8_t*>(sW + (wn * 32 + j * 16 + lr) * WRS + (kc * 64 + kb * 32 + lg * 8) * 2);
+#pragma unroll
+                for (int i = 0; i < 2; ++i)
+#pragma unroll
+                    for (int j = 0; j < 2; ++j)
+                        acc_da[i][j] = __builtin_amdgcn_mfma_f32_16x16x32_bf16(wf[j], af[i], acc_da[i][j], 0, 0, 0);
+            }
+#pragma unroll
+            for (int kb = 0; kb < BM / 32; ++kb) {
+                const int rb = kb * 32 + 8 * lg + q;
+                bf16x8_t ef, cf[2];
+                {
+                    const int colb = (wm * 16 + 4 * p) * 2;
+                    auto lo = __builtin_amdgcn_ds_read_tr16_b64_v4i16((__attribute__((address_space(3))) s16x4_t*)(sDk + rb * RS + colb));
+                    auto hi = __builtin_amdgcn_ds_read_tr16_b64_v4i16((__attribute__((address_space(3))) s16x4_t*)(sDk + (rb + 4) * RS + colb));
+                    ef = bf16x8_t{lo[0], lo[1], lo[2], lo[3], hi[0], hi[1], hi[2], hi[3]};
+                }
+#pragma unroll
+                for (int j = 0; j < 2; ++j) {
+                    const int colb = (wn * 32 + j * 16 + 4 * p) * 2;
+                    auto lo = __builtin_amdgcn_ds_read_tr16_b64_v4i16((__attribute__((address_space(3))) s16x4_t*)(sXt + rb * RS + colb));
+                    auto hi = __builtin_amdgcn_ds_read_tr16_b64_v4i16((__attribute__((address_space(3))) s16x4_t*)(sXt + (rb + 4) * RS + colb));
+                    cf[j] = bf16x8_t{lo[0], lo[1], lo[2], lo[3], hi[0], hi[1], hi[2], hi[3]};
+                }
+#pragma unroll
+                for (int j = 0; j < 2; ++j)
+                    acc_dw[kc][j] = __builtin_amdgcn_mfma_f32_16x16x32_bf16(ef, cf[j], acc_dw[kc][j], 0, 0, 0);
+            }
+            if (kc == 0) {
+#pragma unroll
+                for (int kb = 0; kb < 2; ++kb) {
+                    bf16x8_t af[2], wf[2];
+#pragma unroll
+                    for (int i = 0; i < 2; ++i)
+                        af[i] = *reinterpret_cast<const bf16x8_t*>(sXt + (wm * 32 + i * 16 + lr) * RS + (kb * 4 + lg) * 16);
+#pragma unroll
+                    for (int j = 0; j < 2; ++j)
+                        wf[j] = *reinterpret_cast<const bf16x8_t*>(sW + (wn * 32 + j * 16 + lr) * WRS + (E + kb * 32 + lg * 8) * 2);
+#pragma unroll
+                    for (int i = 0; i < 2; ++i)
+#pragma unroll
+                        for (int j = 0; j < 2; ++j)
+                            acc_da[i][j] = __builtin_amdgcn_mfma_f32_16x16x32_bf16(wf[j], af[i], acc_da[i][j], 0, 0, 0);
+                }
+#pragma unroll
+                for (int kb = 0; kb < BM / 32; ++kb) {
+                    const int rb = kb * 32 + 8 * lg + q;
+                    bf16x8_t ef, cf[2];
+                    {
+                        const int colb = (wm * 16 + 4 * p) * 2;
+                        auto lo = __builtin_amdgcn_ds_read_tr16_b64_v4i16((__attribute__((address_space(3))) s16x4_t*)(sXt + rb * RS + colb));
+                        auto hi = __builtin_amdgcn_ds_read_tr16_b64_v4i16((__attribute__((address_space(3))) s16x4_t*)(sXt + (rb + 4) * RS + colb));
+                        ef = bf16x8_t{lo[0], lo[1], lo[2], lo[3], hi[0], hi[1], hi[2], hi[3]};
+                    }
+#pragma unroll
+                    for (int j = 0; j < 2; ++j) {
+                        const int colb = (wn * 32 + j * 16 + 4 * p) * 2;
+                        auto lo = __builtin_amdgcn_ds_read_tr16_b64_v4i16((__attribute__((address_space(3))) s16x4_t*)(sXt + rb * RS + colb));
+                        auto hi = __builtin_amdgcn_ds_read_tr16_b64_v4i16((__attribute__((address_space(3))) s16x4_t*)(sXt + (rb + 4) * RS + colb));
+                        cf[j] = bf16x8_t{lo[0], lo[1], lo[2], lo[3], hi[0], hi[1], hi[2], hi[3]};
+                    }
+#pragma unroll
+                    for (int j = 0; j < 2; ++j) {
+                        acc_ga[j] = __builtin_amdgcn_mfma_f32_16x16x32_bf16(ef, cf[j], acc_ga[j], 0, 0, 0);
+                        if (wm == 0) acc_s[j] = __builtin_amdgcn_mfma_f32_16x16x32_bf16(ones, cf[j], acc_s[j], 0, 0, 0);
+                    }
+                }
+            }
+        }
+#if PWB_SINK
+        unsigned char* const sSt = sD + ((step + NKC) & 1) * SD_BYTES;
+        step += NKC + 1;
+#else
+        step += NKC;
+#endif
+#pragma unroll
+        for (int i = 0; i < 2; ++i)
+#pragma unroll
+            for (int j = 0; j < 2; ++j) {
+                const size_t m = m0 + wm * 32 + i * 16 + lr;
+                const int n = wn * 32 + j * 16 + 4 * lg;
+                const float4 b4 = *reinterpret_cast<const float4*>(sR3 + n);
+                float o[4] = {acc_da[i][j][0] + b4.x, acc_da[i][j][1] + b4.y, acc_da[i][j][2] + b4.z, acc_da[i][j][3] + b4.w};
+                if (res) {
+                    const int rc = res_n * CIN;
+                    float x4[4] = {0.f, 0.f, 0.f, 0.f};
+                    if (gather) {
+                        const uint2 xv = *reinterpret_cast<const uint2*>(sXt + (wm * 32 + i * 16 + lr) * RS + n * 2);
+                        x4[0] = __uint_as_float(xv.x << 16); x4[1] = __uint_as_float(xv.x & 0xffff0000u);
+                        x4[2] = __uint_as_float(xv.y << 16); x4[3] = __uint_as_float(xv.y & 0xffff0000u);
+                    }
+#pragma unroll
+                    for (int jj = 0; jj < 2; ++jj) {
+                        if (jj >= res_n || !rgat[i]) break;
+                        const uint2 rv = rres[i][j][jj];
+                        const float4 c4 = *reinterpret_cast<const float4*>(sR3 + CIN + jj * CIN + n);
+                        float t[4] = {c4.x * __uint_as_float(rv.x << 16), c4.y * __uint_as_float(rv.x & 0xffff0000u),
+                                      c4.z * __uint_as_float(rv.y << 16), c4.w * __uint_as_float(rv.y & 0xffff0000u)};
+                        if (gather) {
+                            const float4 a2 = *reinterpret_cast<const float4*>(sR3 + CIN + rc + jj * CIN + n);
+                            const float4 a3 = *reinterpret_cast<const float4*>(sR3 + CIN + 2 * rc + jj * CIN + n);
+                            t[0] += fmaf(a2.x, x4[0], a3.x); t[1] += fmaf(a2.y, x4[1], a3.y);
+                            t[2] += fmaf(a2.z, x4[2], a3.z); t[3] += fmaf(a2.w, x4[3], a3.w);
+                        }
+                        o[0] += t[0]; o[1] += t[1]; o[2] += t[2]; o[3] += t[3];
+                    }
+                }
+                uint2 v = make_uint2(pwb_pack2(o[0], o[1]), pwb_pack2(o[2], o[3]));
+#if PWB_SINK
+                *reinterpret_cast<uint2*>(sSt + (wm * 32 + i * 16 + lr) * RS + n * 2) = v;
+#else
+                *reinterpret_cast<uint2*>(da0 + m * CIN + n) = v;
+#endif
+            }
+#if PWB_SINK
+        {
+            int tl = tid;
+            asm volatile("" : "+v"(tl));
+            {
+                const int xrow = tl & (BM - 1), xg = __builtin_amdgcn_readfirstlane(tl >> 7);
+                const float da = xv.a - sXbar[xg], db = xv.b - sXbar[xg + 4];
+                const unsigned h = pk_bf16(da, db);
+                const float ra = da - __uint_as_float(h << 16), rb_ = db - __uint_as_float(h & 0xffff0000u);
+                const unsigned md = pk_bf16(ra, rb_);
+                const unsigned l = pk_bf16(ra - __uint_as_float(md << 16), rb_ - __uint_as_float(md & 0xffff0000u));
+                unsigned short* xr = reinterpret_cast<unsigned short*>(sXa + xrow * XRS);
+                const int c1 = sk.Cin + 1 + xg, c2 = 2 * sk.Cin + 1 + xg;
+                if (xg < sk.Cin) { xr[xg] = (unsigned short)(h & 0xffffu); xr[c1] = (unsigned short)(md & 0xffffu); xr[c2] = (unsigned short)(l & 0xffffu); }
+                if (xg + 4 < sk.Cin) { xr[xg + 4] = (unsigned short)(h >> 16); xr[c1 + 4] = (unsigned short)(md >> 16); xr[c2 + 4] = (unsigned short)(l >> 16); }
+            }
+            nn_lds_barrier();
+            if (tl < 256) {
+            const int lr = tl & 15, lg = (tl >> 4) & 3, wm = tl >> 6, q = lr >> 2, p = lr & 3;
+            f32x4_t acc_st = f32x4_t{0, 0, 0, 0};
+#pragma unroll
+            for (int kh = 0; kh < BM / 32; ++kh) {
+                const int rb = kh * 32 + 8 * lg + q;
+                bf16x8_t ef, cf;
+                {
+                    const int colb = (wm * 16 + 4 * p) * 2;
+                    auto lo = __builtin_amdgcn_ds_read_tr16_b64_v4i16((__attribute__((address_space(3))) s16x4_t*)(sSt + rb * RS + colb));
+                    auto hi = __builtin_amdgcn_ds_read_tr16_b64_v4i16((__attribute__((address_space(3))) s16x4_t*)(sSt + (rb + 4) * RS + colb));
+                    ef = bf16x8_t{lo[0], lo[1], lo[2], lo[3], hi[0], hi[1], hi[2], hi[3]};
+                }
+                {
+                    const int colb = (4 * p) * 2;
+                    auto lo = __builtin_amdgcn_ds_read_tr16_b64_v4i16((__attribute__((address_space(3))) s16x4_t*)(sXa + rb * XRS + colb));
+                    auto hi = __builtin_amdgcn_ds_read_tr16_b64_v4i16((__attribute__((address_space(3))) s16x4_t*)(sXa + (rb + 4) * XRS + colb));
+                    cf = bf16x8_t{lo[0], lo[1], lo[2], lo[3], hi[0], hi[1], hi[2], hi[3]};
+                }
+                acc_st = __builtin_amdgcn_mfma_f32_16x16x32_bf16(ef, cf, acc_st, 0, 0, 0);
+            }
+#pragma unroll
+            for (int r = 0; r < 4; ++r) {
+                const float vm = __shfl(acc_st[r], (tl & 63) + sk.Cin + 1), vl = __shfl(acc_st[r], (tl & 63) + 2 * sk.Cin + 1);
+                if (lr <= sk.Cin)
+                    sAcc[(wm * 16 + 4 * lg + r) * SINK_COLS + lr] += lr < sk.Cin ? ((double)vl + (double)vm) + (double)acc_st[r] : (double)acc_st[r];
+            }
+            }
+        }
+#endif
+    }
+    DET_ENTER();
+#pragma unroll
+    for (int kc = 0; kc < NKC; ++kc)
+#pragma unroll
+        for (int j = 0; j < 2; ++j)
+#pragma unroll
+            for (int r = 0; r < 4; ++r)
+                atomicAdd(tacc + (size_t)(kc * 64 + wm * 16 + 4 * lg + r) * CIN + wn * 32 + j * 16 + lr, acc_dw[kc][j][r]);
+#pragma unroll
+    for (int j = 0; j < 2; ++j) {
+#pragma unroll
+        for (int r = 0; r < 4; ++r)
+            atomicAdd(tacc + (size_t)(E + wm * 16 + 4 * lg + r) * CIN + wn * 32 + j * 16 + lr, acc_ga[j][r]);
+        if (wm == 0 && lg == 0) atomicAdd(tacc + (size_t)KCAT * CIN + wn * 32 + j * 16 + lr, acc_s[j][0]);
+    }
+#if PWB_SINK
+    {
+        if (wn == 0 && lr <= sk.Cin)
+#pragma unroll
+            for (int r = 0; r < 4; ++r) {
+                atomicAdd(sk.acc + ((size_t)(blockIdx.x % DWN_NREP) * CIN + wm * 16 + 4 * lg + r) * 9 + (lr < sk.Cin ? lr : 8),
+                          sAcc[(wm * 16 + 4 * lg + r) * SINK_COLS + lr]);
+            }
+    }
+#endif
+    DET_EXIT();
+}
diff --git a/sensorium_amd/dwiseneuro.py b/sensorium_amd/dwiseneuro.py
--- a/sensorium_amd/dwiseneuro.py
+++ b/sensorium_amd/dwiseneuro.py
@@ -281,8 +281,23 @@
             s = blk.spatial_stride
             h, w = (h - 1) // s + 1, (w - 1) // s + 1
         tables = [blk.geometry(pe, t, hw[0], hw[1], x.device)[:3] for pe, blk, hw in zip(pes, blks, sizes)]
-        x = ops.StemFn.apply(x, self.stem[0].weight, bn.weight, bn.bias, self, dtype, tables[0], ops.bn_mode(bn.training, x))
+        stem_mode = ops.bn_mode(bn.training, x)
+        first = 0
+        stem_trains = any(p.requires_grad for p in self.stem.parameters())
+        blk0_mode = ops.bn_mode_flag(blks[0].conv_pw[1].bn.training, stem_trains)
+        if stem_trains and ops.stem_sink_applies(x, self, blks[0], dtype, stem_mode, blk0_mode):
+            b = x.shape[0]
+            geom = blks[0].geometry(pes[0], t, sizes[0][0], sizes[0][1], x.device)
+            drop = blks[0].drop_path.sample(b, x.device)
+            x = ops.StemBlock0Fn.apply(x, drop, self, blks[0], geom, dtype, tables[0], tables[1] if len(blks) > 1 else None,
+                                       stem_mode, blk0_mode, self.stem[0].weight, bn.weight, bn.bias,
+                                       *blks[0].parameters_in_kernel_order())
+            first = 1
+        else:
+            x = ops.StemFn.apply(x, self.stem[0].weight, bn.weight, bn.bias, self, dtype, tables[0], stem_mode)
         for i, (pe, blk) in enumerate(zip(pes, blks)):
+            if i < first:
+                continue
             x = blk(x, pe, dtype, True, tables[i + 1] if i + 1 < len(blks) else None)
         return x
 
diff --git a/sensorium_amd/ops.py b/sensorium_amd/ops.py
--- a/sensorium_amd/ops.py
+++ b/sensorium_amd/ops.py
@@ -83,11 +83,15 @@
 
 
 def bn_mode(training: bool, x: torch.Tensor) -> int:
+    return bn_mode_flag(training, bool(x.requires_grad))
+
+
+def bn_mode_flag(training: bool, input_needs_grad: bool) -> int:
     if training:
         return L.BN_TRAIN
     if _BN_MODE.override is not None:
         return _BN_MODE.override
-    return L.BN_FROZEN if wants_frozen(x) else L.BN_EVAL
+    return L.BN_FROZEN if torch.is_grad_enabled() and input_needs_grad else L.BN_EVAL
 
 
 def _ddp_flush() -> None:
@@ -311,10 +315,14 @@
 
     @staticmethod
     def backward(ctx, dout):
+        dx, grads = BlockFn.run_backward(ctx, ctx.saved_tensors, dout)
+        return (dx, None, None, None, None, None, None, None) + grads
+
+    @staticmethod
+    def run_backward(ctx, t, dout, sink=None):
         if ctx.mode == L.BN_EVAL:
             raise RuntimeError(_EVAL_BACKWARD_ERROR)
         blk, dtype = ctx.blk, ctx.dtype
-        t = ctx.saved_tensors
         x, y1, y2, y3, y4 = t[:5]
         coefs = list(t[5:10])
         saved = dict(pmean=t[10], hidpre=t[11], gate=t[12])
@@ -337,8 +345,8 @@
         buf_a = torch.empty(max(m_in, m_out) * Cmid, dtype=dtype, device=dev)
         buf_b = torch.empty(m_out * Cmid, dtype=dtype, device=dev)
         dy4 = torch.empty(m_out * Cout, dtype=dtype, device=dev)
-        da0 = torch.empty(m_in * Cin, dtype=dtype, device=dev)
-        dx = torch.empty_like(x)
+        da0 = torch.empty(m_in * Cin, dtype=dtype, device=dev) if sink is None else None
+        dx = torch.empty_like(x) if sink is None else None
         R = blk.se.conv_reduce.out_channels
         dw_pw = grad_out(blk.conv_pw[0].weight)
         dw_dws = grad_out(blk.spat_covn_dw[0].weight)
@@ -346,8 +354,12 @@
         dw_pwl = grad_out(blk.conv_pwl[0].weight)
         dse_wr = grad_out(blk.se.conv_reduce.weight); dse_br = grad_out(blk.se.conv_reduce.bias)
         dse_we = grad_out(blk.se.conv_expand.weight); dse_be = grad_out(blk.se.conv_expand.bias)
-        a.dout = dout.data_ptr(); a.dx = dx.data_ptr()
-        a.buf_a = buf_a.data_ptr(); a.buf_b = buf_b.data_ptr(); a.dy4 = dy4.data_ptr(); a.da0 = da0.data_ptr()
+        a.dout = dout.data_ptr(); a.dx = _ptr(dx)
+        a.buf_a = buf_a.data_ptr(); a.buf_b = buf_b.data_ptr(); a.dy4 = dy4.data_ptr(); a.da0 = _ptr(da0)
+        if sink is not None:
+            stem_x, stem_xmom, stem_acc = sink
+            a.stem_x = stem_x.data_ptr(); a.stem_xmom = stem_xmom.data_ptr(); a.stem_acc = stem_acc.data_ptr()
+            a.stem_Cin = stem_x.shape[1]
         a.dw_pw = dw_pw.data_ptr(); a.dw_dws = dw_dws.data_ptr(); a.dw_dwt = dw_dwt.data_ptr()
         a.dw_pwl = dw_pwl.data_ptr()
         a.dse_wr = dse_wr.data_ptr(); a.dse_br = dse_br.data_ptr(); a.dse_we = dse_we.data_ptr()
@@ -359,7 +371,73 @@
         _ddp_flush()
         grads = (dw_pw, dg[0], db[0], dw_dws, dg[1], db[1], dw_dwt, dg[2], db[2], dse_wr, dse_br, dse_we, dse_be,
                  dw_pwl, dg[3], db[3], dg[4], db[4])
-        return (dx, None, None, None, None, None, None, None) + grads
+        return dx, grads
+
+
+_STEM_SINK = _env_choice("DWN_STEM_SINK", {"": 1, "on": 1, "off": 0})
+STEM_SINK_MAXCIN = 5
+
+
+def stem_sink_applies(x, core, blk, dtype, stem_mode: int, blk_mode: int) -> bool:
+    if not (_STEM_SINK and getattr(core, "_dwn_stem_sink", True) and hasattr(L.lib, "dwn_stem_backward_finalize")):
+        return False
+    if stem_mode != L.BN_TRAIN or blk_mode == L.BN_EVAL or dtype != torch.bfloat16:
+        return False
+    if not torch.is_grad_enabled() or x.requires_grad or x.dim() != 5:
+        return False
+    B, Cin, T, H, W = x.shape
+    C0, Cmid, Cout = blk.in_features, blk.mid_features, blk.out_features
+    if Cin > STEM_SINK_MAXCIN or core.stem[0].out_channels != C0 or Cout % C0 or Cout // C0 > 2 or H + W > 512:
+        return False
+    return bool(L.lib.dwn_pw_bwd_fused_supported(L.DWN_BF16, B * T * H * W, Cmid, C0))
+
+
+class _InnerCtx:
+    saved_tensors = ()
+
+    def save_for_backward(self, *tensors):
+        self.saved_tensors = tensors
+
+
+class StemBlock0Fn(torch.autograd.Function):
+
+    @staticmethod
+    def forward(ctx, x, drop_scale, core, blk, geom, dtype, pe, out_pe, stem_mode, blk_mode, weight, gamma, beta, *params):
+        sctx, bctx = _InnerCtx(), _InnerCtx()
+        a0 = StemFn.forward(sctx, x, weight, gamma, beta, core, dtype, pe, stem_mode)
+        out = BlockFn.forward(bctx, a0, drop_scale, blk, geom, dtype, True, out_pe, blk_mode, *params)
+        ctx.sctx, ctx.bctx = sctx, bctx
+        ctx.n_stem = len(sctx.saved_tensors)
+        ctx.none_at = [i for i, t in enumerate(bctx.saved_tensors) if t is None]
+        ctx.save_for_backward(*sctx.saved_tensors, *[t for t in bctx.saved_tensors if t is not None])
+        sctx.saved_tensors = bctx.saved_tensors = ()
+        return out
+
+    @staticmethod
+    def backward(ctx, dout):
+        saved = list(ctx.saved_tensors)
+        x, weight, xmom, coef = saved[:ctx.n_stem]
+        bt = saved[ctx.n_stem:]
+        for i in ctx.none_at:
+            bt.insert(i, None)
+        core = ctx.sctx.mod
+        bn = core.stem[1].bn
+        dev = x.device
+        B, Cin, T, H, W = x.shape
+        C0 = weight.shape[0]
+        acc = torch.empty(L.DWN_NREP * C0 * 9, dtype=torch.float64, device=dev)
+        _, grads = BlockFn.run_backward(ctx.bctx, bt, dout, sink=(x, xmom, acc))
+        dw = grad_out(core.stem[0].weight)
+        dgamma = grad_out(bn.weight)
+        dbeta = grad_out(bn.bias)
+        a = L.StemArgs()
+        a.dtype = _DT[ctx.sctx.dtype]; a.training = ctx.sctx.mode; a.B = B; a.Cin = Cin; a.C0 = C0; a.S = T * H * W
+        a.eps = bn.eps; a.momentum = bn.momentum
+        a.x = x.data_ptr(); a.w = weight.data_ptr(); a.bn = _bn_struct(bn, coef, dgamma, dbeta)
+        a.xmom = xmom.data_ptr(); a.dw = dw.data_ptr()
+        L.check(L.lib.dwn_stem_backward_finalize(C.byref(a), acc.data_ptr(), dev.index, _stream(dev)), "dwn_stem_backward_finalize")
+        _ddp_flush()
+        return (None,) * 10 + (dw, dgamma, dbeta) + grads
 
 
 class PoolFn(torch.autograd.Function):
```
